# profess-dev/profess-ad

Hardware: AMD Instinct MI355X
Metric: energy+grad evals/sec (higher is better)
Workload: dtype f64; 1 GPU; 256^3 grid, f64, IonElectron+Hartree+WGC99(+TF+vW)+PBE closure chi->(E,dE/dchi); density=converged fcc-Al 32^3 fixture tiled 8^3 + 1e-3 low-|k| perturbation, parallelism=single GPU

## Files before the change

include/ofdft_hip.h:

```cpp
#ifndef OFDFT_HIP_H
#define OFDFT_HIP_H

#include <stdint.h>

#ifdef __cplusplus
extern "C" {
#endif

typedef struct ofdft_ctx ofdft_ctx;

#define OFDFT_OK            0
#define OFDFT_EINVAL       -1
#define OFDFT_EHIP         -2
#define OFDFT_ESTATE       -3
#define OFDFT_ENOMEM       -4

#define OFDFT_F64 0
#define OFDFT_F32 1

#define OFDFT_ION_ELECTRON  (1u << 0)
#define OFDFT_HARTREE       (1u << 1)
#define OFDFT_TF            (1u << 2)
#define OFDFT_VW            (1u << 3)
#define OFDFT_WT_NL         (1u << 4)
#define OFDFT_WGC99_NL      (1u << 5)
#define OFDFT_LDA_X         (1u << 6)
#define OFDFT_PZ_C          (1u << 7)
#define OFDFT_PW_C          (1u << 8)
#define OFDFT_CHACHIYO_C    (1u << 9)
#define OFDFT_PBE_X         (1u << 10)
#define OFDFT_PBE_C         (1u << 11)
#define OFDFT_GGA_K         (1u << 12)
#define OFDFT_VWGTF         (1u << 13)
#define OFDFT_NTERMS        14

#define OFDFT_P_WT_ALPHA    0
#define OFDFT_P_WT_BETA     1
#define OFDFT_P_WGC_ALPHA   2
#define OFDFT_P_WGC_BETA    3
#define OFDFT_P_WGC_GAMMA   4
#define OFDFT_P_WGC_KAPPA   5
#define OFDFT_P_GGAK_KIND   6
#define OFDFT_P_GGAK_MU     7
#define OFDFT_P_GGAK_BETA   8
#define OFDFT_P_GGAK_LAMBDA 9
#define OFDFT_P_GGAK_SIGMA  10
#define OFDFT_P_VWGTF_KIND  11
#define OFDFT_P_WTS_KIND    12
#define OFDFT_NPARAMS       13

#define OFDFT_Q_FFT_COUNT        0
#define OFDFT_Q_WORKSPACE_BYTES  1
#define OFDFT_Q_FAST_PATH        2
#define OFDFT_Q_KERNEL_MS        3
#define OFDFT_Q_LAUNCH_COUNT     4
#define OFDFT_Q_YPASS_COUNT      5
#define OFDFT_Q_GRAPH_REPLAYS     6
#define OFDFT_Q_RESIDENT_EVALS    7
#define OFDFT_Q_XCHG_CHUNKS      9
#define OFDFT_Q_YFWD_FUSED      10
#define OFDFT_Q_RESIDENT_FALLBACKS 8
#define OFDFT_Q_XPASS_KINDS     11
#define OFDFT_XPASS_GROUP    (1u << 0)
#define OFDFT_XPASS_WAVE     (1u << 1)
#define OFDFT_XPASS_CROSS1   (1u << 2)
#define OFDFT_XPASS_CROSS2   (1u << 3)
#define OFDFT_XPASS_CHIRPZ   (1u << 4)

int  ofdft_create(ofdft_ctx** out, int n0, int n1, int n2, int dtype, int device_id);
void ofdft_destroy(ofdft_ctx* ctx);
const char* ofdft_last_error(const ofdft_ctx* ctx);

int  ofdft_set_cell(ofdft_ctx* ctx, const double box_vecs[9]);
int  ofdft_set_terms(ofdft_ctx* ctx, uint32_t term_mask, const double* params, int nparams);

int  ofdft_energy_potential(ofdft_ctx* ctx, const void* den_dev, const void* vext_dev,
                            double* E_terms_host, void* dEdn_dev, void* stream);

int  ofdft_energy_grad_chi(ofdft_ctx* ctx, const void* chi_dev, const void* vext_dev, double n_electrons,
                           double* E_terms_host, double* mu_host, void* grad_dev, void* stream);

int  ofdft_rfftn(ofdft_ctx* ctx, const void* real_dev, void* spec_dev, void* stream);
int  ofdft_irfftn(ofdft_ctx* ctx, const void* spec_dev, void* real_dev, void* stream);
int  ofdft_debug_math(ofdft_ctx* ctx, int kind, const void* in_dev, void* out_dev, long long n, void* stream);

int  ofdft_query(ofdft_ctx* ctx, int what, double* out);

int  ofdft_ipc_export(ofdft_ctx* ctx, void* handle64, unsigned long long* offsets5);
int  ofdft_ipc_attach(ofdft_ctx* ctx, int peer_rank, const void* handle64, const unsigned long long* offsets5);
int  ofdft_ipc_detach(ofdft_ctx* ctx);
int  ofdft_dist_closure(ofdft_ctx* ctx, const void* chi_local_dev, const void* vext_local_dev, double n_electrons_global,
                        double* E_terms_host, double* mu_host, void* grad_local_dev, void* v_work_local_dev, void* stream);

typedef int (*ofdft_all_to_all_fn)(void* user, void* send_dev, void* recv_dev, unsigned long long bytes_per_peer, void* stream);
typedef int (*ofdft_all_reduce_fn)(void* user, double* host_buf, int count);
int  ofdft_set_collectives(ofdft_ctx* ctx, ofdft_all_to_all_fn all_to_all, ofdft_all_reduce_fn all_reduce, void* user);

int  ofdft_create_dist(ofdft_ctx** out, int n0_global, int n1_global, int n2, int dtype, int device_id, int nranks, int rank);
int  ofdft_dist_sumsq(ofdft_ctx* ctx, const void* x_local_dev, int square, double* local_sum_host, void* stream);
int  ofdft_dist_begin(ofdft_ctx* ctx, const void* src_local_dev, int from_chi, double cscale, double n_electrons_global,
                      const void* vext_local_dev, void* v_out_local_dev, void* stream);
int  ofdft_dist_stage(ofdft_ctx* ctx, int stage, int chain, void* stream, unsigned long long* bytes_per_peer, void** sendbuf_dev,
                      void** recvbuf_dev);
int  ofdft_dist_step(ofdft_ctx* ctx, int step, int chain, int chunk, void* stream, unsigned long long* bytes_per_peer,
                     void** sendbuf_dev, void** recvbuf_dev);
int  ofdft_dist_finish(ofdft_ctx* ctx, double* local_sums_host , void* stream);
int  ofdft_dist_scalars(ofdft_ctx* ctx, void** scalars_dev );
int  ofdft_dist_energies(ofdft_ctx* ctx, const double* global_sums , double* E_terms_host, double* vn_integral);
int  ofdft_dist_chi_grad(ofdft_ctx* ctx, const void* chi_local_dev, const void* v_local_dev, void* grad_local_dev,
                         double cscale, double mu, void* stream);

int  ofdft_ionic_potential(ofdft_ctx* ctx, const double* frac_coords_host, int nions, const double* table_k_host,
                           const double* table_v_host, int ntable, double z_ion, int pme_order, void* vext_dev,
                           int accumulate, void* stream);

int  ofdft_ion_electron_forces(ofdft_ctx* ctx, const void* den_dev, const double* frac_coords_host, int nions,
                               const double* table_k_host, const double* table_v_host, int ntable, double z_ion,
                               int pme_order, double* forces_host, void* stream);

int  ofdft_stress(ofdft_ctx* ctx, const void* den_dev, double* sigma_terms_host, void* stream);
int  ofdft_ion_electron_stress(ofdft_ctx* ctx, const void* den_dev, const double* frac_coords_host, int nions,
                               const double* table_k_host, const double* table_v_host, int ntable, double z_ion,
                               int pme_order, double* sigma_host , void* stream);

int  ofdft_ion_ion(ofdft_ctx* ctx, const double* frac_coords_host, const double* charges_host, int nions, double Rc,
                   double* E_host, double* forces_host, double* stress_host, void* stream);

typedef struct ofdft_lbfgs ofdft_lbfgs;
int  ofdft_lbfgs_create(ofdft_lbfgs** out, long long n_local, int history , int device_id);
void ofdft_lbfgs_destroy(ofdft_lbfgs* h);
const char* ofdft_lbfgs_last_error(const ofdft_lbfgs* h);
int  ofdft_lbfgs_reset(ofdft_lbfgs* h);
int  ofdft_lbfgs_direction(ofdft_lbfgs* h, const double* dots , int npairs, int first_iteration,
                           double* coef_s , double* coef_y , double* coef_g, double* g_dot_d,
                           int* npairs_out, int* pushed_out);
int  ofdft_lbfgs_abs_step(ofdft_lbfgs* h, double* abs_step_sum);
int  ofdft_lbfgs_dots(ofdft_lbfgs* h, const void* g_dev, double* dots_host , int* npairs, void* stream);
int  ofdft_lbfgs_commit(ofdft_lbfgs* h, int push);
int  ofdft_lbfgs_update(ofdft_lbfgs* h, const double* coef_s, const double* coef_y, double coef_g, double t, void* x_dev,
                        const void* g_dev, double* abs_step_sum_host, void* stream);

#define OFDFT_OPT_PIPELINE 0
#define OFDFT_OPT_XCHUNKS     2
#define OFDFT_OPT_XCHUNK_MASK 3
#define OFDFT_OPT_SPLIT_COMBINE 4
#define OFDFT_OPT_BLUESTEIN 5
#define OFDFT_OPT_GGA_SPLIT 6
#define OFDFT_OPT_GRAPH 7
#define OFDFT_OPT_SIDE_STREAM 1
#define OFDFT_OPT_MIXED_RADIX 9
#define OFDFT_OPT_RESIDENT 10
#define OFDFT_OPT_XCHG_CHUNKS 12
#define OFDFT_OPT_YBATCH 14
#define OFDFT_OPT_IPC_WAIT_MS 13
#define OFDFT_OPT_TEST_FAULT 11
#define OFDFT_OPT_BS_FUSED 15
#define OFDFT_OPT_WGC_FOLD 28
#define OFDFT_OPT_XWAVE 8
int  ofdft_set_option(ofdft_ctx* ctx, int option, double value);

int  ofdft_set_profiling(ofdft_ctx* ctx, int on);
int  ofdft_profile_count(ofdft_ctx* ctx);
int  ofdft_profile_get(ofdft_ctx* ctx, int idx, char* name_buf, int buflen, double* total_ms, long long* launches);

#ifdef __cplusplus
}
#endif
#endif
```

professad_amd/csrc/engine.hip:

```cpp
#include "engine_ctx.h"
#include <atomic>
#include <chrono>
#ifndef OFDFT_REAL_F32
#include "ion_kernels.h"
#include "stress_kernels.h"
#endif

namespace {
thread_local char g_create_error[512] = "";
}

namespace eng {

int fail(ofdft_ctx* c, int code, const char* fmt, ...) {
    va_list ap;
    va_start(ap, fmt);
    vsnprintf(c ? c->err : g_create_error, 512, fmt, ap);
    va_end(ap);
    return code;
}

int get_twiddle(ofdft_ctx* c, int n, cplx** out) {
    auto it = c->tw.find(n);
    if (it != c->tw.end()) {
// ... 1344 lines not shown
        *bytes_per_peer = (unsigned long long)(sizeof(cplx) * (size_t)c->xg.nxl * c->xg.arr_sz * r.xlist[chain].size());
        *sendbuf = send;
        *recvbuf = recv;
        c->recv_parity[chain] ^= 1;
    }
    HIP_TRY(c, hipGetLastError());
    return OFDFT_OK;
}

int ofdft_dist_step(ofdft_ctx* c, int step, int chain, int chunk, void* stream, unsigned long long* bytes_per_peer, void** sendbuf,
                    void** recvbuf) {
    hipStream_t st = (hipStream_t)stream;
    if (!c || !bytes_per_peer || !sendbuf || !recvbuf || chain < 0 || chain > 1) return OFDFT_EINVAL;
    OFDFT_ON_DEVICE(c, c->device);
    ZRun& r = zrun(c);
    const int K = c->xc.n;
    const bool next_chunk = step == r.step[chain] && chunk == r.step_chunk[chain] + 1 && chunk < K;
    const bool next_step = step == r.step[chain] + 1 && chunk == 0 && (r.step[chain] == 0 || r.step_chunk[chain] == K - 1);
    if (step < 1 || step > 6 || !(next_chunk || next_step) || (chain == 1 && r.step[0] < 1))
        return fail(c, OFDFT_ESTATE, "step %d chunk %d of chain %d out of order (last: step %d chunk %d of %d)", step, chunk, chain,
                    r.step[chain], r.step_chunk[chain], K);
    int rc;
    switch (step) {
        case 1: rc = zstage1(c, st, chain, chunk); break;
        case 2: rc = zstage2(c, st, chain, chunk); break;
        case 3: rc = zstage3(c, st, chain, 1, chunk); break;
        case 4: rc = zstage3(c, st, chain, 2, chunk); break;
        case 5: rc = zstage4(c, st, chain, chunk); break;
        default: rc = chain == 0 ? zstage5(c, nullptr, st, false, 1, chunk) : 0; break;
    }
    if (rc) return rc;
    r.step[chain] = step;
    r.step_chunk[chain] = chunk;
    *bytes_per_peer = 0;
    *sendbuf = *recvbuf = nullptr;
    const bool sends = step == 1 || step == 2 || step == 4 || step == 5;
    if (sends && c->nranks > 1 && !r.xlist[chain].empty()) {
        cplx *send, *recv;
        if ((rc = dist_buffers(c, chain, &send, &recv))) return rc;
        if ((rc = dist_recv_next(c, chain, &recv))) return rc;
        const XcView v = xc_view(c, chunk);
        const long long narr = (long long)r.xlist[chain].size();
        *bytes_per_peer = (unsigned long long)(sizeof(cplx) * (size_t)c->xg.nxl * v.arr_sz * narr);
        *sendbuf = send + narr * v.base1;
        *recvbuf = recv + narr * v.base1;
        if (chunk == K - 1) c->recv_parity[chain] ^= 1;
    }
    if (step == 5 && chunk == K - 1) r.stage[chain] = 4;
    HIP_TRY(c, hipGetLastError());
    return OFDFT_OK;
}

int ofdft_dist_finish(ofdft_ctx* c, double* local_sums, void* stream) {
    hipStream_t st = (hipStream_t)stream;
    if (!c) return OFDFT_EINVAL;
    OFDFT_ON_DEVICE(c, c->device);
    ZRun& r = zrun(c);
    if (r.stage[0] != 4 || r.stage[1] != 4) return fail(c, OFDFT_ESTATE, "ofdft_dist_finish called before stage 4 of both chains");
    const bool stepped = r.step[0] > 0;
    if (stepped && !(r.step[0] == 6 && r.step_chunk[0] == c->xc.n - 1 && r.step[1] == 6 && r.step_chunk[1] == c->xc.n - 1))
        return fail(c, OFDFT_ESTATE, "ofdft_dist_finish called before step 6 of both chains");
    int rc;
    if ((rc = zstage5(c, local_sums, st, false, stepped ? 2 : 0))) return rc;
    if (!local_sums) {
        HIP_TRY(c, hipEventRecord(c->ev1, st));
        c->ms_pending = true;
        HIP_TRY(c, hipGetLastError());
        if (c->profiling) {
            HIP_TRY(c, hipStreamSynchronize(st));
            prof_collect(c);
        }
        return OFDFT_OK;
    }
    return end_call(c, st);
}

int ofdft_dist_energies(ofdft_ctx* c, const double* global_sums, double* E_terms, double* vn_int) {
    if (!c || !global_sums || !E_terms || !vn_int) return OFDFT_EINVAL;
    for (int i = 0; i < OFDFT_NTERMS; ++i) E_terms[i] = 0.0;
    energies_from_sums(c, global_sums, global_sums + kCombineScalars, E_terms, vn_int);
    return OFDFT_OK;
}

int ofdft_dist_chi_grad(ofdft_ctx* c, const void* chi_local, const void* v_local, void* grad_local, double cscale,
                        double mu, void* stream) {
    hipStream_t st = (hipStream_t)stream;
    if (!c || !chi_local || !v_local || !grad_local) return OFDFT_EINVAL;
    OFDFT_ON_DEVICE(c, c->device);
    OFDFT_LAUNCH(c, st, "chi_grad", chi_grad_kernel, dim3(grid_for(c->npts / 2 + 1)), dim3(256), 0, (const real*)chi_local,
                 (const real*)v_local, (real*)grad_local, c->npts, cscale * 2.0 * c->dV,
                 cscale > 0.0 ? (const acc_t*)nullptr : (const acc_t*)c->d_scal, 2.0 * c->dV, mu);
    HIP_TRY(c, hipGetLastError());
    return OFDFT_OK;
}

#ifndef OFDFT_REAL_F32
#include "engine_ions_stress.inc.h"
#else
#define OFDFT_F64_ONLY(c) fail(c, OFDFT_EINVAL, "%s is served by the fp64 library (libofdft_hip.so) only", __func__)
extern "C" {
int ofdft_ionic_potential(ofdft_ctx* c, const double*, int, const double*, const double*, int, double, int, void*, int, void*) {
    return OFDFT_F64_ONLY(c);
}
int ofdft_ion_electron_forces(ofdft_ctx* c, const void*, const double*, int, const double*, const double*, int, double, int,
                              double*, void*) {
    return OFDFT_F64_ONLY(c);
}
int ofdft_stress(ofdft_ctx* c, const void*, double*, void*) { return OFDFT_F64_ONLY(c); }
int ofdft_ion_electron_stress(ofdft_ctx* c, const void*, const double*, int, const double*, const double*, int, double, int,
                              double*, void*) {
    return OFDFT_F64_ONLY(c);
}
int ofdft_ion_ion(ofdft_ctx* c, const double*, const double*, int, double, double*, double*, double*, void*) {
    return OFDFT_F64_ONLY(c);
}
}
#endif

int ofdft_set_collectives(ofdft_ctx* c, ofdft_all_to_all_fn all_to_all, ofdft_all_reduce_fn all_reduce, void* user) {
    if (!c) return OFDFT_EINVAL;
    c->a2a = all_to_all;
    c->allreduce = all_reduce;
    c->coll_user = user;
    return OFDFT_OK;
}

int ofdft_set_option(ofdft_ctx* c, int option, double value) {
    if (!c) return OFDFT_EINVAL;
    c->version++;
    switch (option) {
        case OFDFT_OPT_GRAPH:
            c->use_graph = value != 0.0;
            return OFDFT_OK;
        case OFDFT_OPT_PIPELINE:
            c->force_unfused = value == 1.0;
            c->pipeline = (int)value;
            return OFDFT_OK;
        case OFDFT_OPT_SIDE_STREAM:
            c->use_side_stream = value != 0.0;
            return OFDFT_OK;
        case OFDFT_OPT_XCHUNKS:
            if (value < 0.0 || value > 64.0) return fail(c, OFDFT_EINVAL, "x chunks must be 0 (automatic) or 1..64");
            c->xchunks = (int)value;
            return OFDFT_OK;
        case OFDFT_OPT_BLUESTEIN:
            c->use_bluestein = value != 0.0;
            return OFDFT_OK;
        case OFDFT_OPT_BS_FUSED:
            c->bs_fused = value != 0.0;
            return OFDFT_OK;
        case OFDFT_OPT_GGA_SPLIT:
            c->gga_split = value != 0.0;
            return OFDFT_OK;
        case OFDFT_OPT_SPLIT_COMBINE:
            c->split_combine = value != 0.0;
            c->defer_vpart = value != 1.0;
            return OFDFT_OK;
        case OFDFT_OPT_XCHUNK_MASK:
            c->xchunk_mask = (int)value & 31;
            return OFDFT_OK;
        case OFDFT_OPT_MIXED_RADIX:
            if (c->nranks > 1 && value == 0.0 && !all_pow2(c))
                return fail(c, OFDFT_EINVAL, "a slab-decomposed context on extents with factors 3 / 5 has no other path than the mixed-radix plans");
            c->fast = line_extent_ok(c->n0g) && line_extent_ok(c->n1g) && row_extent_ok(c->n2) && is_pow2(c->nranks) &&
                      (value != 0.0 || all_pow2(c));
            return OFDFT_OK;
        case OFDFT_OPT_XWAVE:
            c->use_xwave = (int)value;
            return OFDFT_OK;
        case OFDFT_OPT_RESIDENT:
            if (value != 0.0 && value != 1.0 && value != 2.0) return fail(c, OFDFT_EINVAL, "OFDFT_OPT_RESIDENT takes 0, 1 or 2");
            c->resident = (int)value;
            return OFDFT_OK;
        case OFDFT_OPT_XCHG_CHUNKS:
            if (value < 0.0 || value > 16.0) return fail(c, OFDFT_EINVAL, "OFDFT_OPT_XCHG_CHUNKS takes 0 (automatic) or 1..16");
            xchg_chunks_set(c, (int)value);
            c->wgc_valid = false;
            return OFDFT_OK;
        case OFDFT_OPT_YBATCH:
            c->ybatch = (int)value;
            return OFDFT_OK;
        case OFDFT_OPT_WGC_FOLD:
            c->wgc_fold = value != 0.0;
            return OFDFT_OK;
        case OFDFT_OPT_IPC_WAIT_MS:
            if (!(value >= 1.0 && value <= 3.6e6)) return fail(c, OFDFT_EINVAL, "OFDFT_OPT_IPC_WAIT_MS takes 1 .. 3 600 000 ms");
            c->ipc_wait_ms = value;
            return OFDFT_OK;
        case OFDFT_OPT_TEST_FAULT:
            c->test_fault = (int)value;
            if (c->test_fault == 2) c->res_fits = 0;
            return OFDFT_OK;
    }
    return fail(c, OFDFT_EINVAL, "unknown option %d", option);
}

int ofdft_set_profiling(ofdft_ctx* c, int on) {
    if (!c) return OFDFT_EINVAL;
    c->profiling = on != 0;
    c->prof.clear();
    c->pending.clear();
    c->ev_used = 0;
    return OFDFT_OK;
}

int ofdft_profile_count(ofdft_ctx* c) { return c ? (int)c->prof.size() : OFDFT_EINVAL; }

int ofdft_profile_get(ofdft_ctx* c, int idx, char* name_buf, int buflen, double* total_ms, long long* launches) {
    if (!c || idx < 0 || idx >= (int)c->prof.size() || !name_buf || buflen < 2) return OFDFT_EINVAL;
    auto it = c->prof.begin();
    std::advance(it, idx);
    std::snprintf(name_buf, (size_t)buflen, "%s", it->first.c_str());
    if (total_ms) *total_ms = it->second.ms;
    if (launches) *launches = it->second.launches;
    return OFDFT_OK;
}

int ofdft_query(ofdft_ctx* c, int what, double* out) {
    if (!c || !out) return OFDFT_EINVAL;
    switch (what) {
        case OFDFT_Q_FFT_COUNT: *out = c->fft_count; return OFDFT_OK;
        case OFDFT_Q_WORKSPACE_BYTES: *out = (double)c->ws_bytes; return OFDFT_OK;
        case OFDFT_Q_FAST_PATH: *out = c->fast ? 1.0 : 0.0; return OFDFT_OK;
        case OFDFT_Q_KERNEL_MS:
            if (c->ms_pending) {
                OFDFT_ON_DEVICE(c, c->device);
                HIP_TRY(c, hipEventSynchronize(c->ev1));
                HIP_TRY(c, hipEventElapsedTime(&c->last_ms, c->ev0, c->ev1));
                c->ms_pending = false;
            }
            *out = c->last_ms;
            return OFDFT_OK;
        case OFDFT_Q_LAUNCH_COUNT: *out = c->launch_count; return OFDFT_OK;
        case OFDFT_Q_YPASS_COUNT: *out = c->ypass_count; return OFDFT_OK;
        case OFDFT_Q_GRAPH_REPLAYS: *out = (double)c->graph_replays; return OFDFT_OK;
        case OFDFT_Q_RESIDENT_EVALS: *out = (double)c->resident_evals; return OFDFT_OK;
        case OFDFT_Q_RESIDENT_FALLBACKS: *out = (double)c->resident_fallbacks; return OFDFT_OK;
        case OFDFT_Q_XCHG_CHUNKS: *out = (double)c->xc.n; return OFDFT_OK;
        case OFDFT_Q_YFWD_FUSED: *out = (double)c->yfwd_fused; return OFDFT_OK;
        case OFDFT_Q_XPASS_KINDS: *out = (double)c->xpass_kinds; return OFDFT_OK;
        case 16: case 17: case 18: case 19: case 20: case 21: case 22: case 23: case 24: case 25: case 26: case 27:
            *out = c->h_partial[what] * 0.01;
            return OFDFT_OK;
    }
    return fail(c, OFDFT_EINVAL, "unknown query %d", what);
}

}

#include "lbfgs_abi.h"
```

professad_amd/csrc/engine_ctx.h:

```cpp
#pragma once
#include <hip/hip_runtime.h>

#include <algorithm>
#include <cmath>
#include <cstdarg>
#include <cstdio>
#include <cstring>
#include <map>
#include <string>
#include <vector>

#include "../../include/ofdft_hip.h"
#include "bluestein.h"
#include "zpass.h"
#include "xwave.h"

using namespace ofdft;

struct DevBuf {
    void* p = nullptr;
    size_t bytes = 0;
    bool borrowed = false;
};

struct XchgChunks {
    int n = 1;
    int kb[17] = {0};
};

struct ofdft_ctx {
    int n0 = 0, n1 = 0, n2 = 0, device = 0;
    int n0g = 0, n1g = 0, nranks = 1, rank = 0;
    SpecGeom g{};
    SpecGeom gx{};
    KGeom kg{};
    XchgGeom xg{};
    XchgChunks xc{};
    int xchg_chunks_req = 0;
    long long npts = 0;
    long long npts_g = 0;
    bool fast = false, cell_set = false, force_unfused = false;
    int pipeline = 0;
    double box[9] = {0}, vol = 0.0, dV = 0.0;
    unsigned mask = 0;
    double params[OFDFT_NPARAMS];
    std::map<int, cplx*> tw;
    std::map<std::string, DevBuf> ws;
    size_t ws_bytes = 0;
    double* d_partial = nullptr;
    double* d_reduced = nullptr;
    double* d_scal = nullptr;
    double* h_partial = nullptr;
    long long partial_rows = 0;
    double* d_wgc_coef = nullptr;
    long long wgc_key_nel = -1;
    int fft_passes_fused = 0;
    int yfwd_fused = 0;
    bool wgc_valid = false;
    double wgc_ck = 0.0;
    bool wgc_fold = true;
    int fft_count = 0, launch_count = 0;
    unsigned xpass_kinds = 0;
    double ypass_count = 0.0;
    float last_ms = 0.f;
    bool ms_pending = false;
    hipEvent_t ev0 = nullptr, ev1 = nullptr, ev_fork = nullptr, ev_join = nullptr, ev_join2 = nullptr, ev_a = nullptr, ev_b = nullptr, ev_c = nullptr;
    hipStream_t side_stream = nullptr, side_stream2 = nullptr;
    bool use_side_stream = true;
    bool bs_fused = true;
    bool use_bluestein = true;
    bool gga_split = true;
    bool split_combine = true;
    bool defer_vpart = true;
    int ybatch = 1;
    int xchunk_mask = 2;
    int use_xwave = 1;
    int xchunks = 1;
    bool profiling = false;
    std::vector<hipEvent_t> ev_pool;
    size_t ev_used = 0;
    struct Pending { const char* name; size_t a, b; };
    std::vector<Pending> pending;
    struct Acc { double ms = 0.0; long long launches = 0; };
    std::map<std::string, Acc> prof;
    struct ofdft_zrun_holder* zr = nullptr;
    struct GraphEntry {
        const void *chi = nullptr, *vext = nullptr, *grad = nullptr;
        double nel = 0.0;
        unsigned long long version = 0;
        int seen = 0;
        hipGraphExec_t exec = nullptr;
        int collect = 0;
        int fft_count = 0, launch_count = 0, yfwd_fused = 0;
        unsigned xpass_kinds = 0;
        double ypass_count = 0.0;
    };
    std::vector<GraphEntry> graphs;
    unsigned long long version = 1;
    bool use_graph = true;
    int resident = 2;
    unsigned* res_sync = nullptr;
    unsigned res_epoch = 0;
    long long resident_evals = 0;
    int test_fault = 0;
    int res_fits = -1;
    long long resident_fallbacks = 0;
    unsigned* res_done = nullptr;
    unsigned res_done_target = 0;
    long long graph_replays = 0;
    hipStream_t cap_stream = nullptr;
    struct ofdft_ipc_state* ipc = nullptr;
    int recv_parity[2] = {0, 0};
    double ipc_wait_ms = 30000.0;
    ofdft_all_to_all_fn a2a = nullptr;
    ofdft_all_reduce_fn allreduce = nullptr;
    void* coll_user = nullptr;
    char err[512] = "";
};


namespace eng {

constexpr unsigned kGgaAny = OFDFT_PBE_X | OFDFT_PBE_C | OFDFT_GGA_K;
constexpr int kNSums = kCombineScalars + kPbeScalars;
constexpr int kSumsqSlot = 15;

inline GgaSel gga_sel(const ofdft_ctx* c) {
    return GgaSel{(c->mask & OFDFT_PBE_X) ? 1 : 0, (c->mask & OFDFT_PBE_C) ? 1 : 0, (c->mask & OFDFT_GGA_K) ? 1 : 0,
                  (int)c->params[OFDFT_P_GGAK_KIND], (real)c->params[OFDFT_P_GGAK_MU], (real)c->params[OFDFT_P_GGAK_BETA],
                  (real)c->params[OFDFT_P_GGAK_LAMBDA], (real)c->params[OFDFT_P_GGAK_SIGMA]};
}

inline bool gga_needs_laplacian(const ofdft_ctx* c) {
    return (c->mask & OFDFT_GGA_K) && (int)c->params[OFDFT_P_GGAK_KIND] == 1 &&
           (c->params[OFDFT_P_GGAK_BETA] != 0.0 || c->params[OFDFT_P_GGAK_LAMBDA] != 0.0 || c->params[OFDFT_P_GGAK_SIGMA] != 0.0);
}
inline bool wts_active(const ofdft_ctx* c) {
    return (int)c->params[OFDFT_P_WTS_KIND] == 1 && (c->mask & OFDFT_TF) && (c->mask & OFDFT_WT_NL);
}
inline bool zfused_serves(const ofdft_ctx* c) {
    return c->fast && c->pipeline == 0 && c->n2 / 2 <= 512 && (!gga_needs_laplacian(c) || c->gga_split);
}

int fail(ofdft_ctx* c, int code, const char* fmt, ...);

#define HIP_TRY(ctx, call)                                                                         \
    do {                                                                                           \
        hipError_t e_ = (call);                                                                    \
        if (e_ != hipSuccess)                                                                      \
            return fail(ctx, OFDFT_EHIP, "%s failed: %s (%s:%d)", #call, hipGetErrorString(e_), __FILE__, __LINE__); \
    } while (0)


#define OFDFT_ON_DEVICE(ctx, dev)                                                                   \
    DeviceScope device_scope_(dev);                                                                 \
    if (device_scope_.err != hipSuccess)                                                            \
        return fail(ctx, OFDFT_EHIP, "cannot select device %d: %s", (dev), hipGetErrorString(device_scope_.err))

inline bool graph_eligible(const ofdft_ctx* c) { return c->use_graph && c->nranks == 1 && c->npts <= (1LL << 19); }
void prof_begin(ofdft_ctx* c, hipStream_t st, const char* name);
void prof_end(ofdft_ctx* c, hipStream_t st);
void prof_collect(ofdft_ctx* c);

#define OFDFT_LAUNCH(c, st, name, kern, grid, block, lds, ...)            \
    do {                                                                  \
        prof_begin(c, st, name);                                          \
        hipLaunchKernelGGL(kern, grid, block, lds, st, __VA_ARGS__);      \
        prof_end(c, st);                                                  \
        (c)->launch_count++;                                              \
    } while (0)

inline bool is_pow2(int n) { return n > 0 && (n & (n - 1)) == 0; }

#if !defined(OFDFT_REAL_F32) || !defined(OFDFT_NO_MIXED_F32)
#define OFDFT_MIXED_LINES(X) X(48) X(96) X(120) X(144) X(160) X(192) X(240) X(250) X(270) X(288) X(320) X(384) X(480)
#define OFDFT_MIXED_ROWS(X) X(24) X(48) X(60) X(72) X(80) X(96) X(120) X(125) X(135) X(144) X(160) X(192) X(240)
#else
#define OFDFT_MIXED_LINES(X)
#define OFDFT_MIXED_ROWS(X)
#endif
inline bool mixed_line(int n) {
#define X(L) if (n == L) return true;
    OFDFT_MIXED_LINES(X)
#undef X
    return false;
}
inline bool line_extent_ok(int n) { return (is_pow2(n) && n >= 8 && n <= 1024) || mixed_line(n); }
inline bool row_extent_ok(int n2) { return (is_pow2(n2) && n2 >= 16 && n2 <= 2048) || mixed_line(n2); }
inline bool all_pow2(const ofdft_ctx* c) { return is_pow2(c->n0g) && is_pow2(c->n1g) && is_pow2(c->n2); }

inline int grid_for(long long n, int tpb = 256, int cap = 2048) {
    long long b = (n + tpb - 1) / tpb;
    if (b > cap) b = cap;
    if (b < 1) b = 1;
    return (int)b;
}

#define OFDFT_REDUCE(c, st, partial, rows, ns, ...)                                                                          \
    do {                                                                                                                     \
        const acc_t* part_ = (partial);                                                                                      \
        const int rows_ = (rows), ns_ = (ns);                                                                                \
        if (rows_ > kRedTwoLevelRows) {                                                                                      \
            acc_t* mid_ = const_cast<acc_t*>(part_) + (size_t)rows_ * ns_;                                                   \
            int g_ = rows_ / 512;                                                                                            \
            g_ = g_ < 1 ? 1 : (g_ > kRedMidRows ? kRedMidRows : g_);                                                         \
            const int per_ = (rows_ + g_ - 1) / g_;                                                                          \
            g_ = (rows_ + per_ - 1) / per_;                                                                                  \
            OFDFT_LAUNCH(c, st, "reduce", reduce_rows_kernel, dim3(g_), dim3(kRedThreads), 0, part_, rows_, ns_, per_, mid_); \
            OFDFT_LAUNCH(c, st, "reduce", reduce_partials_kernel, dim3(ns_), dim3(kRedThreads), 0, (const acc_t*)mid_, g_, ns_, \
                         __VA_ARGS__);                                                                                       \
        } else {                                                                                                             \
            OFDFT_LAUNCH(c, st, "reduce", reduce_partials_kernel, dim3(ns_), dim3(kRedThreads), 0, part_, rows_, ns_, __VA_ARGS__); \
        }                                                                                                                    \
    } while (0)


constexpr int kWholeXchg = -2;
struct XcView {
    int kb0, kb1, nb, nrem;
    long long arr_sz;
    long long base1;
};
inline XcView xc_view(const ofdft_ctx* c, int k) {
    XcView v{};
    const bool whole = k == kWholeXchg || c->xc.n <= 1;
    v.kb0 = whole ? 0 : c->xc.kb[k];
    v.kb1 = whole ? c->xg.nb : c->xc.kb[k + 1];
    v.nb = v.kb1 - v.kb0;
    v.nrem = (whole || k == c->xc.n - 1) ? c->xg.nrem : 0;
    v.arr_sz = ((long long)v.nb * 8 + v.nrem) * c->xg.nyl;
    v.base1 = (long long)c->n0g * c->xg.nyl * 8 * v.kb0;
    return v;
}
inline int xchg_chunks_for(const ofdft_ctx* c, int req) {
    if (c->nranks < 2 || c->xg.nb < 2 || c->xg.nxl % 32 || c->xg.nyl % 32) return 1;
    int k = req;
    if (k <= 0) {
        k = c->npts >= (8LL << 20) ? 4 : (c->npts >= (1LL << 20) ? 2 : 1);
        k = std::min(k, c->xg.nb / 4);
    }
    k = std::max(1, std::min(k, std::min(16, c->xg.nb)));
    return k;
}
inline void xchg_chunks_set(ofdft_ctx* c, int req) {
    c->xchg_chunks_req = req;
    c->xc = XchgChunks{};
    c->xc.n = xchg_chunks_for(c, req);
    for (int k = 0; k <= c->xc.n; ++k) c->xc.kb[k] = (int)((long long)c->xg.nb * k / c->xc.n);
}

int get_twiddle(ofdft_ctx* c, int n, cplx** out);
int get_ws(ofdft_ctx* c, const std::string& name, size_t bytes, void** out);
int real_ws(ofdft_ctx* c, const char* name, real** out);
int spec_ws(ofdft_ctx* c, const char* name, cplx** out);
size_t dist_buffer_bytes(ofdft_ctx* c, int chain);
int dist_buffers(ofdft_ctx* c, int chain, cplx** send, cplx** recv);
int dist_recv_next(ofdft_ctx* c, int chain, cplx** recv);
int dist_exchange(ofdft_ctx* c, cplx* send, cplx* recv, hipStream_t st);
int global_sums(ofdft_ctx* c, double* v, int n);

void pass_maps(const ofdft_ctx* c, int axis, LineMap& main, LineMap& rem);
template <bool INV>
int fast_axis_pass_multi(ofdft_ctx* c, int axis, cplx* const* specs, int narr, hipStream_t st, int x0 = 0, int cx = 0,
                         int kb0 = 0, int kb1 = 0);
template <bool INV> int fast_axis_pass(ofdft_ctx* c, int axis, cplx* spec, hipStream_t st);
template <bool INV> int ypass_xchg(ofdft_ctx* c, const std::vector<cplx*>& list, cplx* buf, hipStream_t st, int xk = -1);
int yderiv(ofdft_ctx* c, const cplx* in, cplx* out, double scale, hipStream_t st, cplx* fwd = nullptr);
int rfftn_internal(ofdft_ctx* c, const real* in, cplx* spec, hipStream_t st);
int rfftn_internal_multi(ofdft_ctx* c, const real* const* in, cplx* const* spec, int n, hipStream_t st);
bool bluestein_xmix_ok(const ofdft_ctx* c);
template <int NIN, int NOUT, class Mix>
int bluestein_xmix(ofdft_ctx* c, const cplx* const* in, cplx* const* out, const Mix& mix, hipStream_t st);
struct BsPrep { int kind[kBsBatch] = {0, 0, 0, 0}; double e[kBsBatch] = {0, 0, 0, 0}; double nref = 0.0; };
int bluestein_fwd_zy_multi(ofdft_ctx* c, const real* const* in, cplx* const* spec, int n, hipStream_t st, const BsPrep* prep = nullptr);
int bluestein_inv_yz_multi(ofdft_ctx* c, cplx* const* spec, real* const* out, int n, double scale, hipStream_t st);
int irfftn_internal_multi(ofdft_ctx* c, cplx* const* spec, real* const* out, int n, double scale, hipStream_t st);
int irfftn_internal(ofdft_ctx* c, cplx* spec, real* out, double scale, hipStream_t st);
int fwd_zy(ofdft_ctx* c, const real* in, cplx* spec, hipStream_t st);
int inv_yz(ofdft_ctx* c, cplx* spec, real* out, double scale, hipStream_t st);

struct XfLayout {
    long long se_in = 0, se_out = 0, tse = 0;
    int kb0 = 0, kb1 = 0;
    int xnb = -1, xnrem = 0;
    int kz0 = 0;
};
template <int NIN, int NOUT, class Mix>
int xfused(ofdft_ctx* c, const XfIo& io, const Mix& mix, hipStream_t st, const char* nm, const XfLayout& lay = XfLayout{});
int xfused_wgc(ofdft_ctx* c, const XfIo& io, const MixWgc& mix, hipStream_t st, const char* nm, const XfLayout& lay = XfLayout{});

int launch_zf_density(ofdft_ctx* c, const DenSrc& ds, cplx* out_n, cplx* out_s, hipStream_t st, int chunk = 0, int nchunks = 1,
                      real* dzn = nullptr);
int ensure_wgc_tables(ofdft_ctx* c, long long nel_rounded, hipStream_t st, double* nref_out);
inline MixWgc wgc_tab(ofdft_ctx* c, long long off = 0) {
    const cplx* t01 = (const cplx*)c->ws["t:wgc"].p;
    return MixWgc{t01 + off, reinterpret_cast<const real*>(t01 + c->g.total) + off, (real)c->wgc_ck};
}
bool resident_serves(const ofdft_ctx* c);
constexpr int kResidentDeclined = 1;
int resident_closure(ofdft_ctx* c, const real* chi, const real* vext, double nel, real* v, real* grad, hipStream_t st, bool from_den = false);
int launch_zf_powers(ofdft_ctx* c, const DenSrc& ds, const PowersArgs& pa, hipStream_t st, int chunk = 0, int nchunks = 1);
int launch_zpbe(ofdft_ctx* c, const DenSrc& ds, cplx* gx, cplx* gy, cplx* gz, real* dfdn, double inv_n, int* blocks_out,
                hipStream_t st, int chunk = 0, int nchunks = 1);
int launch_zpbe2(ofdft_ctx* c, const DenSrc& ds, cplx* A, cplx* B, const real* dzn, real* dfdn, double inv_n, int* blocks_out,
                 hipStream_t st, cplx* L = nullptr);
int launch_zi_combine(ofdft_ctx* c, const ZCombineArgs& a, int* blocks_out, hipStream_t st, int chunk = 0, int nchunks = 1);
int launch_zi_wgc(ofdft_ctx* c, const ZCombineArgs& a, real* v_part, double* partial, int* blocks_out, hipStream_t st);

}
```

professad_amd/csrc/engine_zfused.inc.h:

```cpp
void energies_from_sums(const ofdft_ctx* c, const double* sums, const double* pbe_sums, double* E_terms, double* vn_int) {
    const unsigned mask = c->mask;
    const double dV = c->dV;
    if (mask & OFDFT_ION_ELECTRON) E_terms[0] = sums[0] * dV;
    if (mask & OFDFT_HARTREE) E_terms[1] = sums[1] * dV;
    if (mask & OFDFT_TF) E_terms[2] = sums[2] * dV;
    if (mask & OFDFT_VW) E_terms[3] = sums[3] * dV;
    if (mask & OFDFT_WT_NL) E_terms[4] = sums[4] * dV;
    if (mask & OFDFT_WGC99_NL) E_terms[5] = sums[5] * dV;
    if (mask & OFDFT_LDA_X) E_terms[6] = sums[6] * dV;
    int nc = 0;
    for (int b = 7; b <= 9; ++b) nc += (mask >> b) & 1;
    for (int b = 7; b <= 9; ++b)
        if ((mask >> b) & 1) E_terms[b] = sums[7] * dV / nc;
    if (mask & OFDFT_PBE_X) E_terms[10] = pbe_sums[0] * dV;
    if (mask & OFDFT_PBE_C) E_terms[11] = pbe_sums[1] * dV;
    if (mask & OFDFT_GGA_K) E_terms[12] = pbe_sums[2] * dV;
    if (mask & OFDFT_VWGTF) E_terms[13] = sums[9] * dV;
    *vn_int = sums[8] * dV;
}

struct ZRun {
    DenSrc ds{};
    double nel = 0.0;
    const real* vext = nullptr;
    real* v_out = nullptr;
    ZCombineArgs za{};
    double pbe_sums[kPbeScalars] = {0.0, 0.0, 0.0};
    bool has_h = false, has_g = false, has_vw = false, has_wt = false, has_wgc = false;
    cplx *s_n = nullptr, *s_s = nullptr, *s_vh = nullptr, *s_g[3] = {nullptr, nullptr, nullptr};
    cplx *s_b = nullptr, *s_a = nullptr, *sw[6] = {nullptr, nullptr, nullptr, nullptr, nullptr, nullptr};
    real* dfdn = nullptr;
    double wt_pref = 0.0, wt_kf = 1.0;
    std::vector<cplx*> xlist[2];
    bool gsplit = false;
    bool lapl = false;
    cplx* s_l = nullptr;
    real* dzn = nullptr;
    bool wgc_yinv_done = false;
    bool wgc_split = false;
    bool closure = false;
    bool setup_done = false;
    bool late_join = false;
    bool vpart_deferred = false;
    std::vector<cplx*> deferred;
    int stage[2] = {0, 0};
    int step[2] = {0, 0}, step_chunk[2] = {0, 0};
    std::vector<cplx*> in_list[2];
    int combine_blocks = 0, pbe_blocks = 0;
    hipStream_t sb = nullptr;
    hipStream_t sc = nullptr;
    bool forked = false;
};

}
struct ofdft_zrun_holder { ZRun r; };
namespace {

ZRun& zrun(ofdft_ctx* c);

int chunks_for(const ofdft_ctx* c, int narr, int which = 15) {
    if (c->nranks > 1 || c->xchunks == 1 || !(c->xchunk_mask & which) || !all_pow2(c)) return 1;
    if (which == 8 && wts_active(c)) return 1;
    int want = c->xchunks > 1 ? (c->xchunks * narr + 5) / 6
                              : (int)std::min<double>(64.0, (double)narr * sizeof(cplx) * (double)c->g.total / 100e6);
    int n = 1;
    while (n * 2 <= want && c->n0 % (n * 2) == 0 && ((long long)(c->n0 / (n * 2)) * c->n1) % 256 == 0) n *= 2;
    return n;
}

#ifndef OFDFT_YDERIV_FWD
#define OFDFT_YDERIV_FWD 1
#endif
int zsetup(ofdft_ctx* c) {
    ZRun& r = zrun(c);
    const unsigned mask = c->mask;
    r.has_h = mask & OFDFT_HARTREE;
    r.has_g = mask & kGgaAny;
    r.has_vw = mask & OFDFT_VW;
    r.has_wt = mask & OFDFT_WT_NL;
    r.has_wgc = mask & OFDFT_WGC99_NL;
    r.za = ZCombineArgs{};
    r.za.ds = r.ds;
    r.za.vext = r.vext;
    r.za.v_out = r.v_out;
    r.za.mask = mask;
    r.za.inv_n = 1.0 / (double)c->npts_g;
    r.za.gtf_kind = (int)c->params[OFDFT_P_VWGTF_KIND];
    r.za.gtf_inv_n0 = (mask & OFDFT_VWGTF) ? c->vol / (double)std::llround(r.nel) : 0.0;
    r.pbe_sums[0] = r.pbe_sums[1] = r.pbe_sums[2] = 0.0;
    r.wgc_yinv_done = false;
    r.s_g[0] = r.s_g[1] = r.s_g[2] = nullptr;
    r.s_n = r.s_s = r.s_vh = r.s_b = r.s_a = nullptr;
    if ((mask & OFDFT_ION_ELECTRON) && !r.vext) return fail(c, OFDFT_EINVAL, "IonElectron term needs vext");
    r.setup_done = true;
    return 0;
}

int zstage1(ofdft_ctx* c, hipStream_t st, int chain, int xk = -1) {
    ZRun& r = zrun(c);
    int rc;
    hipStream_t sb = r.forked ? r.sb : st, sc = r.forked ? r.sc : st;
    const bool dx = c->nranks > 1;
    std::vector<cplx*>& xl = r.xlist[chain];
    if (xk <= 0) {
    xl.clear();
    if (chain == 0) {
        if (!r.setup_done && (rc = zsetup(c))) return rc;
        r.setup_done = false;
        if (r.has_h || r.has_g)
            if ((rc = spec_ws(c, "zn", &r.s_n))) return rc;
        if (r.has_vw)
            if ((rc = spec_ws(c, "zs", &r.s_s))) return rc;
        if (r.s_n || r.s_s) {
            cplx* both[2];
            int nb = 0;
            if (r.s_n) both[nb++] = r.s_n;
            if (r.s_s) both[nb++] = r.s_s;
            r.gsplit = r.has_g && c->gga_split;
            r.lapl = r.gsplit && gga_needs_laplacian(c);
            r.s_l = nullptr;
            if (r.gsplit) {
                if ((rc = real_ws(c, "dzn", &r.dzn))) return rc;
                if ((rc = spec_ws(c, "zgx", &r.s_g[0]))) return rc;
                if ((rc = spec_ws(c, "zgy", &r.s_g[1]))) return rc;
                if (r.lapl && (rc = spec_ws(c, "zgl", &r.s_l))) return rc;
            }
            const int nch = r.gsplit ? 1 : chunks_for(c, nb, 1);
            if (nch > 1) {
                for (int ch = 0; ch < nch; ++ch) {
                    if ((rc = launch_zf_density(c, r.ds, r.s_n, r.s_s, st, ch, nch))) return rc;
                    if ((rc = fast_axis_pass_multi<false>(c, 1, both, nb, st, ch * (c->n0 / nch), c->n0 / nch))) return rc;
                }
            } else if ((rc = launch_zf_density(c, r.ds, r.s_n, r.s_s, st, 0, 1, r.gsplit ? r.dzn : nullptr))) {
                return rc;
            }
            const bool yfwd = OFDFT_YDERIV_FWD && r.gsplit && !dx && nch == 1;
            if (r.gsplit && (rc = yderiv(c, r.s_n, r.s_g[1], (double)c->n0g, st, yfwd ? r.s_n : nullptr))) return rc;
            if (r.forked && r.s_s) {
                HIP_TRY(c, hipEventRecord(c->ev_a, st));
                HIP_TRY(c, hipStreamWaitEvent(sc, c->ev_a, 0));
            }
            if (!dx && nch == 1 && r.s_n && !yfwd && (rc = fast_axis_pass<false>(c, 1, r.s_n, st))) return rc;
            if (!dx && nch == 1 && r.s_s && (rc = fast_axis_pass<false>(c, 1, r.s_s, sc))) return rc;
            if (r.s_n) xl.push_back(r.s_n);
            if (r.s_s) xl.push_back(r.s_s);
        }
    } else {
        if (r.has_wt) {
            const double al = c->params[OFDFT_P_WT_ALPHA], be = c->params[OFDFT_P_WT_BETA];
            const double nbar = r.nel / c->vol;
            r.wt_kf = std::cbrt(3.0 * kPi * kPi * nbar);
            r.wt_pref = 5.0 / (9.0 * al * be * std::pow(nbar, al + be - kFiveThirds));
            if ((rc = spec_ws(c, "zwb", &r.s_b))) return rc;
            if (al != be && (rc = spec_ws(c, "zwa", &r.s_a))) return rc;
            PowersArgs pa{};
            pa.out[0] = r.s_b;
            pa.out[3] = r.s_a;
            pa.e0 = be;
            pa.e1 = al;
            if ((rc = launch_zf_powers(c, r.ds, pa, sb))) return rc;
            for (cplx* sp : {r.s_b, r.s_a}) {
                if (!sp) continue;
                if (!dx && (rc = fast_axis_pass<false>(c, 1, sp, sb))) return rc;
                xl.push_back(sp);
            }
            r.za.wt_alpha = al;
            r.za.wt_beta = be;
            r.za.wt_nbar_pa = std::pow(nbar, al);
            r.za.wt_is_56 = (al == kFiveSixths && be == kFiveSixths) ? 1 : 0;
        }
        if (r.has_wgc) {
            const double al = c->params[OFDFT_P_WGC_ALPHA], be = c->params[OFDFT_P_WGC_BETA];
            const long long nel_r = std::llround(r.nel);
            double nref;
            if ((rc = ensure_wgc_tables(c, nel_r, sb, &nref))) return rc;
            const char* wn[6] = {"zw0", "zw1", "zw2", "zw3", "zw4", "zw5"};
            PowersArgs pa{};
            for (int i = 0; i < 6; ++i) {
                if ((rc = spec_ws(c, wn[i], &r.sw[i]))) return rc;
                pa.out[i] = r.sw[i];
            }
            pa.e0 = be;
            pa.e1 = al;
            pa.nref = nref;
            pa.sum53 = (std::fabs(al + be - kFiveThirds) < 4e-16) ? 1 : 0;
            const int nch = chunks_for(c, 6, 2);
            if (nch > 1) {
                for (int ch = 0; ch < nch; ++ch) {
                    if ((rc = launch_zf_powers(c, r.ds, pa, sb, ch, nch))) return rc;
                    if ((rc = fast_axis_pass_multi<false>(c, 1, r.sw, 6, sb, ch * (c->n0 / nch), c->n0 / nch))) return rc;
                }
            } else if ((rc = launch_zf_powers(c, r.ds, pa, sb))) {
                return rc;
            }
            if (r.forked) {
                HIP_TRY(c, hipEventRecord(c->ev_b, sb));
                HIP_TRY(c, hipStreamWaitEvent(sc, c->ev_b, 0));
            }
            if (!dx && nch == 1 && c->ybatch) {
                if ((rc = fast_axis_pass_multi<false>(c, 1, r.sw, 3, sb))) return rc;
                if ((rc = fast_axis_pass_multi<false>(c, 1, r.sw + 3, 3, sc))) return rc;
            }
            for (int i = 0; i < 6; ++i) {
                if (!dx && nch == 1 && !c->ybatch && (rc = fast_axis_pass<false>(c, 1, r.sw[i], i < 3 ? sb : sc))) return rc;
                xl.push_back(r.sw[i]);
            }
            r.za.wgc_alpha = al;
            r.za.wgc_beta = be;
            r.za.nref = nref;
            r.za.wgc_sum_53 = pa.sum53;
        }
    }
    }
    if (dx && !xl.empty()) {
        cplx *send, *recv;
        if ((rc = dist_buffers(c, chain, &send, &recv))) return rc;
        if ((rc = ypass_xchg<false>(c, xl, send, st, xk))) return rc;
    }
    r.stage[chain] = 1;
    return 0;
}

int zstage2(ofdft_ctx* c, hipStream_t st, int chain, int xk = -1) {
    ZRun& r = zrun(c);
    int rc;
    hipStream_t sb = r.forked ? r.sb : st, sc = r.forked ? r.sc : st;
    const bool dx = c->nranks > 1;
    if (dx && xk == -1 && c->xc.n > 1) {
        for (int k = 0; k < c->xc.n; ++k)
            if ((rc = zstage2(c, st, chain, k))) return rc;
        return 0;
    }
    std::vector<cplx*>& xl = r.xlist[chain];
    if (xk <= 0) r.in_list[chain] = xl;
    const std::vector<cplx*>& in_list = r.in_list[chain];
    xl.clear();
    cplx *send = nullptr, *recv = nullptr;
    XfLayout lay{};
    const XcView xv = xc_view(c, xk < 0 ? 0 : xk);
    int nout = 0;
    if (dx) {
        if ((rc = dist_buffers(c, chain, &send, &recv))) return rc;
        nout = chain == 0 ? (r.has_h ? 1 : 0) + (r.has_g ? (r.gsplit ? (r.lapl ? 2 : 1) : 3) : 0) + (r.s_s ? 1 : 0)
                          : (r.s_b ? 1 : 0) + (r.s_a ? 1 : 0) + (r.has_wgc ? 6 : 0);
        lay = XfLayout{(long long)in_list.size() * xv.arr_sz, nout * xv.arr_sz, xv.arr_sz, 0, 0, xv.nb, xv.nrem, xv.kb0 * 8};
        recv += (long long)in_list.size() * xv.base1;
        send += (long long)nout * xv.base1;
    }
    auto in_of = [&](cplx* arr) -> cplx* {
        if (!dx) return arr;
        for (size_t i = 0; i < in_list.size(); ++i)
            if (in_list[i] == arr) return recv + (long long)i * xv.arr_sz;
        return nullptr;
    };
    auto out_of = [&](cplx* arr) -> cplx* {
        xl.push_back(arr);
        return dx ? send + (long long)(xl.size() - 1) * xv.arr_sz : arr;
    };
    if (chain == 0) {
        if (r.s_n) {
            XfIo io{};
            io.in[0] = in_of(r.s_n);
            int no = 0;
            if (r.has_h) {
                if ((rc = spec_ws(c, "zvh", &r.s_vh))) return rc;
                io.out[no++] = out_of(r.s_vh);
            }
            if (r.has_g && r.gsplit) {
                io.out[no++] = out_of(r.s_g[0]);
                if (r.lapl) io.out[no++] = out_of(r.s_l);
            } else if (r.has_g) {
                const char* gn[3] = {"zgx", "zgy", "zgz"};
                for (int k = 0; k < 3; ++k) {
                    if ((rc = spec_ws(c, gn[k], &r.s_g[k]))) return rc;
                    io.out[no++] = out_of(r.s_g[k]);
                }
            }
            if (r.lapl && r.has_h) rc = xfused<1, 3>(c, io, MixDensityA<true, true>{c->kg}, st, "xfused_n", lay);
            else if (r.lapl) rc = xfused<1, 2>(c, io, MixDensityA<false, true>{c->kg}, st, "xfused_n", lay);
            else if (r.gsplit && r.has_h) rc = xfused<1, 2>(c, io, MixDensityA<true>{c->kg}, st, "xfused_n", lay);
            else if (r.gsplit) rc = xfused<1, 1>(c, io, MixDensityA<false>{c->kg}, st, "xfused_n", lay);
            else if (r.has_h && r.has_g) rc = xfused<1, 4>(c, io, MixDensity<true, true>{c->kg}, st, "xfused_n", lay);
            else if (r.has_h) rc = xfused<1, 1>(c, io, MixDensity<true, false>{c->kg}, st, "xfused_n", lay);
            else rc = xfused<1, 3>(c, io, MixDensity<false, true>{c->kg}, st, "xfused_n", lay);
            if (rc) return rc;
        }
        if (r.s_s) {
            XfIo io{};
            io.in[0] = in_of(r.s_s);
            io.out[0] = out_of(r.s_s);
            if ((rc = xfused<1, 1>(c, io, MixScale<SPEC_LAPLACE>{c->kg, 0.0, 0.0}, sc, "xfused_lap", lay))) return rc;
        }
    } else {
        if (r.has_wt) {
            const MixScale<SPEC_LINDHARD> lind{c->kg, (real)r.wt_pref, (real)(1.0 / (2.0 * r.wt_kf))};
            for (cplx* sp : {r.s_b, r.s_a}) {
                if (!sp) continue;
                XfIo io{};
                io.in[0] = in_of(sp);
                io.out[0] = out_of(sp);
                if ((rc = xfused<1, 1>(c, io, lind, sb, "xfused_lind", lay))) return rc;
            }
        }
        if (r.has_wgc) {
            const MixWgc mix = wgc_tab(c, dx ? xv.base1 : 0);
            const int nb = c->g.nzm / 8;
            int nkz = (!dx && (c->xchunk_mask & 16) && c->xchunks != 1) ? chunks_for(c, 6, 16) : 1;
            while (nkz > 1 && nb % nkz) nkz >>= 1;
            r.wgc_yinv_done = nkz > 1;
            for (int half = 0; half < 2; ++half) {
                XfIo io{};
                for (int i = 0; i < 3; ++i) {
                    io.in[i] = in_of(r.sw[3 * half + i]);
                    io.out[i] = out_of(r.sw[3 * half + i]);
                }
                hipStream_t hs = half == 0 ? sb : sc;
                if (nkz == 1) {
                    if ((rc = xfused_wgc(c, io, mix, hs, "xfused_wgc", lay))) return rc;
                    continue;
                }
                for (int ch = 0; ch < nkz; ++ch) {
                    XfLayout lk = lay;
                    lk.kb0 = ch * (nb / nkz);
                    lk.kb1 = (ch + 1) * (nb / nkz);
                    if ((rc = xfused_wgc(c, io, mix, hs, "xfused_wgc", lk))) return rc;
                    if ((rc = fast_axis_pass_multi<true>(c, 1, r.sw + 3 * half, 3, hs, 0, 0, lk.kb0, lk.kb1))) return rc;
                }
            }
        }
    }
    r.stage[chain] = 2;
    return 0;
}

int zstage3(ofdft_ctx* c, hipStream_t st, int chain, int part = 0, int xk = -1) {
    ZRun& r = zrun(c);
    int rc;
    hipStream_t sb = r.forked ? r.sb : st, sc = r.forked ? r.sc : st;
    const bool dx = c->nranks > 1;
    std::vector<cplx*>& xl = r.xlist[chain];
    cplx *send = nullptr, *recv = nullptr;
    if (dx && !xl.empty() && part != 2) {
        if ((rc = dist_buffers(c, chain, &send, &recv))) return rc;
        if ((rc = ypass_xchg<true>(c, xl, recv, st, xk))) return rc;
    }
    if (part == 1) return 0;
    if (part == 2 && xk > 0) {
        if (dx && chain == 0 && !xl.empty()) {
            if ((rc = dist_buffers(c, 0, &send, &recv))) return rc;
            if ((rc = ypass_xchg<false>(c, xl, send, st, xk))) return rc;
        }
        return 0;
    }
    const int yk = part == 2 ? 0 : -1;
    const bool chunked = chunks_for(c, 6, 8) > 1, pbe_chunked = !r.gsplit && chunks_for(c, 6, 4) > 1;
    const bool wbatch = !dx && c->ybatch && chain == 1 && r.has_wgc && !r.wgc_yinv_done && !chunked && xl.size() >= 6;
    if (wbatch) {
        if ((rc = fast_axis_pass_multi<true>(c, 1, r.sw, 3, sb))) return rc;
        if ((rc = fast_axis_pass_multi<true>(c, 1, r.sw + 3, 3, sc))) return rc;
    }
    for (cplx* sp : xl) {
        const bool on_b = sp == r.s_b || sp == r.s_a || sp == r.sw[0] || sp == r.sw[1] || sp == r.sw[2];
        const bool on_c = sp == r.s_s || sp == r.sw[3] || sp == r.sw[4] || sp == r.sw[5];
        const bool is_g = sp == r.s_g[0] || sp == r.s_g[1] || sp == r.s_g[2] || (r.s_l && sp == r.s_l);
        const bool is_w = sp == r.sw[0] || sp == r.sw[1] || sp == r.sw[2] || sp == r.sw[3] || sp == r.sw[4] || sp == r.sw[5];
        if (is_w && (r.wgc_yinv_done || wbatch)) {
        } else if (is_g ? pbe_chunked : chunked) {
            if (!is_g) r.deferred.push_back(sp);
        } else if (!dx && (rc = fast_axis_pass<true>(c, 1, sp, on_b ? sb : (on_c ? sc : st)))) {
            return rc;
        }
        if (!is_g) c->fft_count++;
    }
    xl.clear();
    if (chain == 1) {
        if (r.has_wt) {
            r.za.conv_b = r.s_b;
            r.za.conv_a = r.s_a;
        }
        if (r.has_wgc)
            for (int i = 0; i < 3; ++i) {
                r.za.u[i] = r.sw[i];
                r.za.gw[i] = r.sw[3 + i];
            }
        r.wgc_split = false;
        if (r.has_wgc && !chunked && c->split_combine && !graph_eligible(c)) {
            real* vp;
            acc_t* part2;
            int blocks = 0;
            if ((rc = real_ws(c, "vpart", &vp))) return rc;
            if ((rc = get_ws(c, "zwgc:part", sizeof(double) * 2 * (size_t)(c->partial_rows + kRedMidRows), (void**)&part2))) return rc;
            if (r.forked) {
                HIP_TRY(c, hipEventRecord(c->ev_c, sc));
                HIP_TRY(c, hipStreamWaitEvent(sb, c->ev_c, 0));
            }
            if ((rc = launch_zi_wgc(c, r.za, vp, part2, &blocks, sb))) return rc;
            OFDFT_REDUCE(c, sb, (const acc_t*)part2, blocks, 2, c->d_scal + 2, c->h_partial + kNSums);
            r.za.v_part = vp;
            r.wgc_split = true;
            r.vpart_deferred = r.closure && r.forked && c->defer_vpart;
            r.za.v_part_deferred = r.vpart_deferred ? 1 : 0;
        }
        r.stage[1] = 3;
        return 0;
    }
    if (r.has_h) r.za.vh = r.s_vh;
    if (r.s_s) r.za.lap = r.s_s;
    if (r.has_g && r.gsplit) {
        if ((rc = real_ws(c, "dfdn", &r.dfdn))) return rc;
        if ((rc = launch_zpbe2(c, r.ds, r.s_g[0], r.s_g[1], r.dzn, r.dfdn, r.za.inv_n, &r.pbe_blocks, st, r.lapl ? r.s_l : nullptr)))
            return rc;
        OFDFT_REDUCE(c, st, c->d_partial, r.pbe_blocks, kPbeScalars, c->d_reduced + kCombineScalars, c->h_partial + kCombineScalars);
        if ((rc = yderiv(c, r.s_g[1], r.s_g[1], (double)c->n0g, st))) return rc;
        if (!dx && (rc = fast_axis_pass<false>(c, 1, r.s_g[0], st))) return rc;
        xl.push_back(r.s_g[0]);
        if (r.lapl) {
            if (!dx && (rc = fast_axis_pass<false>(c, 1, r.s_l, st))) return rc;
            xl.push_back(r.s_l);
        }
        if (dx) {
            if ((rc = dist_buffers(c, 0, &send, &recv))) return rc;
            if ((rc = ypass_xchg<false>(c, xl, send, st, yk))) return rc;
        }
    } else if (r.has_g) {
        if ((rc = real_ws(c, "dfdn", &r.dfdn))) return rc;
        const int nch = chunks_for(c, 6, 4);
        for (int ch = 0; ch < nch; ++ch) {
            const int x0 = ch * (c->n0 / nch), cx = c->n0 / nch;
            if (pbe_chunked && (rc = fast_axis_pass_multi<true>(c, 1, r.s_g, 3, st, x0, cx))) return rc;
            if ((rc = launch_zpbe(c, r.ds, r.s_g[0], r.s_g[1], r.s_g[2], r.dfdn, r.za.inv_n, &r.pbe_blocks, st, ch, nch)))
                return rc;
            if (pbe_chunked && (rc = fast_axis_pass_multi<false>(c, 1, r.s_g, 3, st, x0, cx))) return rc;
        }
        OFDFT_REDUCE(c, st, c->d_partial, r.pbe_blocks, kPbeScalars, c->d_reduced + kCombineScalars, c->h_partial + kCombineScalars);
        for (int k = 0; k < 3; ++k) {
            if (!dx && !pbe_chunked && (rc = fast_axis_pass<false>(c, 1, r.s_g[k], st))) return rc;
            xl.push_back(r.s_g[k]);
        }
        if (dx) {
            if ((rc = dist_buffers(c, 0, &send, &recv))) return rc;
            if ((rc = ypass_xchg<false>(c, xl, send, st, yk))) return rc;
        }
    }
    r.stage[0] = 3;
    return 0;
}

int zstage4(ofdft_ctx* c, hipStream_t st, int chain, int xk = -1) {
    ZRun& r = zrun(c);
    if (c->nranks > 1 && xk == -1 && c->xc.n > 1) {
        for (int k = 0; k < c->xc.n; ++k)
            if (int rc = zstage4(c, st, chain, k)) return rc;
        return 0;
    }
    r.xlist[chain].clear();
    const XcView xv = xc_view(c, xk < 0 ? 0 : xk);
    if (chain == 0 && r.has_g && r.gsplit) {
        XfIo dio{};
        XfLayout lay{};
        dio.in[0] = dio.out[0] = r.s_g[0];
        const int nin = r.lapl ? 2 : 1;
        if (c->nranks > 1) {
            cplx *send, *recv;
            if (int rc = dist_buffers(c, 0, &send, &recv)) return rc;
            dio.in[0] = recv + (long long)nin * xv.base1;
            dio.out[0] = send + xv.base1;
            lay = XfLayout{xv.arr_sz, xv.arr_sz, xv.arr_sz, 0, 0, xv.nb, xv.nrem, xv.kb0 * 8};
        }
        if (r.lapl) {
            dio.in[1] = r.s_l;
            if (c->nranks > 1) {
                dio.in[1] = dio.in[0] + xv.arr_sz;
                lay.se_in = 2 * xv.arr_sz;
            }
            if (int rc = xfused<2, 1>(c, dio, MixDerivAL{c->kg}, st, "xfused_div", lay)) return rc;
        } else if (int rc = xfused<1, 1>(c, dio, MixDerivA{c->kg}, st, "xfused_div", lay)) {
            return rc;
        }
        r.xlist[0].push_back(r.s_g[0]);
    } else if (chain == 0 && r.has_g) {
        XfIo dio{};
        XfLayout lay{};
        for (int k = 0; k < 3; ++k) dio.in[k] = r.s_g[k];
        dio.out[0] = r.s_n;
        if (c->nranks > 1) {
            cplx *send, *recv;
            if (int rc = dist_buffers(c, 0, &send, &recv)) return rc;
            for (int k = 0; k < 3; ++k) dio.in[k] = recv + 3 * xv.base1 + k * xv.arr_sz;
            dio.out[0] = send + xv.base1;
            lay = XfLayout{3 * xv.arr_sz, xv.arr_sz, xv.arr_sz, 0, 0, xv.nb, xv.nrem, xv.kb0 * 8};
        }
        if (int rc = xfused<3, 1>(c, dio, MixDiv{c->kg}, st, "xfused_div", lay)) return rc;
        r.xlist[0].push_back(r.s_n);
    }
    r.stage[chain] = 4;
    return 0;
}

constexpr int kCollectWgcSplit = 1;
constexpr int kCollectVnShare = 2;
constexpr int kCollectNoGga = 4;
int collect_flags(const ZRun& r, bool late_join) {
    return (r.wgc_split ? kCollectWgcSplit : 0) | (late_join ? kCollectVnShare : 0) | (r.has_g ? 0 : kCollectNoGga);
}
void zfused_collect(const ofdft_ctx* c, int flags, double* sums) {
    for (int i = 0; i < kNSums; ++i) sums[i] = c->h_partial[i];
    if (flags & kCollectNoGga)
        for (int i = kCombineScalars; i < kNSums; ++i) sums[i] = 0.0;
    if (flags & kCollectWgcSplit) sums[5] += c->h_partial[kNSums];
    if (flags & kCollectVnShare) sums[8] += c->h_partial[kNSums + 1];
}

int zstage5(ofdft_ctx* c, double* sums, hipStream_t st, bool defer = false, int part = 0, int xk = -1) {
    ZRun& r = zrun(c);
    int rc;
    const bool chunked = chunks_for(c, 6, 8) > 1;
    if (part == 1) {
        if (r.has_g && c->nranks > 1) {
            cplx *send, *recv;
            if ((rc = dist_buffers(c, 0, &send, &recv))) return rc;
            if ((rc = ypass_xchg<true>(c, {r.gsplit ? r.s_g[0] : r.s_n}, recv, st, xk))) return rc;
        }
        return 0;
    }
    if (r.has_g) {
        cplx* dsp = r.gsplit ? r.s_g[0] : r.s_n;
        if (c->nranks > 1) {
            cplx *send, *recv;
            if ((rc = dist_buffers(c, 0, &send, &recv))) return rc;
            if (part != 2 && (rc = ypass_xchg<true>(c, {dsp}, recv, st))) return rc;
        } else if (chunked) {
            r.deferred.push_back(dsp);
        } else if ((rc = fast_axis_pass<true>(c, 1, dsp, st))) {
            return rc;
        }
        c->fft_count++;
        r.za.div = dsp;
        r.za.div2 = r.gsplit ? r.s_g[1] : nullptr;
        r.za.dfdn = r.dfdn;
    }
    r.xlist[0].clear();
    r.xlist[1].clear();
    const bool late_join = r.forked && r.vpart_deferred && r.wgc_split;
    if (r.forked) {
        if (!late_join) {
            HIP_TRY(c, hipEventRecord(c->ev_join, r.sb));
            HIP_TRY(c, hipStreamWaitEvent(st, c->ev_join, 0));
        }
        HIP_TRY(c, hipEventRecord(c->ev_join2, r.sc));
        HIP_TRY(c, hipStreamWaitEvent(st, c->ev_join2, 0));
    }
    const bool wts = wts_active(c);
    r.za.wts_w = nullptr;
    if (wts) {
        ZCombineArgs z1 = r.za;
        z1.v_out = nullptr;
        if ((rc = launch_zi_combine(c, z1, &r.combine_blocks, st))) return rc;
        OFDFT_REDUCE(c, st, c->d_partial, r.combine_blocks, kCombineScalars, c->d_reduced);
        OFDFT_LAUNCH(c, st, "reduce", wts_weights_kernel, dim3(1), dim3(64), 0, (const acc_t*)c->d_reduced, c->d_scal + 4);
        r.za.wts_w = c->d_scal + 4;
    }
    if (chunked) {
        const int narr = (int)r.deferred.size();
        const int nch = chunks_for(c, narr + 2, 8);
        for (int ch = 0; ch < nch; ++ch) {
            if (narr && (rc = fast_axis_pass_multi<true>(c, 1, r.deferred.data(), narr, st, ch * (c->n0 / nch), c->n0 / nch)))
                return rc;
            if ((rc = launch_zi_combine(c, r.za, &r.combine_blocks, st, ch, nch))) return rc;
        }
        r.deferred.clear();
    } else if ((rc = launch_zi_combine(c, r.za, &r.combine_blocks, st))) {
        return rc;
    }
    OFDFT_REDUCE(c, st, c->d_partial, r.combine_blocks, kCombineScalars, c->d_reduced, (sums && !wts) ? c->h_partial : (acc_t*)nullptr);
    if (wts) OFDFT_LAUNCH(c, st, "reduce", wts_finalize_kernel, dim3(1), dim3(64), 0, c->d_reduced, (const acc_t*)(c->d_scal + 4));
    if (late_join) {
        HIP_TRY(c, hipEventRecord(c->ev_join, r.sb));
        HIP_TRY(c, hipStreamWaitEvent(st, c->ev_join, 0));
        if (!sums)
            OFDFT_LAUNCH(c, st, "reduce", (axpy_kernel<acc_t>), dim3(1), dim3(64), 0, (const acc_t*)(c->d_scal + 3), c->d_reduced + 8,
                         (long long)1, 1);
    }
    r.late_join = late_join && sums != nullptr;
    if (!r.has_g) HIP_TRY(c, hipMemsetAsync(c->d_reduced + kCombineScalars, 0, kPbeScalars * sizeof(double), st));
    r.stage[0] = r.stage[1] = 5;
    if (!sums) {
        if (r.wgc_split)
            OFDFT_LAUNCH(c, st, "reduce", (axpy_kernel<acc_t>), dim3(1), dim3(64), 0, (const acc_t*)(c->d_scal + 2), c->d_reduced + 5,
                         (long long)1, 1);
        return 0;
    }
    if (wts) HIP_TRY(c, hipMemcpyAsync(c->h_partial, c->d_reduced, sizeof(double) * kCombineScalars, hipMemcpyDeviceToHost, st));
    if (defer) return 0;
    HIP_TRY(c, hipStreamSynchronize(st));
    zfused_collect(c, collect_flags(r, r.late_join), sums);
    return 0;
}

int zfused_enqueue(ofdft_ctx* c, const DenSrc& ds, double nel, const real* vext, real* v_out, double* sums, hipStream_t st,
                   bool defer) {
    if ((c->mask & OFDFT_ION_ELECTRON) && !vext) return fail(c, OFDFT_EINVAL, "IonElectron term needs vext");
    if (!ds.src) return fail(c, OFDFT_EINVAL, "null density pointer");
    ZRun& r = zrun(c);
    r.ds = ds;
    r.nel = nel;
    r.vext = vext;
    r.v_out = v_out;
    r.deferred.clear();
    r.closure = defer;
    r.vpart_deferred = false;
    r.za.v_part_deferred = 0;
    int rc;
    r.forked = c->use_side_stream && c->side_stream && c->side_stream2 && (c->mask & (OFDFT_WT_NL | OFDFT_WGC99_NL)) &&
               (c->mask & (OFDFT_HARTREE | OFDFT_VW | kGgaAny));
    if (r.forked) {
        r.sb = c->side_stream;
        r.sc = c->side_stream2;
        HIP_TRY(c, hipEventRecord(c->ev_fork, st));
        HIP_TRY(c, hipStreamWaitEvent(r.sb, c->ev_fork, 0));
        HIP_TRY(c, hipStreamWaitEvent(r.sc, c->ev_fork, 0));
    }
    r.setup_done = false;
    rc = zsetup(c);
    const bool nl_first = r.forked && c->nranks == 1;
    for (int i = 0; i < 2 && !rc; ++i) rc = zstage1(c, st, nl_first ? 1 - i : i);
    for (int chain = 0; chain < 2 && !rc; ++chain) rc = zstage2(c, st, chain);
    for (int chain = 0; chain < 2 && !rc; ++chain) rc = zstage3(c, st, chain);
    if (!rc) rc = zstage4(c, st, 0);
    if (!rc) rc = zstage5(c, sums, st, defer);
    r.setup_done = false;
    return rc;
}

int run_terms_zfused(ofdft_ctx* c, const DenSrc& ds, double nel, const real* vext, double* E_terms, real* v_out,
                     double* vn_int, hipStream_t st) {
    for (int i = 0; i < OFDFT_NTERMS; ++i) E_terms[i] = 0.0;
    double sums[kNSums];
    if (int rc = zfused_enqueue(c, ds, nel, vext, v_out, sums, st, false)) return rc;
    energies_from_sums(c, sums, sums + kCombineScalars, E_terms, vn_int);
    return 0;
}

ZRun& zrun(ofdft_ctx* c) {
    if (!c->zr) c->zr = new ofdft_zrun_holder();
    return c->zr->r;
}

int begin_call(ofdft_ctx* c, hipStream_t st, bool timed = true) {
    if (!c) return OFDFT_EINVAL;
    if (!c->cell_set) return fail(c, OFDFT_ESTATE, "ofdft_set_cell has not been called");
    c->fft_count = 0;
    c->launch_count = 0;
    c->xpass_kinds = 0;
    c->ypass_count = 0.0;
    c->yfwd_fused = 0;
    if (timed) HIP_TRY(c, hipEventRecord(c->ev0, st));
    return 0;
}
int end_call(ofdft_ctx* c, hipStream_t st, bool timed = true) {
    if (timed) HIP_TRY(c, hipEventRecord(c->ev1, st));
    HIP_TRY(c, hipStreamSynchronize(st));
    if (timed) HIP_TRY(c, hipEventElapsedTime(&c->last_ms, c->ev0, c->ev1));
    else c->last_ms = 0.f;
    c->ms_pending = false;
    HIP_TRY(c, hipGetLastError());
    if (c->profiling) prof_collect(c);
    return 0;
}

}
```

professad_amd/csrc/fft_kernels.h:

```cpp
#pragma once
#include "fft_radix.h"

namespace ofdft {

struct SpecGeom {
    int n0, n1, n2, nzc, nzm;
    int blk0 = 0;
    long long nrows;
    long long main_count;
    long long total;
};

__host__ __device__ inline long long spec_index(const SpecGeom& g, int x, int y, int kz) {
    const long long row = (long long)x * g.n1 + y;
    if (kz < g.nzm) return (((long long)(kz >> 3)) * g.nrows + row) * 8 + (kz & 7);
    return g.main_count + (long long)(kz - g.nzm) * g.nrows + row;
}

__device__ inline void spec_decode(const SpecGeom& g, long long i, int& x, int& y, int& kz) {
    if (i < g.main_count) {
        const int kin = (int)(i & 7);
        const long long r = i >> 3;
        const long long row = r % g.nrows;
        kz = (int)(r / g.nrows) * 8 + kin;
        x = (int)(row / g.n1);
        y = (int)(row % g.n1);
    } else {
        const long long r = i - g.main_count;
        const long long row = r % g.nrows;
        kz = g.nzm + (int)(r / g.nrows);
        x = (int)(row / g.n1);
        y = (int)(row % g.n1);
    }
}

struct LineMap {
    long long sb;
    long long se;
    int d;
    int sl;
    int nlines;
    int lf;
    int gc = 0, gn = 0, g0 = 0;
    int blk0 = 0;
    int kz0 = 0;
};

#ifndef OFDFT_CPASS_TPB
#define OFDFT_CPASS_TPB 256
#endif
template <int LEN> struct PassCfg {
    static constexpr int P = Plan<LEN>::P;
    static constexpr int E = Plan<LEN>::E;
    static constexpr int TPB = (8 * P > OFDFT_CPASS_TPB) ? 8 * P : OFDFT_CPASS_TPB;
    static constexpr int LPW = TPB / P;
    static constexpr int LSTR = kCXMul * LineBuf<LEN>::STRIDE;
    static constexpr size_t LDS = (Plan<LEN>::NST > 1) ? sizeof(real) * LPW * LSTR : 0;
};

__device__ __forceinline__ long long line_base(const LineMap& m, long long L) {
    long long grp = L / m.d;
    if (m.gc) grp = (grp / m.gc) * m.gn + m.g0 + grp % m.gc;
    return grp * m.sb + (L % m.d) * (long long)m.sl;
}

struct ArrList { cplx* p[16]; };

#ifndef OFDFT_CPASS_LD_AUX
#define OFDFT_CPASS_LD_AUX 2
#endif
#ifndef OFDFT_CPASS_ST_AUX
#define OFDFT_CPASS_ST_AUX 2
#endif
#ifndef OFDFT_XF_LD_AUX
#define OFDFT_XF_LD_AUX 0
#endif
#ifndef OFDFT_XF_BATCH_TABLES
#define OFDFT_XF_BATCH_TABLES 1
#endif
#ifndef OFDFT_XF_ST_AUX
#define OFDFT_XF_ST_AUX 2
#endif
#ifndef OFDFT_ZS_LD_AUX
#define OFDFT_ZS_LD_AUX 0
#endif
#ifndef OFDFT_ZS_ST_AUX
#define OFDFT_ZS_ST_AUX 0
#endif
#ifndef OFDFT_ZR_LD_AUX
#define OFDFT_ZR_LD_AUX 0
#endif
#ifndef OFDFT_ZR_ST_AUX
#define OFDFT_ZR_ST_AUX 0
#endif

#ifndef OFDFT_CPASS_TILES
#define OFDFT_CPASS_TILES 1
#endif
template <int LEN, bool INV>
__global__ __launch_bounds__(PassCfg<LEN>::TPB) void cpass_kernel(ArrList arrs, LineMap m_main, LineMap m_rem,
                                                                   int main_blocks, long long rem_offset,
                                                                   const cplx* __restrict__ tw) {
    cplx* data0 = arrs.p[blockIdx.y];
    constexpr int P = PassCfg<LEN>::P, E = PassCfg<LEN>::E, LPW = PassCfg<LEN>::LPW, T = OFDFT_CPASS_TILES;
    extern __shared__ __attribute__((aligned(16))) real lds[];
    const int tid = threadIdx.x;
    using PL = Plan<LEN>;
    cplx v[T][E];
    cplx* ubs[T];
    unsigned voffs[T];
    bool valids[T];
    long long se_us[T];
    int js[T], ls[T];
#pragma unroll
    for (int t = 0; t < T; ++t) {
        const int blk = (int)blockIdx.x * T + t;
        const bool in_rem = blk >= main_blocks;
        const LineMap m = in_rem ? m_rem : m_main;
        cplx* data = in_rem ? data0 + rem_offset : data0;
        const int bid = in_rem ? blk - main_blocks : blk + m.blk0;
        const int l_lo = tid % m.lf;
        const int j = (tid / m.lf) % P;
        const int l = (tid / (m.lf * P)) * m.lf + l_lo;
        const long long L0 = (long long)bid * LPW;
        const long long L = L0 + l;
        const bool valid = L < m.nlines;
        const long long b0 = uniform64(line_base(m, L0));
        ubs[t] = data + b0;
        voffs[t] = valid ? (unsigned)((line_base(m, L) - b0 + (long long)j * m.se) * kCB) : 0u;
        se_us[t] = uniform64(m.se);
        valids[t] = valid;
        js[t] = j;
        ls[t] = l;
#pragma unroll
        for (int q = 0; q < E; ++q)
            v[t][q] = (PL::slot_in(q) && valid && PL::lane_in(j, q)) ? buf_load_c_aux<OFDFT_CPASS_LD_AUX>(ubs[t] + PL::cin(q) * se_us[t], voffs[t])
                                                                       : mkc(0.0, 0.0);
    }
#pragma unroll
    for (int t = 0; t < T; ++t) {
        if (t > 0) __syncthreads();
        line_fft<LEN, INV, kCX>(v[t], js[t], lds + ls[t] * PassCfg<LEN>::LSTR, tw);
        if (valids[t]) {
#pragma unroll
            for (int q = 0; q < E; ++q)
                if (PL::slot_out(q) && PL::lane_out(js[t], q)) buf_store_c_aux<OFDFT_CPASS_ST_AUX>(ubs[t] + PL::cout(q) * se_us[t], voffs[t], v[t][q]);
        }
    }
}

template <class PL, bool WAVE>
__device__ __forceinline__ void repattern_out_to_in(cplx (&v)[PL::E], int j, real* line) {
    if constexpr (!PL::EXACT) {
        constexpr int E = PL::E;
        real re[E];
        exchange_sync<WAVE>();
#pragma unroll
        for (int q = 0; q < E; ++q)
            if (PL::slot_out(q) && PL::lane_out(j, q)) line[lpos<PL>(j + PL::cout(q))] = v[q].x;
        exchange_sync<WAVE>();
#pragma unroll
        for (int q = 0; q < E; ++q) re[q] = (PL::slot_in(q) && PL::lane_in(j, q)) ? line[lpos<PL>(j + PL::cin(q))] : (real)0.0;
        exchange_sync<WAVE>();
#pragma unroll
        for (int q = 0; q < E; ++q)
            if (PL::slot_out(q) && PL::lane_out(j, q)) line[lpos<PL>(j + PL::cout(q))] = v[q].y;
        exchange_sync<WAVE>();
#pragma unroll
        for (int q = 0; q < E; ++q)
            v[q] = (PL::slot_in(q) && PL::lane_in(j, q)) ? mkc(re[q], line[lpos<PL>(j + PL::cin(q))]) : mkc(0.0, 0.0);
        exchange_sync<WAVE>();
    }
}

template <int LEN>
__global__ __launch_bounds__(PassCfg<LEN>::TPB) void yderiv_kernel(const cplx* in, cplx* out,
                                                                   LineMap m_main, LineMap m_rem, int main_blocks,
                                                                   long long rem_offset, const cplx* __restrict__ tw,
                                                                   real scale, cplx* fwd) {
    constexpr int P = PassCfg<LEN>::P, E = PassCfg<LEN>::E, LPW = PassCfg<LEN>::LPW;
    extern __shared__ __attribute__((aligned(16))) real lds[];
    const int tid = threadIdx.x;
    const bool in_rem = (int)blockIdx.x >= main_blocks;
    const LineMap m = in_rem ? m_rem : m_main;
    const long long roff = in_rem ? rem_offset : 0;
    const int bid = in_rem ? (int)blockIdx.x - main_blocks : (int)blockIdx.x + m.blk0;
    const int l_lo = tid % m.lf;
    const int j = (tid / m.lf) % P;
    const int l = (tid / (m.lf * P)) * m.lf + l_lo;
    const long long L0 = (long long)bid * LPW;
    const long long L = L0 + l;
    const bool valid = L < m.nlines;
    const long long b0 = uniform64(line_base(m, L0));
    const unsigned voff = valid ? (unsigned)((line_base(m, L) - b0 + (long long)j * m.se) * kCB) : 0u;
    const long long se_u = uniform64(m.se);
    using PL = Plan<LEN>;
    cplx v[E];
#pragma unroll
    for (int q = 0; q < E; ++q)
        v[q] = (PL::slot_in(q) && valid && PL::lane_in(j, q)) ? buf_load_c(in + roff + b0 + PL::cin(q) * se_u, voff) : mkc(0.0, 0.0);
    real* mine = lds + l * PassCfg<LEN>::LSTR;
    line_fft<LEN, false, kCX>(v, j, mine, tw);
    if (fwd && valid) {
#pragma unroll
        for (int q = 0; q < E; ++q)
            if (PL::slot_out(q) && PL::lane_out(j, q)) buf_store_c_aux<OFDFT_CPASS_ST_AUX>(fwd + roff + b0 + PL::cout(q) * se_u, voff, v[q]);
    }
#pragma unroll
    for (int q = 0; q < E; ++q) {
        const int e = j + PL::cout(q);
        const real f = scale * (real)(e <= LEN / 2 ? e : e - LEN);
        v[q] = mkc(-f * v[q].y, f * v[q].x);
    }
    __syncthreads();
    repattern_out_to_in<PL, false>(v, j, mine);
    line_fft<LEN, true, kCX>(v, j, mine, tw);
    if (valid) {
#pragma unroll
        for (int q = 0; q < E; ++q)
            if (PL::slot_out(q) && PL::lane_out(j, q)) buf_store_c_aux<OFDFT_CPASS_ST_AUX>(out + roff + b0 + PL::cout(q) * se_u, voff, v[q]);
    }
}

struct XchgGeom {
    int nxl, nyl, log_nyl, nb, nrem;
    long long arr_sz;
    long long rec;
    long long chunk;
    int kb0 = 0;
};
template <int LEN, bool INV>
__global__ __launch_bounds__(PassCfg<LEN>::TPB) void ypass_xchg_kernel(ArrList arrs, cplx* __restrict__ buf, XchgGeom xg,
                                                                       LineMap m_main, LineMap m_rem, int main_blocks,
                                                                       long long rem_offset,
                                                                       const cplx* __restrict__ tw) {
    constexpr int P = PassCfg<LEN>::P, E = PassCfg<LEN>::E, LPW = PassCfg<LEN>::LPW;
    extern __shared__ __attribute__((aligned(16))) real lds[];
    const int tid = threadIdx.x;
    const int a = blockIdx.y;
    const bool in_rem = (int)blockIdx.x >= main_blocks;
    const LineMap m = in_rem ? m_rem : m_main;
    cplx* data = arrs.p[a] + (in_rem ? rem_offset : 0);
    const int bid = in_rem ? (int)blockIdx.x - main_blocks : (int)blockIdx.x + m.blk0;
    const int l_lo = tid % m.lf;
    const int j = (tid / m.lf) % P;
    const int l = (tid / (m.lf * P)) * m.lf + l_lo;
    const long long L0 = (long long)bid * LPW;
    const long long L = L0 + l;
    const bool valid = L < m.nlines;
    const long long b0 = uniform64(line_base(m, L0));
    cplx* ub = data + b0;
    const unsigned voff = valid ? (unsigned)((line_base(m, L) - b0 + (long long)j * m.se) * kCB) : 0u;
    using PL = Plan<LEN>;
    long long lb;
    int es;
    if (!in_rem) {
        const long long r = L >> 3;
        const int kin = (int)(L & 7), xl = (int)(r % xg.nxl);
        const long long b = r / xg.nxl - xg.kb0;
        lb = xl * xg.rec + a * xg.arr_sz + b * xg.nyl * 8 + kin;
        es = 8;
    } else {
        const int xl = (int)(L % xg.nxl);
        const long long plane = L / xg.nxl;
        lb = xl * xg.rec + a * xg.arr_sz + (long long)xg.nb * xg.nyl * 8 + plane * xg.nyl;
        es = 1;
    }
    auto bpos = [&](int e) -> long long {
        int peer, yl;
        if constexpr (PL::EXACT) {
            peer = e >> xg.log_nyl;
            yl = e & (xg.nyl - 1);
        } else {
            peer = e / xg.nyl;
            yl = e - peer * xg.nyl;
        }
        return lb + (long long)peer * xg.chunk + (long long)yl * es;
    };
    const long long se_u = uniform64(m.se);
    cplx v[E];
#pragma unroll
    for (int q = 0; q < E; ++q) {
        const bool on = valid && PL::slot_in(q) && PL::lane_in(j, q);
        if (INV) v[q] = on ? nt_load_c(buf + bpos(j + PL::cin(q))) : mkc(0.0, 0.0);
        else v[q] = on ? buf_load_c_aux<OFDFT_CPASS_LD_AUX>(ub + PL::cin(q) * se_u, voff) : mkc(0.0, 0.0);
    }
    line_fft<LEN, INV, kCX>(v, j, lds + l * PassCfg<LEN>::LSTR, tw);
    if (valid) {
#pragma unroll
        for (int q = 0; q < E; ++q) {
            if (!(PL::slot_out(q) && PL::lane_out(j, q))) continue;
            if (INV) buf_store_c_aux<OFDFT_CPASS_ST_AUX>(ub + PL::cout(q) * se_u, voff, v[q]);
            else nt_store_c(buf + bpos(j + PL::cout(q)), v[q]);
        }
    }
}

template <int M> struct ZCfg {
    static constexpr int P = Plan<M>::P;
    static constexpr int E = Plan<M>::E;
    static constexpr int TPB = (8 * P > 256) ? 8 * P : 256;
    static constexpr int RPW = TPB / P;
    static constexpr int RS = LineBuf<M>::STRIDE;
    static constexpr size_t LDS = sizeof(real) * RPW * RS;
};

struct PreIdentity {
    __device__ __forceinline__ real operator()(real a, long long) const { return a; }
};

template <int M, class Pre>
__global__ __launch_bounds__(ZCfg<M>::TPB) void zfwd_kernel(const real* __restrict__ in, cplx* __restrict__ spec,
                                                            SpecGeom g, const cplx* __restrict__ twM,
                                                            const cplx* __restrict__ twN, Pre pre) {
    constexpr int P = ZCfg<M>::P, E = ZCfg<M>::E, RPW = ZCfg<M>::RPW, RS = ZCfg<M>::RS, TPB = ZCfg<M>::TPB;
    constexpr int N2 = 2 * M;
    extern __shared__ __attribute__((aligned(16))) real lds[];
    const int tid = threadIdx.x;
    const int j = tid % P, r = tid / P;
    const long long row0 = (long long)blockIdx.x * RPW;
    const long long row = row0 + r;
    const bool valid = row < g.nrows;
    cplx v[E];
    if (valid) {
        const cplx* ub = reinterpret_cast<const cplx*>(in + row0 * N2);
        const unsigned voff = (unsigned)((r * M + j) * kCB);
#pragma unroll
        for (int q = 0; q < E; ++q) {
            const cplx t = buf_load_c(ub + q * P, voff);
            const long long e = row * N2 + 2 * (j + P * q);
            v[q] = mkc(pre(t.x, e), pre(t.y, e + 1));
        }
    } else {
#pragma unroll
        for (int q = 0; q < E; ++q) v[q] = mkc(0.0, 0.0);
    }
    real* mine = lds + r * RS;
    line_fft<M, false>(v, j, mine, twM);

    real cr_k[E], cr_m[E], c0r = 0.0, c0i = 0.0;
    __syncthreads();
#pragma unroll
    for (int q = 0; q < E; ++q) mine[lpad(j + P * q)] = v[q].x;
    __syncthreads();
#pragma unroll
    for (int it = 0; it < E; ++it) {
        const int idx = tid + it * TPB;
        const int kin = idx & 7, rr = (idx >> 3) % RPW, b = idx / (8 * RPW);
        const int k = 8 * b + kin, mk = (M - k) & (M - 1);
        cr_k[it] = lds[rr * RS + lpad(k)];
        cr_m[it] = lds[rr * RS + lpad(mk)];
    }
    if (tid < RPW) c0r = lds[tid * RS];
    __syncthreads();
#pragma unroll
    for (int q = 0; q < E; ++q) mine[lpad(j + P * q)] = v[q].y;
    __syncthreads();
#pragma unroll
    for (int it = 0; it < E; ++it) {
        const int idx = tid + it * TPB;
        const int kin = idx & 7, rr = (idx >> 3) % RPW, b = idx / (8 * RPW);
        const int k = 8 * b + kin, mk = (M - k) & (M - 1);
        const real ci_k = lds[rr * RS + lpad(k)];
        const real ci_m = lds[rr * RS + lpad(mk)];
        const cplx ev = mkc(0.5 * (cr_k[it] + cr_m[it]), 0.5 * (ci_k - ci_m));
// ... 408 lines not shown
```

professad_amd/csrc/lines.hip:

```cpp
#include "engine_ctx.h"

namespace eng {

template <int LEN, bool INV>
int launch_cpass_t(ofdft_ctx* c, const ArrList& arrs, int narr, const LineMap& main, const LineMap& rem, hipStream_t st,
                   const char* nm) {
    cplx* tw;
    if (int rc = get_twiddle(c, LEN, &tw)) return rc;
    using Cfg = PassCfg<LEN>;
    LineMap mm = main;
    mm.blk0 = main.blk0 / Cfg::LPW;
    constexpr int T = OFDFT_CPASS_TILES;
    const int mb = ((main.nlines - main.blk0 + Cfg::LPW - 1) / Cfg::LPW + T - 1) / T * T, rb = (rem.nlines + Cfg::LPW - 1) / Cfg::LPW;
    OFDFT_LAUNCH(c, st, nm, (cpass_kernel<LEN, INV>), dim3((mb + rb + T - 1) / T, narr), dim3(Cfg::TPB), Cfg::LDS, arrs, mm, rem, mb,
                 c->g.main_count, tw);
    return 0;
}

void pass_maps(const ofdft_ctx* c, int axis, LineMap& main, LineMap& rem) {
    const SpecGeom& g = axis == 0 ? c->gx : c->g;
    const int nb = g.nzm / 8, nrem = g.nzc - g.nzm;
    if (axis == 0) {
        main.d = g.n1 * 8; main.sb = (long long)g.n0 * g.n1 * 8; main.sl = 1; main.se = (long long)g.n1 * 8;
        main.nlines = nb * g.n1 * 8; main.lf = 0;
// ... 403 lines not shown
        int x, yl, kz;
        spec_decode(gx, i, x, yl, kz);
        const long long r = (long long)x * xg.arr_sz +
                            (kz < gx.nzm ? (((long long)(kz >> 3) * xg.nyl + yl) * 8 + (kz & 7))
                                         : ((long long)xg.nb * xg.nyl * 8 + (long long)(kz - gx.nzm) * xg.nyl + yl));
        if (pack) const_cast<cplx*>(buf)[r] = spec[i];
        else spec[i] = buf[r];
    }
}
static int dist_rfftn(ofdft_ctx* c, const real* in, cplx* spec, hipStream_t st);
static int dist_irfftn(ofdft_ctx* c, cplx* spec, real* out, double scale, hipStream_t st);

static bool bluestein_ok_fwd(const ofdft_ctx* c);
int rfftn_internal_multi(ofdft_ctx* c, const real* const* in, cplx* const* spec, int n, hipStream_t st) {
    if (n > 1 && n <= kBsBatch && c->nranks == 1 && !c->fast && bluestein_ok_fwd(c)) {
        BsIo io{};
        for (int a = 0; a < n; ++a) {
            io.spec[a] = spec[a];
            io.rin[a] = in[a];
        }
        c->fft_count += n;
        if (int rc = bluestein_pass_multi(c, 1, 2, 0, io, n, 1.0, st)) return rc;
        if (int rc = bluestein_pass_multi(c, 0, 1, 0, io, n, 1.0, st)) return rc;
        return bluestein_pass_multi(c, 0, 0, 0, io, n, 1.0, st);
    }
    for (int a = 0; a < n; ++a)
        if (int rc = rfftn_internal(c, in[a], spec[a], st)) return rc;
    return 0;
}
int irfftn_internal_multi(ofdft_ctx* c, cplx* const* spec, real* const* out, int n, double scale, hipStream_t st) {
    if (n > 1 && n <= kBsBatch && c->nranks == 1 && !c->fast && bluestein_ok_fwd(c)) {
        BsIo io{};
        for (int a = 0; a < n; ++a) {
            io.spec[a] = spec[a];
            io.rout[a] = out[a];
        }
        c->fft_count += n;
        if (int rc = bluestein_pass_multi(c, 0, 0, 1, io, n, 1.0, st)) return rc;
        if (int rc = bluestein_pass_multi(c, 0, 1, 1, io, n, 1.0, st)) return rc;
        return bluestein_pass_multi(c, 2, 2, 1, io, n, scale, st);
    }
    for (int a = 0; a < n; ++a)
        if (int rc = irfftn_internal(c, spec[a], out[a], scale, st)) return rc;
    return 0;
}

int rfftn_internal(ofdft_ctx* c, const real* in, cplx* spec, hipStream_t st) {
    c->fft_count++;
    if (c->nranks > 1) return dist_rfftn(c, in, spec, st);
    if (c->fast) {
        int rc = zfwd_any(c, in, spec, st);
        if (rc) return rc;
        if ((rc = fast_axis_pass<false>(c, 1, spec, st))) return rc;
        return fast_axis_pass<false>(c, 0, spec, st);
    }
    if (bluestein_ok(c)) {
        if (int rc = bluestein_pass(c, 1, 2, 0, spec, in, nullptr, 1.0, st)) return rc;
        if (int rc = bluestein_pass(c, 0, 1, 0, spec, nullptr, nullptr, 1.0, st)) return rc;
        return bluestein_pass(c, 0, 0, 0, spec, nullptr, nullptr, 1.0, st);
    }
    cplx *tw2, *tmp;
    if (int rc = get_twiddle(c, c->n2, &tw2)) return rc;
    if (int rc = spec_ws(c, "gen_tmp", &tmp)) return rc;
    OFDFT_LAUNCH(c, st, "gen_r2c_z", gen_r2c_z_kernel, dim3((unsigned)((c->g.total + 255) / 256)), dim3(256), 0, in, spec, c->g, tw2);
    cplx *cur = spec, *other = tmp;
    if (int rc = gen_axis(c, 1, 0, cur, other, st)) return rc;
    if (int rc = gen_axis(c, 0, 0, cur, other, st)) return rc;
    if (cur != spec) HIP_TRY(c, hipMemcpyAsync(spec, cur, sizeof(cplx) * c->g.total, hipMemcpyDeviceToDevice, st));
    return 0;
}

int irfftn_internal(ofdft_ctx* c, cplx* spec, real* out, double scale, hipStream_t st) {
    c->fft_count++;
    if (c->nranks > 1) return dist_irfftn(c, spec, out, scale, st);
    if (c->fast) {
        int rc;
        if ((rc = fast_axis_pass<true>(c, 0, spec, st))) return rc;
        if ((rc = fast_axis_pass<true>(c, 1, spec, st))) return rc;
        return zinv_any(c, spec, out, scale, st);
    }
    if (bluestein_ok(c)) {
        if (int rc = bluestein_pass(c, 0, 0, 1, spec, nullptr, nullptr, 1.0, st)) return rc;
        if (int rc = bluestein_pass(c, 0, 1, 1, spec, nullptr, nullptr, 1.0, st)) return rc;
        return bluestein_pass(c, 2, 2, 1, spec, nullptr, out, scale, st);
    }
    cplx *tw2, *tmp;
    if (int rc = get_twiddle(c, c->n2, &tw2)) return rc;
    if (int rc = spec_ws(c, "gen_tmp", &tmp)) return rc;
    cplx *cur = spec, *other = tmp;
    if (int rc = gen_axis(c, 0, 1, cur, other, st)) return rc;
    if (int rc = gen_axis(c, 1, 1, cur, other, st)) return rc;
    PostScale post{(real)scale};
    OFDFT_LAUNCH(c, st, "gen_c2r_z", (gen_c2r_z_kernel<PostScale>), dim3((unsigned)((c->npts + 255) / 256)), dim3(256), 0, cur, out,
                       c->g, tw2, post);
    return 0;
}


int fwd_zy(ofdft_ctx* c, const real* in, cplx* spec, hipStream_t st) {
    c->fft_count++;
    int rc = zfwd_any(c, in, spec, st);
    if (rc) return rc;
    return fast_axis_pass<false>(c, 1, spec, st);
}

int inv_yz(ofdft_ctx* c, cplx* spec, real* out, double scale, hipStream_t st) {
    c->fft_count++;
    if (int rc = fast_axis_pass<true>(c, 1, spec, st)) return rc;
    return zinv_any(c, spec, out, scale, st);
}

static int dist_rfftn(ofdft_ctx* c, const real* in, cplx* spec, hipStream_t st) {
    cplx *send, *recv, *tmp;
    if (int rc = dist_buffers(c, 0, &send, &recv)) return rc;
    if (int rc = spec_ws(c, "x:tmp", &tmp)) return rc;
    int rc = zfwd_any(c, in, tmp, st);
    if (rc) return rc;
    if ((rc = ypass_xchg<false>(c, {tmp}, send, st, kWholeXchg))) return rc;
    if ((rc = dist_exchange(c, send, recv, st))) return rc;
    XchgGeom xg = c->xg;
    xg.rec = xg.arr_sz;
    OFDFT_LAUNCH(c, st, "xchg_unpack", xchg_unpack_kernel, dim3(grid_for(c->gx.total)), dim3(256), 0, (const cplx*)recv, spec, c->gx, xg, 0);
    return fast_axis_pass<false>(c, 0, spec, st);
}

static int dist_irfftn(ofdft_ctx* c, cplx* spec, real* out, double scale, hipStream_t st) {
    cplx *send, *recv, *tmp;
    if (int rc = dist_buffers(c, 0, &send, &recv)) return rc;
    if (int rc = spec_ws(c, "x:tmp", &tmp)) return rc;
    int rc;
    if ((rc = fast_axis_pass<true>(c, 0, spec, st))) return rc;
    XchgGeom xg = c->xg;
    xg.rec = xg.arr_sz;
    OFDFT_LAUNCH(c, st, "xchg_pack", xchg_unpack_kernel, dim3(grid_for(c->gx.total)), dim3(256), 0, (const cplx*)send, spec, c->gx, xg, 1);
    if ((rc = dist_exchange(c, send, recv, st))) return rc;
    if ((rc = ypass_xchg<true>(c, {tmp}, recv, st, kWholeXchg))) return rc;
    return zinv_any(c, tmp, out, scale, st);
}


template <int LEN>
int launch_yderiv_t(ofdft_ctx* c, const cplx* in, cplx* out, double scale, hipStream_t st, cplx* fwd) {
    cplx* tw;
    if (int rc = get_twiddle(c, LEN, &tw)) return rc;
    using Cfg = PassCfg<LEN>;
    LineMap main, rem;
    pass_maps(c, 1, main, rem);
    const int mb = (main.nlines + Cfg::LPW - 1) / Cfg::LPW, rb = (rem.nlines + Cfg::LPW - 1) / Cfg::LPW;
    OFDFT_LAUNCH(c, st, "yderiv", (yderiv_kernel<LEN>), dim3(mb + rb), dim3(Cfg::TPB), Cfg::LDS, in, out, main, rem, mb,
                 c->g.main_count, (const cplx*)tw, (real)scale, fwd);
    if (fwd) c->fft_passes_fused++, c->yfwd_fused++;
    return 0;
}
int yderiv(ofdft_ctx* c, const cplx* in, cplx* out, double scale, hipStream_t st, cplx* fwd) {
    switch (c->n1) {
        case 8: return launch_yderiv_t<8>(c, in, out, scale, st, fwd);
        case 16: return launch_yderiv_t<16>(c, in, out, scale, st, fwd);
        case 32: return launch_yderiv_t<32>(c, in, out, scale, st, fwd);
        case 64: return launch_yderiv_t<64>(c, in, out, scale, st, fwd);
        case 128: return launch_yderiv_t<128>(c, in, out, scale, st, fwd);
        case 256: return launch_yderiv_t<256>(c, in, out, scale, st, fwd);
        case 512: return launch_yderiv_t<512>(c, in, out, scale, st, fwd);
        case 1024: return launch_yderiv_t<1024>(c, in, out, scale, st, fwd);
#define X(L) case L: return launch_yderiv_t<L>(c, in, out, scale, st, fwd);
        OFDFT_MIXED_LINES(X)
#undef X
    }
    return fail(c, OFDFT_EINVAL, "unsupported fast FFT length %d", c->n1);
}


template int fast_axis_pass_multi<false>(ofdft_ctx*, int, cplx* const*, int, hipStream_t, int, int, int, int);
template int fast_axis_pass_multi<true>(ofdft_ctx*, int, cplx* const*, int, hipStream_t, int, int, int, int);
template int fast_axis_pass<false>(ofdft_ctx*, int, cplx*, hipStream_t);
template int fast_axis_pass<true>(ofdft_ctx*, int, cplx*, hipStream_t);
template int ypass_xchg<false>(ofdft_ctx*, const std::vector<cplx*>&, cplx*, hipStream_t, int);
template int ypass_xchg<true>(ofdft_ctx*, const std::vector<cplx*>&, cplx*, hipStream_t, int);

}
```

professad_amd/csrc/pointwise_kernels.h:

```cpp
#pragma once
#include <type_traits>

#include "fastmath.h"
#include "fft_kernels.h"

namespace ofdft {

constexpr double kPi = (double)3.14159265358979323846264338327950288L;
constexpr double kFiveThirds = (double)5 / 3, kFiveSixths = (double)5 / 6;
constexpr real kPiR = (real)kPi;
constexpr real kThird = (real)(1.0L / 3.0L);
constexpr real kCbrt9Pi4 = (real)9.570780000627306053141655531512398907L;
constexpr real kCbrt3OverPi = (real)0.984745021842696541178973376907781690L;
constexpr real kCrs = (real)0.620350490899400016668006812047778167L;
constexpr real kSqrtCrs = (real)0.787623317899743250528011536241166179L;
constexpr real kInvSqrtCrs = (real)1.269642451250142171583074982042715431L;
constexpr real kCbrtPiOver3 = (real)1.015491297563259267239386001491459489L;
constexpr real kPbeGamma = (real)0.031090690869654895034940863712730629L;
constexpr real kPbeInvGamma = (real)32.16396844291482112072009037084516073L;
constexpr real kLn2 = (real)0.693147180559945309417232121458176568L;
constexpr real kCtf = (real)(0.3L * 9.570780000627306053141655531512398907L);
constexpr real kCs2 = (real)(0.25L / 9.570780000627306053141655531512398907L);
constexpr real kCx = (real)(-0.75L * 0.984745021842696541178973376907781690L);
constexpr int kRedBlocks = 1024;
// ... 269 lines not shown
    if (z < tm.nzm)
        for (k = 0; k < tm.nch - 1 && b >= tm.kb[k + 1]; ++k) {}
    const int kb0 = tm.kb[k], nbk = tm.kb[k + 1] - kb0;
    const long long arr = ((long long)nbk * 8 + (k == tm.nch - 1 ? tm.nrem : 0)) * tm.nyl;
    const long long base = (long long)tm.n0g * tm.nyl * 8 * kb0;
    const long long in = z < tm.nzm ? (((long long)(b - kb0) * tm.nyl + y) * 8 + (z & 7))
                                    : ((long long)nbk * 8 * tm.nyl + (long long)(z - tm.nzm) * tm.nyl + y);
    return base + x * arr + in;
}

template <bool THIRD>
__device__ __forceinline__ void wgc_series(double eta, const WgcSeries& s, double& w0, double& w1, double& w2, double& w3) {
    const bool inner = eta <= 1.0;
    const bool on = (s.u >= 0.0) ? inner : !inner;
    const double C1 = on ? s.c1 : 0.0, C2 = on ? s.c2 : 0.0;
    const double le = log(eta);
    double H0, H1, H2, H3 = 0.0;
    if (s.v > 0.0) {
        const double rv = sqrt(s.v), x = s.u + rv, y = s.u - rv;
        const double px = pow(eta, x - 2.0), py = pow(eta, y - 2.0);
        H0 = (C1 * px + C2 * py) * eta * eta;
        H1 = (C1 * x * px + C2 * y * py) * eta;
        H2 = C1 * x * (x - 1.0) * px + C2 * y * (y - 1.0) * py;
        if (THIRD) H3 = (C1 * x * (x - 1.0) * (x - 2.0) * px + C2 * y * (y - 1.0) * (y - 2.0) * py) / eta;
    } else if (s.v == 0.0) {
        const double pu2 = pow(eta, s.u - 2.0), pu1 = pu2 * eta, pu = pu1 * eta;
        H0 = pu * (C2 * le + C1);
        H1 = C2 * pu1 * (1.0 + s.u * le) + C1 * s.u * pu1;
        H2 = C2 * ((s.u - 1.0) * pu2 * (1.0 + s.u * le) + pu2) + C1 * s.u * (s.u - 1.0) * pu2;
        if (THIRD) {
            const double a3 = s.u * (s.u - 1.0) * (s.u - 2.0), b3 = 3.0 * s.u * s.u - 6.0 * s.u + 2.0;
            H3 = pu2 / eta * (C2 * (a3 * le + b3) + C1 * a3);
        }
    } else {
        const double rv = sqrt(-s.v);
        const double tc = cos(rv * le), ts = sin(rv * le);
        const double p = s.u * tc - rv * ts, q = s.u * ts + rv * tc;
        const double pu2 = pow(eta, s.u - 2.0), pu1 = pu2 * eta, pu = pu1 * eta;
        H0 = pu * (C1 * tc + C2 * ts);
        H1 = pu1 * (C1 * p + C2 * q);
        H2 = pu2 * ((s.u - 1.0) * (C1 * p + C2 * q) + rv * (C2 * p - C1 * q));
        if (THIRD) {
            const double zr = s.u, zi = rv;
            double ar = zr * (zr - 1.0) - zi * zi, ai = zi * (2.0 * zr - 1.0);
            const double br = ar * (zr - 2.0) - ai * zi, bi = ar * zi + ai * (zr - 2.0);
            const double dr = C1 * br + C2 * bi, di = C1 * bi - C2 * br;
            H3 = pu2 / eta * (dr * tc - di * ts);
        }
    }
    const double x = inner ? eta * eta : 1.0 / (eta * eta);
    double P0 = 0.0, P1 = 0.0, P2 = 0.0, P3 = 0.0;
    for (int t = s.nt - 1; t >= 0; --t) {
        const double ti = 2.0 * t;
        const double c = inner ? s.cb[t] : s.ca[t];
        const double d1 = inner ? ti * c : -ti * c;
        const double d2 = inner ? ti * (ti - 1.0) * c : ti * (ti + 1.0) * c;
        P0 = P0 * x + c;
        P1 = P1 * x + d1;
        P2 = P2 * x + d2;
        if (THIRD) P3 = P3 * x + (inner ? ti * (ti - 1.0) * (ti - 2.0) * c : -ti * (ti + 1.0) * (ti + 2.0) * c);
    }
    P1 /= eta;
    P2 /= eta * eta;
    w0 = H0 + P0;
    w1 = H1 + P1;
    w2 = H2 + P2;
    w3 = THIRD ? H3 + P3 / (eta * eta * eta) : 0.0;
}

static __global__ void wgc_table_kernel(cplx* __restrict__ t01, real* __restrict__ t2, KGeom kg, WgcSeries s, TabMap tm) {
    for (long long ii = (long long)blockIdx.x * blockDim.x + threadIdx.x; ii < kg.g.total; ii += (long long)gridDim.x * blockDim.x) {
        real kx, ky, kz, k2;
        kvec(kg, ii, kx, ky, kz, k2);
        long long i = ii;
        if (tm.on) {
            int x, y, z;
            spec_decode(kg.g, ii, x, y, z);
            i = tabmap_index(tm, x, y, z);
        }
        const double eta = (k2 != 0.0) ? sqrt((double)k2) * s.inv2kf : 0.0;
        double w0 = 0.0, w1 = 0.0, w2 = 0.0, w3;
        if (eta != 0.0) wgc_series<false>(eta, s, w0, w1, w2, w3);
        w0 *= s.pref;
        w1 *= s.pref;
        w2 *= s.pref;
        t01[i] = mkc((real)w0, (real)(-eta * w1 / (6.0 * s.nref)));
        t2[i] = (real)((eta * eta * w2 + (7.0 - s.gamma) * eta * w1) / (36.0 * s.nref * s.nref));
    }
}

__device__ __forceinline__ void kvec_xyz(const KGeom& kg, int x, int y, int z, real& kx, real& ky, real& kz,
                                         real& k2) {
    const real fa = ifreq(x, kg.g.n0), fb = ifreq(y + kg.y0, kg.n1g), fc = (real)z;
    kx = fa * kg.b[0] + fb * kg.b[3] + fc * kg.b[6];
    ky = fa * kg.b[1] + fb * kg.b[4] + fc * kg.b[7];
    kz = fa * kg.b[2] + fb * kg.b[5] + fc * kg.b[8];
    k2 = kx * kx + ky * ky + kz * kz;
}

template <bool HAS_H, bool HAS_G> struct MixDensity {
    KGeom kg;
    static __device__ __forceinline__ constexpr bool imag(int o) { return HAS_H ? o >= 1 : true; }
    template <int O, int I> static __device__ __forceinline__ constexpr bool present() { return true; }
    template <int O, int I> static __device__ __forceinline__ constexpr bool imag_oi() { return imag(O); }
    template <int O, int I>
    __device__ __forceinline__ real coef(int x, int y, int z, long long, unsigned) const {
        real kx, ky, kz, k2;
        kvec_xyz(kg, x, y, z, kx, ky, kz, k2);
        if (HAS_H && O == 0) return (k2 != 0.0) ? 4.0 * kPiR / k2 : 0.0;
        constexpr int c = O - (HAS_H ? 1 : 0);
        return c == 0 ? kx : (c == 1 ? ky : kz);
    }
};

template <bool HAS_H, bool HAS_L = false> struct MixDensityA {
    KGeom kg;
    static __device__ __forceinline__ constexpr bool imag(int o) { return o == (HAS_H ? 1 : 0); }
    template <int O, int I> static __device__ __forceinline__ constexpr bool present() { return true; }
    template <int O, int I> static __device__ __forceinline__ constexpr bool imag_oi() { return imag(O); }
    template <int O, int I>
    __device__ __forceinline__ real coef(int x, int y, int z, long long, unsigned) const {
        if constexpr (O == (HAS_H ? 1 : 0)) {
            return ifreq(x, kg.g.n0);
        } else {
            real kx, ky, kz, k2;
            kvec_xyz(kg, x, y, z, kx, ky, kz, k2);
            if (HAS_H && O == 0) return (k2 != 0.0) ? 4.0 * kPiR / k2 : 0.0;
            return -k2;
        }
    }
};
struct MixDerivA {
    KGeom kg;
    static __device__ __forceinline__ constexpr bool imag(int) { return true; }
    template <int O, int I> static __device__ __forceinline__ constexpr bool present() { return true; }
    template <int O, int I> static __device__ __forceinline__ constexpr bool imag_oi() { return true; }
    template <int O, int I>
    __device__ __forceinline__ real coef(int x, int, int, long long, unsigned) const { return ifreq(x, kg.g.n0); }
};
struct MixDerivAL {
    KGeom kg;
    static __device__ __forceinline__ constexpr bool imag(int) { return true; }
    template <int O, int I> static __device__ __forceinline__ constexpr bool present() { return true; }
    template <int O, int I> static __device__ __forceinline__ constexpr bool imag_oi() { return I == 0; }
    template <int O, int I>
    __device__ __forceinline__ real coef(int x, int y, int z, long long, unsigned) const {
        if constexpr (I == 0) {
            return ifreq(x, kg.g.n0);
        } else {
            real kx, ky, kz, k2;
            kvec_xyz(kg, x, y, z, kx, ky, kz, k2);
            return 0.5 * k2;
        }
    }
};

template <int OP> struct MixScale {
    KGeom kg;
    real p0, p1;
    static __device__ __forceinline__ constexpr bool imag(int) { return false; }
    template <int O, int I> static __device__ __forceinline__ constexpr bool present() { return true; }
    template <int O, int I> static __device__ __forceinline__ constexpr bool imag_oi() { return imag(O); }
    template <int O, int I>
    __device__ __forceinline__ real coef(int x, int y, int z, long long, unsigned) const {
        real kx, ky, kz, k2;
        kvec_xyz(kg, x, y, z, kx, ky, kz, k2);
        if (OP == SPEC_HARTREE) return (k2 != 0.0) ? 4.0 * kPiR / k2 : 0.0;
        if (OP == SPEC_LAPLACE) return -k2;
        return p0 * lindhard_shape((k2 != 0.0) ? sqrt(k2) * p1 : 0.0);
    }
};

struct MixDiv {
    KGeom kg;
    static __device__ __forceinline__ constexpr bool imag(int) { return true; }
    template <int O, int I> static __device__ __forceinline__ constexpr bool present() { return true; }
    template <int O, int I> static __device__ __forceinline__ constexpr bool imag_oi() { return imag(O); }
    template <int O, int I>
    __device__ __forceinline__ real coef(int x, int y, int z, long long, unsigned) const {
        real kx, ky, kz, k2;
        kvec_xyz(kg, x, y, z, kx, ky, kz, k2);
        return I == 0 ? kx : (I == 1 ? ky : kz);
    }
};

struct MixWgc {
    static constexpr bool kTables = true;
    const cplx* t01;
    const real* t2;
    real ck;
    static __device__ __forceinline__ constexpr bool imag(int) { return false; }
    template <int O, int I> static __device__ __forceinline__ constexpr bool present() { return O + I <= 2; }
    template <int O, int I> static __device__ __forceinline__ constexpr bool imag_oi() { return false; }
    template <int O, int I>
    __device__ __forceinline__ real coef(int, int, int, long long uoff, unsigned loff) const {
        if constexpr (O + I <= 1) {
            const cplx pr = buf_load_c(t01 + uoff, loff * (unsigned)sizeof(cplx));
            return (O + I == 0) ? pr.x : pr.y;
        } else {
            const real k2 = buf_load_d(t2 + uoff, loff * (unsigned)sizeof(real));
            if constexpr (O == 1) {
                const cplx pr = buf_load_c(t01 + uoff, loff * (unsigned)sizeof(cplx));
                return k2 + ck * pr.y;
            } else {
                return k2;
            }
        }
    }
    static constexpr int kTableReals = 3;
    __device__ __forceinline__ void fetch(real (&cf)[3], long long uoff, unsigned loff, bool valid) const {
#ifdef OFDFT_WGC_TABLE_PROBE
        cf[0] = (real)1.0; cf[1] = (real)0.5; cf[2] = valid ? (real)0.25 : (real)0.0;
        (void)uoff; (void)loff;
#else
        const cplx p0 = valid ? buf_load_c(t01 + uoff, loff * (unsigned)sizeof(cplx)) : mkc(0.0, 0.0);
        const real k2 = valid ? buf_load_d(t2 + uoff, loff * (unsigned)sizeof(real)) : (real)0.0;
        cf[0] = p0.x; cf[1] = p0.y; cf[2] = k2;
#endif
    }
    __device__ __forceinline__ void apply(cplx (&o)[3], const cplx (&in)[3], const real (&cf)[3]) const {
        const real k3 = cf[2] + ck * cf[1];
        o[0] = mkc(cf[0] * in[0].x + cf[1] * in[1].x + cf[2] * in[2].x, cf[0] * in[0].y + cf[1] * in[1].y + cf[2] * in[2].y);
        o[1] = mkc(cf[1] * in[0].x + k3 * in[1].x, cf[1] * in[0].y + k3 * in[1].y);
        o[2] = mkc(cf[2] * in[0].x, cf[2] * in[0].y);
    }
};

struct MixWgcFold : MixWgc {
    int fold_n0;
};

__device__ __forceinline__ void pw92(real rs, real& eps, real& deps_drs) {
    const real A = 0.0310907, a1 = 0.2137, b1 = 7.5957, b2 = 3.5876, b3 = 1.6382, b4 = 0.49294;
    const real sr = sqrt(rs);
    const real zeta = 2.0 * A * (b1 * sr + b2 * rs + b3 * rs * sr + b4 * rs * rs);
    const real izeta = 1.0 / zeta;
    const real lg = log(1.0 + izeta);
    eps = -2.0 * A * (1.0 + a1 * rs) * lg;
    const real dzeta = 2.0 * A * (0.5 * b1 / sr + b2 + 1.5 * b3 * sr + 2.0 * b4 * rs);
    deps_drs = -2.0 * A * a1 * lg + 2.0 * A * (1.0 + a1 * rs) * dzeta * izeta / (zeta + 1.0);
}
__device__ __forceinline__ void pw92_roots(real sr, real isr, real& eps, real& deps_drs) {
    const real A = 0.0310907, a1 = 0.2137, b1 = 7.5957, b2 = 3.5876, b3 = 1.6382, b4 = 0.49294;
    const real rs = sr * sr;
    const real zeta = 2.0 * A * (sr * (b1 + sr * (b2 + sr * (b3 + sr * b4))));
    const real zp1 = zeta + 1.0;
    const real iz2 = fm::rcp(zeta * zp1);
    const real lg = fm::log(zp1 * zp1 * iz2);
    const real pre = 2.0 * A * (1.0 + a1 * rs);
    eps = -pre * lg;
    const real dzeta = 2.0 * A * (0.5 * b1 * isr + b2 + 1.5 * b3 * sr + 2.0 * b4 * rs);
    deps_drs = -2.0 * A * a1 * lg + pre * dzeta * iz2;
}

struct XcLocal { real ex, vx, ec, vc; };

__device__ __forceinline__ XcLocal lda_point(real n, unsigned mask, const fm::Roots<real>& q) {
    XcLocal r = {0.0, 0.0, 0.0, 0.0};
    const real n13 = q.n13;
    if (mask & (1u << 6)) {
        r.ex = kCx * n13 * n;
        r.vx = (4.0 / 3.0) * kCx * n13;
    }
    if (mask & ((1u << 7) | (1u << 8) | (1u << 9))) {
        const real rs = kCrs * q.inv13;
        if (mask & (1u << 7)) {
            const real gm = -0.1423, b1 = 1.0529, b2 = 0.3334, A = 0.0311, B = -0.048, C = 0.002, D = -0.0116;
            real eps, v;
            if (rs < 1.0) {
                const real lr = fm::log(rs);
                eps = A * lr + B + C * rs * lr + D * rs;
                v = lr * (A + (2.0 / 3.0) * C * rs) + (B - A / 3.0) + rs * ((2.0 * D - C) / 3.0);
            } else {
                const real sr = kSqrtCrs * q.y, iden = fm::rcp(1.0 + b1 * sr + b2 * rs);
                eps = gm * iden;
                v = gm * (1.0 + (7.0 / 6.0) * b1 * sr + (4.0 / 3.0) * b2 * rs) * iden * iden;
            }
            r.ec += eps * n;
            r.vc += v;
        }
        if (mask & (1u << 8)) {
            real eps, d;
            pw92_roots(kSqrtCrs * q.y, kInvSqrtCrs * (n * q.inv13 * q.inv13 * q.y), eps, d);
            r.ec += eps * n;
            r.vc += eps - rs * kThird * d;
        }
        if (mask & (1u << 9)) {
            const real a = (kLn2 - 1.0) / (2.0 * kPiR * kPiR), b = 20.4562557;
            const real irs = fm::rcp(rs);
            const real arg = 1.0 + b * irs + b * irs * irs;
            const real eps = a * fm::log(arg);
            const real d = a * fm::rcp(arg) * (-b * irs * irs - 2.0 * b * irs * irs * irs);
            r.ec += eps * n;
            r.vc += eps - rs * kThird * d;
        }
    }
    return r;
}

__device__ __forceinline__ XcLocal lda_point(real n, unsigned mask) { return lda_point(n, mask, fm::roots(n)); }

struct PbePoint { real fx, fc, fk, dfdn, dfdg; };
struct GgaSel { int x, c, k, kkind; real kmu, kbeta, klambda, ksigma; };
constexpr int kPbeScalars = 3;

__device__ __forceinline__ PbePoint pbe_point(real n, real gn2, const GgaSel& sel) {
// ... 364 lines not shown
```

professad_amd/csrc/xcross.h:

```cpp
#pragma once
#include "xwave.h"

namespace ofdft {

#ifndef OFDFT_XC_A512
#define OFDFT_XC_A512 8
#endif
template <int LEN> struct XcWaves { static constexpr int A = 4; };
#ifndef OFDFT_XC_A256
#ifdef OFDFT_REAL_F32
#define OFDFT_XC_A256 4
#else
#define OFDFT_XC_A256 4
#endif
#endif
template <> struct XcWaves<256> { static constexpr int A = OFDFT_XC_A256; };
template <> struct XcWaves<512> { static constexpr int A = OFDFT_XC_A512; };
template <> struct XcWaves<1024> { static constexpr int A = 8; };

#ifndef OFDFT_XC_NL_F32
#define OFDFT_XC_NL_F32 2
#endif
template <int LEN> struct XcCfg {
    static constexpr int A = XcWaves<LEN>::A;
// ... 51 lines not shown
    } else {
        o[0] = buf_load_c_aux<AUX>(ubase, voff_bytes);
        o[1] = buf_load_c_aux<AUX>(ubase + 1, voff_bytes);
    }
}
template <int NL, int AUX> __device__ __forceinline__ void buf_store_cn(cplx* ubase, unsigned voff_bytes, const cplx (&v)[NL]) {
    if constexpr (NL == 1) {
        buf_store_c_aux<AUX>(ubase, voff_bytes, v[0]);
    } else if constexpr (sizeof(cplx) == 8) {
        u32x4 t;
        *reinterpret_cast<cplx*>(&t) = v[0];
        *(reinterpret_cast<cplx*>(&t) + 1) = v[1];
        __builtin_amdgcn_raw_buffer_store_b128(t, make_rsrc(ubase), (int)voff_bytes, 0, AUX);
    } else {
        buf_store_c_aux<AUX>(ubase, voff_bytes, v[0]);
        buf_store_c_aux<AUX>(ubase + 1, voff_bytes, v[1]);
    }
}

template <int LEN, int NIN, int NOUT, class Mix>
__global__ __launch_bounds__(XcCfg<LEN>::TPB, (xc_waves<LEN, NIN, NOUT>())) void xc_kernel(XfIo io, LineMap m_main, LineMap m_rem, int main_blocks,
                                                                              SpecGeom g, const cplx* __restrict__ tw_g, Mix mix,
                                                                              XfStride xs) {
    using Cfg = XcCfg<LEN>;
    constexpr int A = Cfg::A, S = Cfg::S, E = Cfg::E, LPWV = Cfg::LPWV, LPB = Cfg::LPB, PP = Cfg::PP, RR = Cfg::RR,
                  TPB = Cfg::TPB, WREG = Cfg::WREG, WPT = Cfg::WPT, NL = Cfg::NL, G = NIN > NOUT ? NIN : NOUT;
    constexpr int LDA = (LPB * sizeof(cplx) >= 128) ? OFDFT_XC_LD_AUX : 0;
    constexpr int STA = (LPB * sizeof(cplx) >= 128) ? OFDFT_XC_ST_AUX : OFDFT_XC_ST_AUX_HALF;
    extern __shared__ __attribute__((aligned(16))) real lds[];
    constexpr bool ONEBUF = xc_one_buffer<LEN, NIN, NOUT>();
    cplx* xb = reinterpret_cast<cplx*>(lds);
    cplx* twN = xb + (ONEBUF ? 1 : 2) * Cfg::XB;
    cplx* twS = twN + Cfg::TWN;
    const int t = threadIdx.x;
    const int lane = t & 63;
    const int a = __builtin_amdgcn_readfirstlane(t >> 6);
    const int l = lane % LPWV;
    const int j = lane / LPWV;
    const int J = t / LPWV;
    constexpr int TWC = (Cfg::TWN + TPB - 1) / TPB;
    cplx twr[TWC];
#pragma unroll
    for (int c = 0; c < TWC; ++c) {
        const int i = t + c * TPB;
        twr[c] = tw_g[i < Cfg::TWN ? i : 0];
    }
    const cplx tws = tw_g[(t < S ? t : 0) * A];
    const bool is_rem = (int)blockIdx.x >= main_blocks;
    const LineMap m = is_rem ? m_rem : m_main;
    int bid = is_rem ? (int)blockIdx.x - main_blocks : (int)blockIdx.x;
    if (LPB * sizeof(cplx) < 128 && !is_rem && bid < (main_blocks & ~15)) {
        bid = (bid & ~15) + ((bid & 7) << 1) + ((bid >> 3) & 1);
    }
    if (!is_rem) bid += m.blk0;
    const long long L0 = (long long)bid * LPB;
    const long long L = L0 + NL * l;
    const bool valid = L < m.nlines;
    const long long base = valid ? (L / m.d) * m.sb + (L % m.d) * (long long)m.sl : 0;
    int y[NL], kz[NL];
#pragma unroll
    for (int nl = 0; nl < NL; ++nl) {
        const long long Ln = L + nl;
        if (is_rem) {
            y[nl] = (int)(Ln % g.n1);
            kz[nl] = g.nzm + (int)(Ln / g.n1);
        } else {
            const int c = (int)(Ln % m.d);
            y[nl] = c >> 3;
            kz[nl] = m.kz0 + (int)(Ln / m.d) * 8 + (c & 7);
        }
    }
    const long long region = is_rem ? g.main_count : 0;
    const long long lb0 = line_base(m, L0);
    const long long b0 = uniform64(region + lb0);
    const long long se_o = xs.se_out ? xs.se_out : m.se, se_t = xs.tse ? xs.tse : m.se;
    const int xa = A * j + a;
    const unsigned voff = valid ? (unsigned)((base - lb0 + (long long)xa * m.se) * kCB) : 0u;
    const unsigned voff_o = valid ? (unsigned)((base - lb0 + (long long)xa * se_o) * kCB) : 0u;
    const unsigned tloff = valid ? (unsigned)(base - lb0 + (long long)J * se_t) : 0u;
    const unsigned tl0 = valid ? (unsigned)(base - lb0) : 0u;
    const long long qstep = uniform64((long long)PP * m.se), qstep_o = uniform64((long long)PP * se_o),
                    tqstep = uniform64((long long)PP * se_t);

    cplx v[G][NL][E];
    static_for<NIN>([&](auto ic) {
        constexpr int I = decltype(ic)::value;
        const cplx* ub = io.in[I] + b0;
#pragma unroll
        for (int q = 0; q < E; ++q) {
            cplx pr[NL];
            if (valid) {
                buf_load_cn<NL, LDA>(pr, ub + q * qstep, voff);
            } else {
#pragma unroll
                for (int nl = 0; nl < NL; ++nl) pr[nl] = mkc(0.0, 0.0);
            }
#pragma unroll
            for (int nl = 0; nl < NL; ++nl) v[I][nl][q] = pr[nl];
        }
    });
    constexpr int NC = OFDFT_XW_PREFETCH ? mix_coef_count<Mix>::N : 0;
    real cfs[NL][E][NC > 0 ? NC : 1];
    if constexpr (NC > 0) {
#pragma unroll
        for (int nl = 0; nl < NL; ++nl)
#pragma unroll
            for (int q = 0; q < E; ++q) {
                if constexpr (mix_has_fold<Mix>::value) {
                    const int xq = J + PP * q, xf = 2 * xq > mix.fold_n0 ? mix.fold_n0 - xq : xq;
                    mix.fetch(cfs[nl][q], b0, tl0 + nl + (unsigned)xf * (unsigned)se_t, valid);
                } else {
                    mix.fetch(cfs[nl][q], b0 + q * tqstep, tloff + nl, valid);
                }
            }
    }
#pragma unroll
    for (int c = 0; c < TWC; ++c) {
        const int i = t + c * TPB;
        if (i < Cfg::TWN) twN[i] = twr[c];
    }
    if (t < S) twS[t] = tws;
    __syncthreads();
    const int lx = (l * XwSwz<S>::LMUL) & 31;
    static_for<NIN>([&](auto ic) {
        constexpr int I = decltype(ic)::value;
        cplx* buf = ONEBUF ? xb : xb + (I & 1) * Cfg::XB;
        if constexpr (ONEBUF && I > 0) __syncthreads();
#pragma unroll
        for (int nl = 0; nl < NL; ++nl) {
            real* mine = reinterpret_cast<real*>(buf + a * WREG) + (nl * LPWV + l) * Cfg::RS;
            xw_line_fft<S, false>(v[I][nl], j, mine, twS, lx);
        }
        exchange_sync<true>();
#pragma unroll
        for (int nl = 0; nl < NL; ++nl)
#pragma unroll
            for (int q = 0; q < E; ++q) buf[a * WREG + nl * WPT + lane + 64 * q] = v[I][nl][q];
        __syncthreads();
#pragma unroll
        for (int nl = 0; nl < NL; ++nl)
#pragma unroll
            for (int r = 0; r < RR; ++r) {
                const int bp = J + PP * r;
                cplx c[A];
#pragma unroll
                for (int aa = 0; aa < A; ++aa) c[aa] = buf[aa * WREG + nl * WPT + t + TPB * r];
#pragma unroll
                for (int aa = 1; aa < A; ++aa) c[aa] = cmul(c[aa], twN[aa * bp]);
                Dft<A, false>::run(c);
#pragma unroll
                for (int ap = 0; ap < A; ++ap) v[I][nl][r + RR * ap] = c[ap];
            }
    });
#pragma unroll
    for (int nl = 0; nl < NL; ++nl)
#pragma unroll
        for (int q = 0; q < E; ++q) {
            cplx in[NIN], out[NOUT];
#pragma unroll
            for (int I = 0; I < NIN; ++I) in[I] = v[I][nl][q];
            if constexpr (NC > 0) mix.apply(out, in, cfs[nl][q]);
            else xw_outputs<NIN, NOUT, 0, Mix>(out, in, mix, J + PP * q, y[nl], kz[nl], b0 + q * tqstep, tloff + nl);
#pragma unroll
            for (int O = 0; O < NOUT; ++O) v[O][nl][q] = out[O];
        }
    static_for<NOUT>([&](auto oc) {
        constexpr int O = decltype(oc)::value;
        cplx* buf = ONEBUF ? xb : xb + ((NIN + O) & 1) * Cfg::XB;
        if constexpr (ONEBUF) __syncthreads();
#pragma unroll
        for (int nl = 0; nl < NL; ++nl)
#pragma unroll
            for (int r = 0; r < RR; ++r) {
                const int bp = J + PP * r;
                cplx c[A];
#pragma unroll
                for (int ap = 0; ap < A; ++ap) c[ap] = v[O][nl][r + RR * ap];
                Dft<A, true>::run(c);
#pragma unroll
                for (int aa = 1; aa < A; ++aa) c[aa] = cmul(c[aa], cconj(twN[aa * bp]));
#pragma unroll
                for (int aa = 0; aa < A; ++aa) buf[aa * WREG + nl * WPT + t + TPB * r] = c[aa];
            }
        __syncthreads();
#pragma unroll
        for (int nl = 0; nl < NL; ++nl)
#pragma unroll
            for (int q = 0; q < E; ++q) v[O][nl][q] = buf[a * WREG + nl * WPT + lane + 64 * q];
        exchange_sync<true>();
#pragma unroll
        for (int nl = 0; nl < NL; ++nl) {
            real* mine = reinterpret_cast<real*>(buf + a * WREG) + (nl * LPWV + l) * Cfg::RS;
            xw_line_fft<S, true>(v[O][nl], j, mine, twS, lx);
        }
        exchange_sync<true>();
        if (valid) {
            cplx* ub = io.out[O] + b0;
#pragma unroll
            for (int q = 0; q < E; ++q) {
                cplx pr[NL];
#pragma unroll
                for (int nl = 0; nl < NL; ++nl) pr[nl] = v[O][nl][q];
                if (xs.se_out) buf_store_cn<NL, 0>(ub + q * qstep_o, voff_o, pr);
                else buf_store_cn<NL, STA>(ub + q * qstep_o, voff_o, pr);
            }
        }
    });
}

}
```

professad_amd/csrc/xpass_a.hip:

```cpp
#include "xpass_impl.h"

namespace eng {
template int xfused<3, 3, MixWgc>(ofdft_ctx*, const XfIo&, const MixWgc&, hipStream_t, const char*, const XfLayout&);
template int xfused<1, 1, MixScale<SPEC_LAPLACE>>(ofdft_ctx*, const XfIo&, const MixScale<SPEC_LAPLACE>&, hipStream_t, const char*, const XfLayout&);
template int xfused<1, 1, MixScale<SPEC_LINDHARD>>(ofdft_ctx*, const XfIo&, const MixScale<SPEC_LINDHARD>&, hipStream_t, const char*, const XfLayout&);
template int xfused<1, 1, MixDerivA>(ofdft_ctx*, const XfIo&, const MixDerivA&, hipStream_t, const char*, const XfLayout&);
template int xfused<2, 1, MixDerivAL>(ofdft_ctx*, const XfIo&, const MixDerivAL&, hipStream_t, const char*, const XfLayout&);
template int xfused<3, 1, MixDiv>(ofdft_ctx*, const XfIo&, const MixDiv&, hipStream_t, const char*, const XfLayout&);
}
```

professad_amd/csrc/xpass_impl.h:

```cpp
#pragma once
#include "engine_ctx.h"
#include "xcross.h"

namespace eng {

template <int LEN, int NIN, int NOUT, class Mix>
int launch_xfused_t(ofdft_ctx* c, const XfIo& io, const Mix& mix, const XfLayout& lay, hipStream_t st, const char* nm) {
    constexpr int G = NIN > NOUT ? NIN : NOUT;
    using Cfg = XfCfg<LEN, G, NOUT>;
    cplx* tw;
    if (int rc = get_twiddle(c, LEN, &tw)) return rc;
    LineMap main, rem;
    SpecGeom gk = c->gx;
    if (lay.se_in) {
        const int nyl = c->xg.nyl;
        const int xnb = lay.xnb >= 0 ? lay.xnb : c->xg.nb, xnrem = lay.xnb >= 0 ? lay.xnrem : c->xg.nrem;
        main.d = nyl * 8; main.sb = nyl * 8; main.sl = 1; main.se = lay.se_in; main.nlines = xnb * nyl * 8;
        main.kz0 = lay.kz0;
        rem.d = nyl; rem.sb = nyl; rem.sl = 1; rem.se = lay.se_in; rem.nlines = xnrem * nyl;
        if (main.nlines == 0) main.d = 1;
        if (rem.nlines == 0) rem.d = 1;
        gk.main_count = (long long)xnb * nyl * 8;
    } else {
        pass_maps(c, 0, main, rem);
    }
    main.lf = rem.lf = Cfg::LPW;
    int line0 = 0;
    if (lay.kb1 > lay.kb0 && !lay.se_in) {
        const int per_block = c->gx.n1 * 8;
        line0 = lay.kb0 * per_block;
        main.nlines = lay.kb1 * per_block;
        if (lay.kb1 != c->gx.nzm / 8) rem.nlines = 0;
    }
    main.blk0 = line0 / Cfg::LPW;
    const int mb = (main.nlines - line0 + Cfg::LPW - 1) / Cfg::LPW, rb = (rem.nlines + Cfg::LPW - 1) / Cfg::LPW;
    c->xpass_kinds |= OFDFT_XPASS_GROUP;
    OFDFT_LAUNCH(c, st, nm, (xfused_kernel<LEN, NIN, NOUT, Mix>), dim3(mb + rb), dim3(Cfg::TPB), Cfg::LDS, io, main, rem, mb,
                 gk, tw, mix, XfStride{lay.se_out, lay.tse});
    return 0;
}

template <int LEN, int NIN, int NOUT, class Mix>
int launch_xw_t(ofdft_ctx* c, const XfIo& io, const Mix& mix, const XfLayout& lay, hipStream_t st, const char* nm) {
    using Cfg = XwCfg<LEN>;
    cplx* tw;
    if (int rc = get_twiddle(c, LEN, &tw)) return rc;
    LineMap main, rem;
    SpecGeom gk = c->gx;
    if (lay.se_in) {
        const int nyl = c->xg.nyl;
        const int xnb = lay.xnb >= 0 ? lay.xnb : c->xg.nb, xnrem = lay.xnb >= 0 ? lay.xnrem : c->xg.nrem;
        main.d = nyl * 8; main.sb = nyl * 8; main.sl = 1; main.se = lay.se_in; main.nlines = xnb * nyl * 8;
        main.kz0 = lay.kz0;
        rem.d = nyl; rem.sb = nyl; rem.sl = 1; rem.se = lay.se_in; rem.nlines = xnrem * nyl;
        if (main.nlines == 0) main.d = 1;
        if (rem.nlines == 0) rem.d = 1;
        gk.main_count = (long long)xnb * nyl * 8;
    } else {
        pass_maps(c, 0, main, rem);
    }
    main.lf = rem.lf = Cfg::LPB;
    int line0 = 0;
    if (lay.kb1 > lay.kb0 && !lay.se_in) {
        const int per_block = c->gx.n1 * 8;
        if (per_block % Cfg::LPB) return fail(c, OFDFT_EINVAL, "kz-range x pass needs whole workgroups per kz block");
        line0 = lay.kb0 * per_block;
        main.nlines = lay.kb1 * per_block;
        if (lay.kb1 != c->gx.nzm / 8) rem.nlines = 0;
    }
    main.blk0 = line0 / Cfg::LPB;
    const int mb = (main.nlines - line0 + Cfg::LPB - 1) / Cfg::LPB, rb = (rem.nlines + Cfg::LPB - 1) / Cfg::LPB;
    c->xpass_kinds |= OFDFT_XPASS_WAVE;
    OFDFT_LAUNCH(c, st, nm, (xw_kernel<LEN, NIN, NOUT, Mix>), dim3(mb + rb), dim3(Cfg::TPB), Cfg::LDS, io, main, rem, mb, gk,
                 (const cplx*)tw, mix, XfStride{lay.se_out, lay.tse});
    return 0;
}

template <int LEN, int NIN, int NOUT, class Mix>
int launch_xc_t(ofdft_ctx* c, const XfIo& io, const Mix& mix, const XfLayout& lay, hipStream_t st, const char* nm) {
    using Cfg = XcCfg<LEN>;
    cplx* tw;
    if (int rc = get_twiddle(c, LEN, &tw)) return rc;
    LineMap main, rem;
    SpecGeom gk = c->gx;
    if (lay.se_in) {
        const int nyl = c->xg.nyl;
        const int xnb = lay.xnb >= 0 ? lay.xnb : c->xg.nb, xnrem = lay.xnb >= 0 ? lay.xnrem : c->xg.nrem;
        main.d = nyl * 8; main.sb = nyl * 8; main.sl = 1; main.se = lay.se_in; main.nlines = xnb * nyl * 8;
        main.kz0 = lay.kz0;
        rem.d = nyl; rem.sb = nyl; rem.sl = 1; rem.se = lay.se_in; rem.nlines = xnrem * nyl;
        if (main.nlines == 0) main.d = 1;
        if (rem.nlines == 0) rem.d = 1;
        gk.main_count = (long long)xnb * nyl * 8;
    } else {
        pass_maps(c, 0, main, rem);
    }
    main.lf = rem.lf = Cfg::LPB;
    if constexpr (Cfg::NL > 1) {
        if (main.sl != 1 || rem.sl != 1 || main.d % Cfg::NL || rem.d % Cfg::NL || main.nlines % Cfg::NL || rem.nlines % Cfg::NL)
        {
            if constexpr (LEN <= 512) return launch_xw_t<LEN, NIN, NOUT, Mix>(c, io, mix, lay, st, nm);
            else return launch_xfused_t<LEN, NIN, NOUT, Mix>(c, io, mix, lay, st, nm);
        }
    }
    int line0 = 0;
    if (lay.kb1 > lay.kb0 && !lay.se_in) {
        const int per_block = c->gx.n1 * 8;
        if (per_block % Cfg::LPB) return fail(c, OFDFT_EINVAL, "kz-range x pass needs whole workgroups per kz block");
        line0 = lay.kb0 * per_block;
        main.nlines = lay.kb1 * per_block;
        if (lay.kb1 != c->gx.nzm / 8) rem.nlines = 0;
    }
    main.blk0 = line0 / Cfg::LPB;
    const int mb = (main.nlines - line0 + Cfg::LPB - 1) / Cfg::LPB, rb = (rem.nlines + Cfg::LPB - 1) / Cfg::LPB;
    constexpr size_t lds = Cfg::lds_bytes(xc_one_buffer<LEN, NIN, NOUT>());
    if constexpr (lds > 64 * 1024) {
        static bool declared[64] = {};
        const int dv = c->device & 63;
        if (!declared[dv]) {
            HIP_TRY(c, hipFuncSetAttribute(reinterpret_cast<const void*>(&xc_kernel<LEN, NIN, NOUT, Mix>),
                                           hipFuncAttributeMaxDynamicSharedMemorySize, (int)lds));
            declared[dv] = true;
        }
    }
    c->xpass_kinds |= Cfg::NL == 2 ? OFDFT_XPASS_CROSS2 : OFDFT_XPASS_CROSS1;
    OFDFT_LAUNCH(c, st, nm, (xc_kernel<LEN, NIN, NOUT, Mix>), dim3(mb + rb), dim3(Cfg::TPB), lds, io, main, rem, mb, gk,
                 (const cplx*)tw, mix, XfStride{lay.se_out, lay.tse});
    return 0;
}

template <int NIN, int NOUT> bool xc_serves(const ofdft_ctx* c) {
    constexpr bool xc_1024_f32 = sizeof(real) == 4;
    const bool xc_len = (c->n0g == 256 && !(sizeof(real) == 4 && NIN + NOUT == 2)) || c->n0g == 512;
    const bool len_ok = c->n0g == 128 || c->n0g == 256 || c->n0g == 512 || c->n0g == 1024;
    return len_ok && (c->use_xwave == 5 || (c->use_xwave == 6 && NIN + NOUT >= 3) ||
                      (c->use_xwave == 1 && (xc_len || (c->n0g == 1024 && (NIN + NOUT >= 3 || xc_1024_f32)))));
}

template <int NIN, int NOUT, class Mix>
int xfused(ofdft_ctx* c, const XfIo& io, const Mix& mix, hipStream_t st, const char* nm, const XfLayout& lay) {
    if (xc_serves<NIN, NOUT>(c)) {
        switch (c->n0g) {
            case 128: return launch_xc_t<128, NIN, NOUT, Mix>(c, io, mix, lay, st, nm);
            case 256: return launch_xc_t<256, NIN, NOUT, Mix>(c, io, mix, lay, st, nm);
            case 512: return launch_xc_t<512, NIN, NOUT, Mix>(c, io, mix, lay, st, nm);
            case 1024: return launch_xc_t<1024, NIN, NOUT, Mix>(c, io, mix, lay, st, nm);
        }
    }
    if (c->use_xwave == 2 || ((c->use_xwave == 1 || c->use_xwave >= 5 || (c->use_xwave == 4 && c->n0g < 512)) && NIN + NOUT >= 3)) {
        switch (c->n0g) {
            case 8: return launch_xw_t<8, NIN, NOUT, Mix>(c, io, mix, lay, st, nm);
            case 16: return launch_xw_t<16, NIN, NOUT, Mix>(c, io, mix, lay, st, nm);
            case 32: return launch_xw_t<32, NIN, NOUT, Mix>(c, io, mix, lay, st, nm);
            case 64: return launch_xw_t<64, NIN, NOUT, Mix>(c, io, mix, lay, st, nm);
            case 128: return launch_xw_t<128, NIN, NOUT, Mix>(c, io, mix, lay, st, nm);
            case 256: return launch_xw_t<256, NIN, NOUT, Mix>(c, io, mix, lay, st, nm);
            case 512: return launch_xw_t<512, NIN, NOUT, Mix>(c, io, mix, lay, st, nm);
        }
    }
    switch (c->n0g) {
        case 8: return launch_xfused_t<8, NIN, NOUT, Mix>(c, io, mix, lay, st, nm);
        case 16: return launch_xfused_t<16, NIN, NOUT, Mix>(c, io, mix, lay, st, nm);
        case 32: return launch_xfused_t<32, NIN, NOUT, Mix>(c, io, mix, lay, st, nm);
        case 64: return launch_xfused_t<64, NIN, NOUT, Mix>(c, io, mix, lay, st, nm);
        case 128: return launch_xfused_t<128, NIN, NOUT, Mix>(c, io, mix, lay, st, nm);
        case 256: return launch_xfused_t<256, NIN, NOUT, Mix>(c, io, mix, lay, st, nm);
        case 512: return launch_xfused_t<512, NIN, NOUT, Mix>(c, io, mix, lay, st, nm);
        case 1024: return launch_xfused_t<1024, NIN, NOUT, Mix>(c, io, mix, lay, st, nm);
#define X(L) case L: return launch_xfused_t<L, NIN, NOUT, Mix>(c, io, mix, lay, st, nm);
        OFDFT_MIXED_LINES(X)
#undef X
    }
    return fail(c, OFDFT_EINVAL, "unsupported fast FFT length %d", c->n0g);
}

}
```

professad_amd/csrc/xwave.h:

```cpp
#pragma once
#include "fft_kernels.h"

namespace ofdft {

#ifndef OFDFT_XW_SWIZZLE
#define OFDFT_XW_SWIZZLE 1
#endif
template <int LEN> struct XwSwz { static constexpr int XS = 0, XM = 0, XMUL = 0, LMUL = 0, RS = LineBuf<LEN>::STRIDE; };
#if OFDFT_XW_SWIZZLE
#if defined(OFDFT_REAL_F32) && !OFDFT_F32_CX
template <> struct XwSwz<32> { static constexpr int XS = 3, XM = 1, XMUL = 1, LMUL = 0, RS = 34; };
template <> struct XwSwz<64> { static constexpr int XS = 3, XM = 3, XMUL = 1, LMUL = 0, RS = 68; };
template <> struct XwSwz<128> { static constexpr int XS = 3, XM = 7, XMUL = 1, LMUL = 0, RS = 136; };
template <> struct XwSwz<256> { static constexpr int XS = 3, XM = 15, XMUL = 1, LMUL = 0, RS = 272; };
template <> struct XwSwz<512> { static constexpr int XS = 3, XM = 31, XMUL = 1, LMUL = 0, RS = 512; };
#else
template <> struct XwSwz<32> { static constexpr int XS = 1, XM = 1, XMUL = 1, LMUL = 1, RS = 48; };
template <> struct XwSwz<64> { static constexpr int XS = 1, XM = 1, XMUL = 1, LMUL = 1, RS = 72; };
template <> struct XwSwz<128> { static constexpr int XS = 1, XM = 15, XMUL = 1, LMUL = 5, RS = 144; };
template <> struct XwSwz<256> { static constexpr int XS = 3, XM = 7, XMUL = 1, LMUL = 8, RS = 272; };
template <> struct XwSwz<512> { static constexpr int XS = 3, XM = 15, XMUL = 1, LMUL = 0, RS = 512; };
#endif
#endif
template <int LEN> struct XwPlan : ZPlan<LEN, 8> {};
template <int LEN> struct LdsLayout<XwPlan<LEN>> : LdsLayoutDefault {
    static constexpr int XS = XwSwz<LEN>::XS, XM = XwSwz<LEN>::XM, XMUL = XwSwz<LEN>::XMUL;
};
template <int LEN, bool INV>
__device__ __forceinline__ void xw_line_fft(cplx (&v)[8], int j, real* line, const cplx* __restrict__ tw, int lx) {
    StageP<XwPlan<LEN>, 0, 1, INV, true, false, kCX>::run(v, j, line, tw, lx);
}

template <int LEN> struct XwCfg {
    static constexpr int E = 8;
    using PL = ZPlan<LEN, E>;
    static constexpr int P = LEN / E;
    static constexpr int LPWV = 64 / P;
#ifndef OFDFT_XW_TPB512
#define OFDFT_XW_TPB512 0
#endif
#ifdef OFDFT_XW_TPB
    static constexpr int TPB = OFDFT_XW_TPB;
#else
    static constexpr int TPB = (P == 64 && OFDFT_XW_TPB512) ? 512 : 256;
#endif
    static constexpr int LPB = LPWV * (TPB / 64);
    static constexpr int RS = kCXMul * XwSwz<LEN>::RS;
    static constexpr int ROWS = LPB * RS;
    static constexpr size_t LDS = sizeof(real) * ROWS + sizeof(cplx) * LEN;
};

template <class Mix, class = void> struct mix_has_fold : std::false_type {};
template <class Mix> struct mix_has_fold<Mix, std::void_t<decltype(std::declval<const Mix&>().fold_n0)>> : std::true_type {};
template <class Mix, class = void> struct mix_coef_count { static constexpr int N = 0; };
template <class Mix> struct mix_coef_count<Mix, std::void_t<decltype(Mix::kTableReals)>> { static constexpr int N = Mix::kTableReals; };

template <int NIN, int NOUT, int O, int I, class Mix>
__device__ __forceinline__ void xw_accumulate(real& acr, real& aci, const cplx (&in)[NIN], const Mix& mix, int x, int y, int kz,
                                              long long uoff, unsigned loff) {
    if constexpr (I < NIN) {
        if constexpr (Mix::template present<O, I>()) {
            const real cf = mix.template coef<O, I>(x, y, kz, uoff, loff);
            if constexpr (Mix::template imag_oi<O, I>()) {
                acr -= cf * in[I].y;
                aci += cf * in[I].x;
            } else {
                acr += cf * in[I].x;
                aci += cf * in[I].y;
            }
        }
        xw_accumulate<NIN, NOUT, O, I + 1, Mix>(acr, aci, in, mix, x, y, kz, uoff, loff);
    }
}
template <int NIN, int NOUT, int O, class Mix>
__device__ __forceinline__ void xw_outputs(cplx (&out)[NOUT], const cplx (&in)[NIN], const Mix& mix, int x, int y, int kz,
                                           long long uoff, unsigned loff) {
    if constexpr (O < NOUT) {
        real acr = 0.0, aci = 0.0;
        xw_accumulate<NIN, NOUT, O, 0, Mix>(acr, aci, in, mix, x, y, kz, uoff, loff);
        out[O] = mkc(acr, aci);
        xw_outputs<NIN, NOUT, O + 1, Mix>(out, in, mix, x, y, kz, uoff, loff);
    }
}

#ifndef OFDFT_XW_WAVES
#define OFDFT_XW_WAVES 2
#endif
#ifndef OFDFT_XW_LD_AUX
#define OFDFT_XW_LD_AUX 0
#endif
#ifndef OFDFT_XW_ST_AUX
#define OFDFT_XW_ST_AUX 0
#endif

template <int LEN, int NIN, int NOUT, class Mix>
__global__ __launch_bounds__(XwCfg<LEN>::TPB, (NIN + NOUT > 3 ? OFDFT_XW_WAVES : 3)) void xw_kernel(XfIo io, LineMap m_main, LineMap m_rem,
                                                                                     int main_blocks, SpecGeom g,
                                                                                     const cplx* __restrict__ tw_g, Mix mix,
                                                                                     XfStride xs) {
    using Cfg = XwCfg<LEN>;
    constexpr int E = Cfg::E, P = Cfg::P, LPWV = Cfg::LPWV, LPB = Cfg::LPB, G = NIN > NOUT ? NIN : NOUT;
    extern __shared__ __attribute__((aligned(16))) real lds[];
    const int lane = threadIdx.x & 63;
    const int wave = __builtin_amdgcn_readfirstlane((int)(threadIdx.x >> 6));
    const int l = lane % LPWV;
    const int j = lane / LPWV;
    constexpr int TWC = (LEN + Cfg::TPB - 1) / Cfg::TPB;
    cplx twr[TWC];
#pragma unroll
    for (int c = 0; c < TWC; ++c) {
        const int i = threadIdx.x + c * Cfg::TPB;
        twr[c] = tw_g[i < LEN ? i : 0];
    }
    const bool is_rem = (int)blockIdx.x >= main_blocks;
    const LineMap m = is_rem ? m_rem : m_main;
    int bid = is_rem ? (int)blockIdx.x - main_blocks : (int)blockIdx.x;
    if (LPB * sizeof(cplx) < 128 && !is_rem && bid < (main_blocks & ~15)) {
        bid = (bid & ~15) + ((bid & 7) << 1) + ((bid >> 3) & 1);
    }
    if (!is_rem) bid += m.blk0;
    const long long L0 = (long long)bid * LPB;
    const long long L = L0 + wave * LPWV + l;
    const bool valid = L < m.nlines;
    const long long base = valid ? (L / m.d) * m.sb + (L % m.d) * (long long)m.sl : 0;
    int y, kz;
    if (is_rem) {
        y = (int)(L % g.n1);
        kz = g.nzm + (int)(L / g.n1);
    } else {
        const int c = (int)(L % m.d);
        y = c >> 3;
        kz = m.kz0 + (int)(L / m.d) * 8 + (c & 7);
    }
    const long long region = is_rem ? g.main_count : 0;
    const long long lb0 = line_base(m, L0);
    const long long b0 = uniform64(region + lb0);
    const long long se_o = xs.se_out ? xs.se_out : m.se, se_t = xs.tse ? xs.tse : m.se;
    const unsigned voff = valid ? (unsigned)((base - lb0 + (long long)j * m.se) * kCB) : 0u;
    const unsigned voff_o = valid ? (unsigned)((base - lb0 + (long long)j * se_o) * kCB) : 0u;
    const unsigned tloff = valid ? (unsigned)(base - lb0 + (long long)j * se_t) : 0u;
    const long long qstep = uniform64((long long)P * m.se), qstep_o = uniform64((long long)P * se_o),
                    tqstep = uniform64((long long)P * se_t);

    cplx a[G][E];
    static_for<NIN>([&](auto ic) {
        constexpr int I = decltype(ic)::value;
        const cplx* ub = io.in[I] + b0;
#pragma unroll
        for (int q = 0; q < E; ++q) a[I][q] = valid ? buf_load_c_aux<OFDFT_XW_LD_AUX>(ub + q * qstep, voff) : mkc(0.0, 0.0);
    });
#ifndef OFDFT_XW_PREFETCH
#define OFDFT_XW_PREFETCH 1
#endif
    constexpr int NC = OFDFT_XW_PREFETCH ? mix_coef_count<Mix>::N : 0;
    real cfs[E][NC > 0 ? NC : 1];
    if constexpr (NC > 0) {
#pragma unroll
        for (int q = 0; q < E; ++q) mix.fetch(cfs[q], b0 + q * tqstep, tloff, valid);
    }
    cplx* tw = reinterpret_cast<cplx*>(lds + Cfg::ROWS);
#pragma unroll
    for (int c = 0; c < TWC; ++c) {
        const int i = threadIdx.x + c * Cfg::TPB;
        if (i < LEN) tw[i] = twr[c];
    }
    __syncthreads();
    real* mine = lds + (wave * LPWV + l) * Cfg::RS;
    const int lx = (l * XwSwz<LEN>::LMUL) & 31;
    static_for<NIN>([&](auto ic) {
        constexpr int I = decltype(ic)::value;
        xw_line_fft<LEN, false>(a[I], j, mine, tw, lx);
        exchange_sync<true>();
    });
#pragma unroll
    for (int q = 0; q < E; ++q) {
        cplx in[NIN], out[NOUT];
#pragma unroll
        for (int I = 0; I < NIN; ++I) in[I] = a[I][q];
        if constexpr (NC > 0) mix.apply(out, in, cfs[q]);
        else xw_outputs<NIN, NOUT, 0, Mix>(out, in, mix, j + P * q, y, kz, b0 + q * tqstep, tloff);
#pragma unroll
        for (int O = 0; O < NOUT; ++O) a[O][q] = out[O];
    }
    static_for<NOUT>([&](auto oc) {
        constexpr int O = decltype(oc)::value;
        xw_line_fft<LEN, true>(a[O], j, mine, tw, lx);
        exchange_sync<true>();
        if (valid) {
            cplx* ub = io.out[O] + b0;
#pragma unroll
            for (int q = 0; q < E; ++q) {
                if (xs.se_out) buf_store_c(ub + q * qstep_o, voff_o, a[O][q]);
                else buf_store_c_aux<OFDFT_XW_ST_AUX>(ub + q * qstep_o, voff_o, a[O][q]);
            }
        }
    });
}

}
```

professad_amd/csrc/zpass.h:

```cpp
#pragma once
#include "pointwise_kernels.h"

namespace ofdft {

#ifndef OFDFT_ZPBE_WAVES
#define OFDFT_ZPBE_WAVES 2
#endif
#ifndef OFDFT_ZIWGC_WAVES
#define OFDFT_ZIWGC_WAVES 2
#endif
#ifndef OFDFT_Z_PREFETCH
#define OFDFT_Z_PREFETCH 1
#endif
#ifndef OFDFT_Z_PIPE_BIG_F32
#define OFDFT_Z_PIPE_BIG_F32 0
#endif
#ifndef OFDFT_ZI_ROOTS_ONCE
#define OFDFT_ZI_ROOTS_ONCE 0
#endif
#ifndef OFDFT_Z_LDS_TWIDDLES
#define OFDFT_Z_LDS_TWIDDLES 1
#endif

#ifndef OFDFT_Z_CX
// ... 482 lines not shown
    for (int q = 0; q < E; ++q) {
        __builtin_amdgcn_sched_barrier(0);
        const real ax = a[q].x * inv_n, bx = b[q].x * inv_n, cx = c[q].x * inv_n;
        const real ay = a[q].y * inv_n, by = b[q].y * inv_n, cy = c[q].y * inv_n;
        PbePoint p0 = {0, 0, 0, 0, 0}, p1 = {0, 0, 0, 0, 0};
        if (z.valid && ZW<M, E>::PL::slot_out(q) && ZW<M, E>::PL::lane_out(z.j, q)) {
            p0 = pbe_point(ds(n[q].x), ax * ax + bx * bx + cx * cx, sel);
            p1 = pbe_point(ds(n[q].y), ay * ay + by * by + cy * cy, sel);
        }
        acc[0] += p0.fx + p1.fx;
        acc[1] += p0.fc + p1.fc;
        acc[2] += p0.fk + p1.fk;
        d[q] = mkc(p0.dfdn, p1.dfdn);
        a[q] = mkc(p0.dfdg * ax, p1.dfdg * ay);
        b[q] = mkc(p0.dfdg * bx, p1.dfdg * by);
        c[q] = mkc(p0.dfdg * cx, p1.dfdg * cy);
    }
    z_store_real<M, E>(d, z, dfdn);
    using PL = typename ZW<M, E>::PL;
    repattern_out_to_in<PL, true>(a, z.j, z.mine);
    z_forward_store<M, E>(a, z, gx, g, twM, twN);
    repattern_out_to_in<PL, true>(b, z.j, z.mine);
    z_forward_store<M, E>(b, z, gy, g, twM, twN);
    repattern_out_to_in<PL, true>(c, z.j, z.mine);
    z_forward_store<M, E>(c, z, gz, g, twM, twN);
    block_reduce_store<kPbeScalars>(acc, partial + (long long)g.blk0 * kPbeScalars);
}

struct Bmat { real b[9]; };
#ifndef OFDFT_ZPBE_TWTAB
#define OFDFT_ZPBE_TWTAB 1
#endif
constexpr bool kZpbeTT = OFDFT_ZPBE_TWTAB != 0;
template <int M, int E, bool LAPL>
__global__ __launch_bounds__(256, (z_waves<M, E, OFDFT_Z_EMAX_PBE>(2))) void zpbe2_kernel(DenSrc ds, cplx* __restrict__ A, cplx* __restrict__ B,
                                                                      const real* __restrict__ dzn,
                                                                      real* __restrict__ dfdn, real inv_n, real inv_nz,
                                                                      GgaSel sel, Bmat bm, SpecGeom g,
                                                                      const cplx* __restrict__ twM_g,
                                                                      const cplx* __restrict__ twN_g,
                                                                      acc_t* __restrict__ partial, cplx* __restrict__ Lsp) {
    extern __shared__ __attribute__((aligned(16))) real lds[];
    const cplx *twM, *twN;
    const ZTwReq<M, E> twq = z_tw_request<M, E>(twM_g, twN_g);
    ds = ds.resolved();
    const ZLane<M, E> z(g, lds);
    cplx a[E], b[E], c[E], n[E];
    cplx lp[LAPL ? E : 1];
#if OFDFT_Z_PREFETCH
    {
        real nyq_a, nyq_b;
        z_issue_row<M, E>(a, nyq_a, z, A, g);
        z_issue_row<M, E>(b, nyq_b, z, B, g);
        z_tw_commit<M, E>(lds, twq, twM_g, twN_g, twM, twN);
        z_inverse_regs<M, E, kZpbeTT>(a, z, twM, twN, nyq_a);
        if constexpr (LAPL) {
            real nyq_l;
            z_issue_row<M, E>(lp, nyq_l, z, Lsp, g);
            z_inverse_regs<M, E, kZpbeTT>(b, z, twM, twN, nyq_b);
            z_inverse_regs<M, E, kZpbeTT>(lp, z, twM, twN, nyq_l);
        } else {
            z_inverse_regs<M, E, kZpbeTT>(b, z, twM, twN, nyq_b);
        }
    }
#else
    z_tw_commit<M, E>(lds, twq, twM_g, twN_g, twM, twN);
    z_load_inverse<M, E, kZpbeTT>(a, z, A, g, twM, twN);
    z_load_inverse<M, E, kZpbeTT>(b, z, B, g, twM, twN);
    if constexpr (LAPL) z_load_inverse<M, E, kZpbeTT>(lp, z, Lsp, g, twM, twN);
#endif
    z_load_real<M, E, true>(c, z, dzn);
    z_load_real<M, E, true>(n, z, ds.src);
    acc_t acc[kPbeScalars] = {0.0, 0.0, 0.0};
    cplx d[E];
    const bool diag = bm.b[1] == 0.0 && bm.b[2] == 0.0 && bm.b[3] == 0.0 && bm.b[5] == 0.0 && bm.b[6] == 0.0 && bm.b[7] == 0.0;
#pragma unroll
    for (int q = 0; q < E; ++q) {
        __builtin_amdgcn_sched_barrier(0);
        const real da0 = a[q].x * inv_n, db0 = b[q].x * inv_n, dc0 = c[q].x;
        const real da1 = a[q].y * inv_n, db1 = b[q].y * inv_n, dc1 = c[q].y;
        real gx0, gx1, gy0, gy1, gz0, gz1;
        if (diag) {
            gx0 = bm.b[0] * da0; gx1 = bm.b[0] * da1;
            gy0 = bm.b[4] * db0; gy1 = bm.b[4] * db1;
            gz0 = bm.b[8] * dc0; gz1 = bm.b[8] * dc1;
        } else {
            gx0 = bm.b[0] * da0 + bm.b[3] * db0 + bm.b[6] * dc0; gx1 = bm.b[0] * da1 + bm.b[3] * db1 + bm.b[6] * dc1;
            gy0 = bm.b[1] * da0 + bm.b[4] * db0 + bm.b[7] * dc0; gy1 = bm.b[1] * da1 + bm.b[4] * db1 + bm.b[7] * dc1;
            gz0 = bm.b[2] * da0 + bm.b[5] * db0 + bm.b[8] * dc0; gz1 = bm.b[2] * da1 + bm.b[5] * db1 + bm.b[8] * dc1;
        }
        PbePoint p0 = {0, 0, 0, 0, 0}, p1 = {0, 0, 0, 0, 0};
        if constexpr (LAPL) {
            real dl0 = 0.0, dl1 = 0.0;
            if (z.valid && ZW<M, E>::PL::slot_out(q) && ZW<M, E>::PL::lane_out(z.j, q)) {
                GgaSel nk = sel;
                nk.k = 0;
                const real g20 = gx0 * gx0 + gy0 * gy0 + gz0 * gz0, g21 = gx1 * gx1 + gy1 * gy1 + gz1 * gz1;
                p0 = pbe_point(ds(n[q].x), g20, nk);
                p1 = pbe_point(ds(n[q].y), g21, nk);
                pg_laplacian_point(ds(n[q].x), g20, lp[q].x * inv_n, sel, p0, dl0);
                pg_laplacian_point(ds(n[q].y), g21, lp[q].y * inv_n, sel, p1, dl1);
            }
            lp[q] = mkc(dl0, dl1);
        } else if (z.valid && ZW<M, E>::PL::slot_out(q) && ZW<M, E>::PL::lane_out(z.j, q)) {
            p0 = pbe_point(ds(n[q].x), gx0 * gx0 + gy0 * gy0 + gz0 * gz0, sel);
            p1 = pbe_point(ds(n[q].y), gx1 * gx1 + gy1 * gy1 + gz1 * gz1, sel);
        }
        acc[0] += p0.fx + p1.fx;
        acc[1] += p0.fc + p1.fc;
        acc[2] += p0.fk + p1.fk;
        d[q] = mkc(p0.dfdn, p1.dfdn);
        if (diag) {
            a[q] = mkc(p0.dfdg * (bm.b[0] * gx0), p1.dfdg * (bm.b[0] * gx1));
            b[q] = mkc(p0.dfdg * (bm.b[4] * gy0), p1.dfdg * (bm.b[4] * gy1));
            c[q] = mkc(p0.dfdg * (bm.b[8] * gz0), p1.dfdg * (bm.b[8] * gz1));
        } else {
            a[q] = mkc(p0.dfdg * (bm.b[0] * gx0 + bm.b[1] * gy0 + bm.b[2] * gz0),
                       p1.dfdg * (bm.b[0] * gx1 + bm.b[1] * gy1 + bm.b[2] * gz1));
            b[q] = mkc(p0.dfdg * (bm.b[3] * gx0 + bm.b[4] * gy0 + bm.b[5] * gz0),
                       p1.dfdg * (bm.b[3] * gx1 + bm.b[4] * gy1 + bm.b[5] * gz1));
            c[q] = mkc(p0.dfdg * (bm.b[6] * gx0 + bm.b[7] * gy0 + bm.b[8] * gz0),
                       p1.dfdg * (bm.b[6] * gx1 + bm.b[7] * gy1 + bm.b[8] * gz1));
        }
    }
    using PL = typename ZW<M, E>::PL;
    repattern_out_to_in<PL, true>(a, z.j, z.mine);
    z_forward_store<M, E, kZpbeTT>(a, z, A, g, twM, twN);
    repattern_out_to_in<PL, true>(b, z.j, z.mine);
    z_forward_store<M, E, kZpbeTT>(b, z, B, g, twM, twN);
    if constexpr (LAPL) {
        repattern_out_to_in<PL, true>(lp, z.j, z.mine);
        z_forward_store<M, E, kZpbeTT>(lp, z, Lsp, g, twM, twN);
    }
    repattern_out_to_in<PL, true>(c, z.j, z.mine);
    z_deriv_row<M, E, kZpbeTT>(c, z, twM, twN);
#pragma unroll
    for (int q = 0; q < E; ++q) d[q] = mkc(d[q].x - 2.0 * inv_nz * c[q].x, d[q].y - 2.0 * inv_nz * c[q].y);
    z_store_real<M, E>(d, z, dfdn);
    block_reduce_store<kPbeScalars>(acc, partial + (long long)g.blk0 * kPbeScalars);
}

struct ZCombineArgs {
    DenSrc ds;
    const real* vext;
    const real* dfdn;
    const cplx* vh;
    const cplx* lap;
    const cplx* conv_b;
    const cplx* conv_a;
    const cplx* u[3];
    const cplx* gw[3];
    const cplx* div;
    const cplx* div2;
    real* v_out;
    const real* v_part;
    int v_part_deferred;
    unsigned mask;
    real inv_n;
    real wt_alpha, wt_beta, wt_nbar_pa;
    real wgc_alpha, wgc_beta, nref;
    real gtf_inv_n0;
    int gtf_kind;
    int wt_is_56, wgc_sum_53;
    const acc_t* wts_w;
};

template <int M, int E>
__device__ __forceinline__ real wgc_row_section(const cplx (&n)[E], cplx (&vacc)[E], cplx (&w)[E], const ZLane<M, E>& z,
                                                  const ZCombineArgs& a, const SpecGeom& g, const cplx* __restrict__ twM,
                                                  const cplx* __restrict__ twN, real sc, real ctf) {
    cplx t1[E], t2[E];
    real e = 0.0;
#if OFDFT_Z_PREFETCH
    cplx nx[E];
    real nyq_nx, nyq_w;
    z_issue_row<M, E>(nx, nyq_nx, z, a.u[0], g);
#define OFDFT_ZROW(cur, nxt)                                                          \
    {                                                                                 \
        _Pragma("unroll") for (int q = 0; q < E; ++q) w[q] = nx[q];                   \
        nyq_w = nyq_nx;                                                               \
        if ((nxt) != nullptr) z_issue_row<M, E>(nx, nyq_nx, z, (nxt), g);             \
        z_inverse_regs<M, E>(w, z, twM, twN, nyq_w);                                  \
    }
#else
#define OFDFT_ZROW(cur, nxt) z_load_inverse<M, E>(w, z, (cur), g, twM, twN);
#endif
    OFDFT_ZROW(a.u[0], a.u[1])
#pragma unroll
    for (int q = 0; q < E; ++q) t1[q] = mkc(w[q].x * sc, w[q].y * sc);
    OFDFT_ZROW(a.u[1], a.u[2])
#pragma unroll
    for (int q = 0; q < E; ++q) {
        const real x0 = w[q].x * sc, x1 = w[q].y * sc;
        t1[q].x += (n[q].x - a.nref) * x0;
        t1[q].y += (n[q].y - a.nref) * x1;
        t2[q] = mkc(x0, x1);
    }
    OFDFT_ZROW(a.u[2], a.gw[0])
#pragma unroll
    for (int q = 0; q < E; ++q) {
        __builtin_amdgcn_sched_barrier(0);
        const real x0 = w[q].x * sc, x1 = w[q].y * sc;
        const real h0 = n[q].x - a.nref, h1 = n[q].y - a.nref;
        t1[q].x += 0.5 * h0 * h0 * x0;
        t1[q].y += 0.5 * h1 * h1 * x1;
        t2[q].x += h0 * x0;
        t2[q].y += h1 * x1;
        const real l0 = fm::log(n[q].x), l1 = fm::log(n[q].y);
        const real pb0 = fm::exp((a.wgc_beta - 1.0) * l0), pb1 = fm::exp((a.wgc_beta - 1.0) * l1);
        const real pa0 = fm::exp((a.wgc_alpha - 1.0) * l0), pa1 = fm::exp((a.wgc_alpha - 1.0) * l1);
        e += ctf * (pa0 * n[q].x * t1[q].x + pa1 * n[q].y * t1[q].y);
        vacc[q].x += ctf * pa0 * (a.wgc_alpha * t1[q].x + n[q].x * t2[q].x);
        vacc[q].y += ctf * pa1 * (a.wgc_alpha * t1[q].y + n[q].y * t2[q].y);
        t2[q] = mkc(pb0, pb1);
    }
    OFDFT_ZROW(a.gw[0], a.gw[1])
#pragma unroll
    for (int q = 0; q < E; ++q) t1[q] = mkc(a.wgc_beta * w[q].x * sc, a.wgc_beta * w[q].y * sc);
    OFDFT_ZROW(a.gw[1], a.gw[2])
#pragma unroll
    for (int q = 0; q < E; ++q) {
        t1[q].x += (a.wgc_beta * (n[q].x - a.nref) + n[q].x) * w[q].x * sc;
        t1[q].y += (a.wgc_beta * (n[q].y - a.nref) + n[q].y) * w[q].y * sc;
    }
    OFDFT_ZROW(a.gw[2], nullptr)
#pragma unroll
    for (int q = 0; q < E; ++q) {
        const real h0 = n[q].x - a.nref, h1 = n[q].y - a.nref;
        t1[q].x += (0.5 * a.wgc_beta * h0 * h0 + n[q].x * h0) * w[q].x * sc;
        t1[q].y += (0.5 * a.wgc_beta * h1 * h1 + n[q].y * h1) * w[q].y * sc;
        vacc[q].x += ctf * t2[q].x * t1[q].x;
        vacc[q].y += ctf * t2[q].y * t1[q].y;
    }
#undef OFDFT_ZROW
    return e;
}

constexpr int kParkIe = 0, kParkH = 1, kParkVw = 2, kParkWt = 3, kParkWgc = 4, kParkSlots = 5;
#ifndef OFDFT_ZI_WAVES_BIG_F32
#define OFDFT_ZI_WAVES_BIG_F32 4
#endif
template <int M, int E, bool WGC_INLINE> constexpr int zi_combine_waves() {
    if (sizeof(real) == 4 && M >= 512 && E <= 8 && !WGC_INLINE) return OFDFT_ZI_WAVES_BIG_F32;
    return z_waves<M, E>(2);
}
template <int M, int E, bool WGC_INLINE>
__global__ __launch_bounds__(256, (zi_combine_waves<M, E, WGC_INLINE>())) void zi_combine_kernel(ZCombineArgs a, SpecGeom g, const cplx* __restrict__ twM_g,
                                                         const cplx* __restrict__ twN_g, acc_t* __restrict__ partial) {
    extern __shared__ __attribute__((aligned(16))) real lds[];
    const cplx *twM, *twN;
    const ZTwReq<M, E> twq = z_tw_request<M, E>(twM_g, twN_g);
    a.ds = a.ds.resolved();
    const ZLane<M, E> z(g, lds);
    const real ctf = kCtf;
    real* park = lds + ZW<M, E>::LDS / sizeof(real) + threadIdx.x;
#pragma unroll
    for (int s = 0; s < kParkSlots; ++s) park[s * 256] = 0.0;
    cplx n[E], vacc[E], w[E];
    z_load_real<M, E, true>(n, z, a.ds.src);
    z_tw_commit<M, E>(lds, twq, twM_g, twN_g, twM, twN);
    using PL = typename ZW<M, E>::PL;
#pragma unroll
    for (int q = 0; q < E; ++q) {
        n[q] = (z.valid && PL::slot_out(q) && PL::lane_out(z.j, q)) ? mkc(a.ds(n[q].x), a.ds(n[q].y)) : mkc(1.0, 1.0);
        vacc[q] = mkc(0.0, 0.0);
    }
    const real sc = a.inv_n;
    const real w_tf = a.wts_w ? (real)a.wts_w[0] : (real)1.0, w_nl = a.wts_w ? (real)a.wts_w[1] : (real)1.0;
    constexpr unsigned kRootTerms = 4u | 8u | 16u | (0xFu << 6) | (1u << 13);
    constexpr bool ROOTS_ONCE = OFDFT_ZI_ROOTS_ONCE != 0;
    cplx yv[ROOTS_ONCE ? E : 1];
    if constexpr (ROOTS_ONCE) {
        if (a.mask & kRootTerms) {
#pragma unroll
            for (int q = 0; q < E; ++q)
                yv[q] = mkc(n[q].x != 0.0 ? fm::rsixth(n[q].x) : (real)0.0, n[q].y != 0.0 ? fm::rsixth(n[q].y) : (real)0.0);
        }
    }
    auto root_y = [&](int q, int c) -> real {
        if constexpr (ROOTS_ONCE) return c ? yv[q].y : yv[q].x;
        else {
            const real nn = c ? n[q].y : n[q].x;
            return nn != 0.0 ? fm::rsixth(nn) : (real)0.0;
        }
    };
    constexpr bool PIPE = OFDFT_Z_PREFETCH && !WGC_INLINE && (M < 512 || (sizeof(real) == 4 && OFDFT_Z_PIPE_BIG_F32));
    const bool gga = (a.mask & (7u << 10)) != 0;
    const cplx* chain[6] = {(a.mask & 2u) ? a.vh : nullptr,  (a.mask & 8u) ? a.lap : nullptr, (a.mask & 16u) ? a.conv_b : nullptr,
                            (a.mask & 16u) ? a.conv_a : nullptr, gga ? a.div : nullptr, gga ? a.div2 : nullptr};
    cplx nx[PIPE ? E : 1];
    real nyq_nx = 0.0;
    auto request_after = [&](auto ic) {
        constexpr int I = decltype(ic)::value;
        const cplx* p = nullptr;
#pragma unroll
        for (int k = 5; k > I; --k)
            if (chain[k]) p = chain[k];
        if constexpr (PIPE)
            if (p) z_issue_row<M, E>(nx, nyq_nx, z, p, g);
    };
    auto take_row = [&](auto ic, const cplx* spec) {
        if constexpr (PIPE) {
#pragma unroll
            for (int q = 0; q < E; ++q) w[q] = nx[q];
            const real nyq_w = nyq_nx;
            request_after(ic);
            z_inverse_regs<M, E>(w, z, twM, twN, nyq_w);
        } else {
            z_load_inverse<M, E>(w, z, spec, g, twM, twN);
        }
    };
    request_after(std::integral_constant<int, -1>{});
    if (a.mask & 2u) {
        take_row(std::integral_constant<int, 0>{}, a.vh);
        real e = 0.0;
#pragma unroll
        for (int q = 0; q < E; ++q) {
            const real x0 = w[q].x * sc, x1 = w[q].y * sc;
            e += 0.5 * (n[q].x * x0 + n[q].y * x1);
            vacc[q].x += x0;
            vacc[q].y += x1;
        }
        park[kParkH * 256] = e;
    }
    if (a.mask & 8u) {
        take_row(std::integral_constant<int, 1>{}, a.lap);
        real e = 0.0;
#pragma unroll
        for (int q = 0; q < E; ++q) {
            __builtin_amdgcn_sched_barrier(0);
            const real x0 = w[q].x * sc, x1 = w[q].y * sc;
            const real y0 = root_y(q, 0), y1 = root_y(q, 1);
            const real r0 = y0 * y0 * y0, r1 = y1 * y1 * y1;
            e += -0.5 * (n[q].x * r0 * x0 + n[q].y * r1 * x1);
            vacc[q].x += -0.5 * x0 * r0;
            vacc[q].y += -0.5 * x1 * r1;
        }
        park[kParkVw * 256] = e;
    }
    if (a.mask & 16u) {
        take_row(std::integral_constant<int, 2>{}, a.conv_b);
        cplx pa1[E];
        real e = 0.0;
#pragma unroll
        for (int q = 0; q < E; ++q) {
            __builtin_amdgcn_sched_barrier(0);
            const real x0 = w[q].x * sc, x1 = w[q].y * sc;
            pa1[q] = a.wt_is_56 ? mkc(root_y(q, 0), root_y(q, 1)) : mkc(pow_pos(n[q].x, a.wt_alpha - 1.0), pow_pos(n[q].y, a.wt_alpha - 1.0));
            e += ctf * ((pa1[q].x * n[q].x - a.wt_nbar_pa) * x0 + (pa1[q].y * n[q].y - a.wt_nbar_pa) * x1);
            const real f = w_nl * (a.conv_a ? a.wt_alpha : 2.0 * a.wt_alpha);
            vacc[q].x += ctf * f * pa1[q].x * x0;
            vacc[q].y += ctf * f * pa1[q].y * x1;
        }
        park[kParkWt * 256] = e;
        if (a.conv_a) {
            take_row(std::integral_constant<int, 3>{}, a.conv_a);
#pragma unroll
            for (int q = 0; q < E; ++q) {
                vacc[q].x += w_nl * ctf * a.wt_beta * pow_pos(n[q].x, a.wt_beta - 1.0) * w[q].x * sc;
                vacc[q].y += w_nl * ctf * a.wt_beta * pow_pos(n[q].y, a.wt_beta - 1.0) * w[q].y * sc;
            }
        }
    }
    if (a.mask & 32u) {
        if (WGC_INLINE) {
            park[kParkWgc * 256] = wgc_row_section<M, E>(n, vacc, w, z, a, g, twM, twN, sc, ctf);
        } else if (!a.v_part_deferred) {
            z_load_real<M, E, true>(w, z, a.v_part);
#pragma unroll
            for (int q = 0; q < E; ++q) {
                vacc[q].x += w[q].x;
                vacc[q].y += w[q].y;
            }
        }
    }
    if (a.mask & (7u << 10)) {
        take_row(std::integral_constant<int, 4>{}, a.div);
        cplx d[E];
        z_load_real<M, E, true>(d, z, a.dfdn);
#pragma unroll
        for (int q = 0; q < E; ++q) {
            vacc[q].x += d[q].x - 2.0 * w[q].x * sc;
            vacc[q].y += d[q].y - 2.0 * w[q].y * sc;
        }
        if (a.div2) {
            take_row(std::integral_constant<int, 5>{}, a.div2);
#pragma unroll
            for (int q = 0; q < E; ++q) {
                vacc[q].x -= 2.0 * w[q].x * sc;
                vacc[q].y -= 2.0 * w[q].y * sc;
            }
        }
    }
    if (a.mask & 1u) {
        cplx ve[E];
        z_load_real<M, E, true>(ve, z, a.vext);
        real e = 0.0;
#pragma unroll
        for (int q = 0; q < E; ++q) {
            e += n[q].x * ve[q].x + n[q].y * ve[q].y;
            vacc[q].x += ve[q].x;
            vacc[q].y += ve[q].y;
        }
        park[kParkIe * 256] = e;
    }
    acc_t acc[kCombineScalars];
#pragma unroll
    for (int s = 0; s < kCombineScalars; ++s) acc[s] = 0.0;
#pragma unroll
    for (int q = 0; q < E; ++q) {
        __builtin_amdgcn_sched_barrier(0);
        if (!(PL::slot_out(q) && PL::lane_out(z.j, q))) continue;
        const fm::Roots<real> rt0 = fm::roots_from_y(n[q].x, root_y(q, 0)), rt1 = fm::roots_from_y(n[q].y, root_y(q, 1));
        if (a.mask & 4u) {
            const real c0 = rt0.n13, c1 = rt1.n13;
            acc[2] += ctf * (c0 * c0 * n[q].x + c1 * c1 * n[q].y);
            vacc[q].x += w_tf * (5.0 / 3.0) * ctf * c0 * c0;
            vacc[q].y += w_tf * (5.0 / 3.0) * ctf * c1 * c1;
        }
        if (a.mask & (1u << 13)) {
            real e0, v0, e1, v1;
            vwgtf_point(n[q].x, rt0.n13, ctf, a.gtf_inv_n0, a.gtf_kind, e0, v0);
            vwgtf_point(n[q].y, rt1.n13, ctf, a.gtf_inv_n0, a.gtf_kind, e1, v1);
            acc[9] += e0 + e1;
            vacc[q].x += v0;
            vacc[q].y += v1;
        }
        if (a.mask & (0xFu << 6)) {
            const XcLocal x0 = lda_point(n[q].x, a.mask, rt0), x1 = lda_point(n[q].y, a.mask, rt1);
            acc[6] += x0.ex + x1.ex;
            acc[7] += x0.ec + x1.ec;
            vacc[q].x += x0.vx + x0.vc;
            vacc[q].y += x1.vx + x1.vc;
        }
        acc[8] += vacc[q].x * n[q].x + vacc[q].y * n[q].y;
    }
    acc[0] = park[kParkIe * 256];
    acc[1] = park[kParkH * 256];
    acc[3] = park[kParkVw * 256];
    acc[4] = park[kParkWt * 256];
    acc[5] = park[kParkWgc * 256];
    if (!z.valid) {
#pragma unroll
        for (int s = 0; s < kCombineScalars; ++s) acc[s] = 0.0;
    }
    if (a.v_out) z_store_real<M, E>(vacc, z, a.v_out);
    block_reduce_store<kCombineScalars>(acc, partial + (long long)g.blk0 * kCombineScalars);
}

template <int M, int E>
__global__ __launch_bounds__(256, (z_waves<M, E>(OFDFT_ZIWGC_WAVES))) void zi_wgc_kernel(ZCombineArgs a, real* __restrict__ v_part, SpecGeom g,
                                                       const cplx* __restrict__ twM_g, const cplx* __restrict__ twN_g,
                                                       acc_t* __restrict__ partial) {
    extern __shared__ __attribute__((aligned(16))) real lds[];
    const cplx *twM, *twN;
    const ZTwReq<M, E> twq = z_tw_request<M, E>(twM_g, twN_g);
    a.ds = a.ds.resolved();
    const ZLane<M, E> z(g, lds);
    const real ctf = kCtf;
    cplx n[E], vacc[E], w[E];
    z_load_real<M, E, true>(n, z, a.ds.src);
    z_tw_commit<M, E>(lds, twq, twM_g, twN_g, twM, twN);
    using PL = typename ZW<M, E>::PL;
#pragma unroll
    for (int q = 0; q < E; ++q) {
        n[q] = (z.valid && PL::slot_out(q) && PL::lane_out(z.j, q)) ? mkc(a.ds(n[q].x), a.ds(n[q].y)) : mkc(1.0, 1.0);
        vacc[q] = mkc(0.0, 0.0);
    }
    acc_t acc[2];
    acc[0] = wgc_row_section<M, E>(n, vacc, w, z, a, g, twM, twN, a.inv_n, ctf);
    acc[1] = 0.0;
#pragma unroll
    for (int q = 0; q < E; ++q)
        if (PL::slot_out(q) && PL::lane_out(z.j, q)) acc[1] += vacc[q].x * n[q].x + vacc[q].y * n[q].y;
    if (!z.valid) acc[0] = acc[1] = 0.0;
    z_store_real<M, E>(vacc, z, v_part);
    block_reduce_store<2>(acc, partial + (long long)g.blk0 * 2);
}

}
```

Baseline: 394.7 evals/s.

## Fold Hartree potential into GGA divergence spectrum and integrate Hartree energy in x pass

Adds a default-on pot_spectrum path. In the GGA-split case, the Hartree potential spectrum is no longer produced as a separate output and inverse-transformed on its own. The Hartree term is now added into the divergence x pass with the k^-2 coefficient, and the y-derivative kernel gains an add-input variant so the second gradient component is combined there. The Hartree energy is integrated in reciprocal space inside the x-pass kernel as per-block partials, which one combine block then sums. This removes one spectral buffer, one inverse transform and one potential row read in the z combine, at the cost of extra inputs in the x pass and a serial partial sum in a single block.

```diff
diff --git a/include/ofdft_hip.h b/include/ofdft_hip.h
--- a/include/ofdft_hip.h
+++ b/include/ofdft_hip.h
@@ -155,6 +155,7 @@
 #define OFDFT_OPT_IPC_WAIT_MS 13
 #define OFDFT_OPT_TEST_FAULT 11
 #define OFDFT_OPT_BS_FUSED 15
+#define OFDFT_OPT_POT_SPECTRUM 16
 #define OFDFT_OPT_WGC_FOLD 28
 #define OFDFT_OPT_XWAVE 8
 int  ofdft_set_option(ofdft_ctx* ctx, int option, double value);
diff --git a/professad_amd/csrc/engine.hip b/professad_amd/csrc/engine.hip
--- a/professad_amd/csrc/engine.hip
+++ b/professad_amd/csrc/engine.hip
@@ -1520,6 +1520,9 @@
         case OFDFT_OPT_GGA_SPLIT:
             c->gga_split = value != 0.0;
             return OFDFT_OK;
+        case OFDFT_OPT_POT_SPECTRUM:
+            c->pot_spectrum = value != 0.0;
+            return OFDFT_OK;
         case OFDFT_OPT_SPLIT_COMBINE:
             c->split_combine = value != 0.0;
             c->defer_vpart = value != 1.0;
diff --git a/professad_amd/csrc/engine_ctx.h b/professad_amd/csrc/engine_ctx.h
--- a/professad_amd/csrc/engine_ctx.h
+++ b/professad_amd/csrc/engine_ctx.h
@@ -60,6 +60,7 @@
     double wgc_ck = 0.0;
     bool wgc_fold = true;
     int fft_count = 0, launch_count = 0;
+    int xpass_blocks = 0;
     unsigned xpass_kinds = 0;
     double ypass_count = 0.0;
     float last_ms = 0.f;
@@ -70,6 +71,7 @@
     bool bs_fused = true;
     bool use_bluestein = true;
     bool gga_split = true;
+    bool pot_spectrum = true;
     bool split_combine = true;
     bool defer_vpart = true;
     int ybatch = 1;
@@ -266,6 +268,7 @@
 template <bool INV> int fast_axis_pass(ofdft_ctx* c, int axis, cplx* spec, hipStream_t st);
 template <bool INV> int ypass_xchg(ofdft_ctx* c, const std::vector<cplx*>& list, cplx* buf, hipStream_t st, int xk = -1);
 int yderiv(ofdft_ctx* c, const cplx* in, cplx* out, double scale, hipStream_t st, cplx* fwd = nullptr);
+int yderiv_add(ofdft_ctx* c, const cplx* in, const cplx* add, cplx* out, double scale, hipStream_t st);
 int rfftn_internal(ofdft_ctx* c, const real* in, cplx* spec, hipStream_t st);
 int rfftn_internal_multi(ofdft_ctx* c, const real* const* in, cplx* const* spec, int n, hipStream_t st);
 bool bluestein_xmix_ok(const ofdft_ctx* c);
@@ -288,6 +291,9 @@
 template <int NIN, int NOUT, class Mix>
 int xfused(ofdft_ctx* c, const XfIo& io, const Mix& mix, hipStream_t st, const char* nm, const XfLayout& lay = XfLayout{});
 int xfused_wgc(ofdft_ctx* c, const XfIo& io, const MixWgc& mix, hipStream_t st, const char* nm, const XfLayout& lay = XfLayout{});
+template <int NIN, class Mix>
+int xfused_energy(ofdft_ctx* c, const XfIo& io, const Mix& mix, hipStream_t st, const char* nm);
+bool xfused_energy_serves(const ofdft_ctx* c, int nin);
 
 int launch_zf_density(ofdft_ctx* c, const DenSrc& ds, cplx* out_n, cplx* out_s, hipStream_t st, int chunk = 0, int nchunks = 1,
                       real* dzn = nullptr);
diff --git a/professad_amd/csrc/engine_zfused.inc.h b/professad_amd/csrc/engine_zfused.inc.h
--- a/professad_amd/csrc/engine_zfused.inc.h
+++ b/professad_amd/csrc/engine_zfused.inc.h
@@ -34,6 +34,7 @@
     std::vector<cplx*> xlist[2];
     bool gsplit = false;
     bool lapl = false;
+    bool pspec = false;
     cplx* s_l = nullptr;
     real* dzn = nullptr;
     bool wgc_yinv_done = false;
@@ -91,6 +92,7 @@
     r.wgc_yinv_done = false;
     r.s_g[0] = r.s_g[1] = r.s_g[2] = nullptr;
     r.s_n = r.s_s = r.s_vh = r.s_b = r.s_a = nullptr;
+    r.pspec = false;
     if ((mask & OFDFT_ION_ELECTRON) && !r.vext) return fail(c, OFDFT_EINVAL, "IonElectron term needs vext");
     r.setup_done = true;
     return 0;
@@ -119,6 +121,7 @@
             r.gsplit = r.has_g && c->gga_split;
             r.lapl = r.gsplit && gga_needs_laplacian(c);
             r.s_l = nullptr;
+            r.pspec = r.gsplit && r.has_h && !dx && c->pot_spectrum && xfused_energy_serves(c, r.lapl ? 3 : 2);
             if (r.gsplit) {
                 if ((rc = real_ws(c, "dzn", &r.dzn))) return rc;
                 if ((rc = spec_ws(c, "zgx", &r.s_g[0]))) return rc;
@@ -262,7 +265,8 @@
             XfIo io{};
             io.in[0] = in_of(r.s_n);
             int no = 0;
-            if (r.has_h) {
+            const bool vh = r.has_h && !r.pspec;
+            if (vh) {
                 if ((rc = spec_ws(c, "zvh", &r.s_vh))) return rc;
                 io.out[no++] = out_of(r.s_vh);
             }
@@ -276,9 +280,9 @@
                     io.out[no++] = out_of(r.s_g[k]);
                 }
             }
-            if (r.lapl && r.has_h) rc = xfused<1, 3>(c, io, MixDensityA<true, true>{c->kg}, st, "xfused_n", lay);
+            if (r.lapl && vh) rc = xfused<1, 3>(c, io, MixDensityA<true, true>{c->kg}, st, "xfused_n", lay);
             else if (r.lapl) rc = xfused<1, 2>(c, io, MixDensityA<false, true>{c->kg}, st, "xfused_n", lay);
-            else if (r.gsplit && r.has_h) rc = xfused<1, 2>(c, io, MixDensityA<true>{c->kg}, st, "xfused_n", lay);
+            else if (r.gsplit && vh) rc = xfused<1, 2>(c, io, MixDensityA<true>{c->kg}, st, "xfused_n", lay);
             else if (r.gsplit) rc = xfused<1, 1>(c, io, MixDensityA<false>{c->kg}, st, "xfused_n", lay);
             else if (r.has_h && r.has_g) rc = xfused<1, 4>(c, io, MixDensity<true, true>{c->kg}, st, "xfused_n", lay);
             else if (r.has_h) rc = xfused<1, 1>(c, io, MixDensity<true, false>{c->kg}, st, "xfused_n", lay);
@@ -404,14 +408,14 @@
         r.stage[1] = 3;
         return 0;
     }
-    if (r.has_h) r.za.vh = r.s_vh;
+    if (r.has_h && !r.pspec) r.za.vh = r.s_vh;
     if (r.s_s) r.za.lap = r.s_s;
     if (r.has_g && r.gsplit) {
         if ((rc = real_ws(c, "dfdn", &r.dfdn))) return rc;
         if ((rc = launch_zpbe2(c, r.ds, r.s_g[0], r.s_g[1], r.dzn, r.dfdn, r.za.inv_n, &r.pbe_blocks, st, r.lapl ? r.s_l : nullptr)))
             return rc;
         OFDFT_REDUCE(c, st, c->d_partial, r.pbe_blocks, kPbeScalars, c->d_reduced + kCombineScalars, c->h_partial + kCombineScalars);
-        if ((rc = yderiv(c, r.s_g[1], r.s_g[1], (double)c->n0g, st))) return rc;
+        if (!r.pspec && (rc = yderiv(c, r.s_g[1], r.s_g[1], (double)c->n0g, st))) return rc;
         if (!dx && (rc = fast_axis_pass<false>(c, 1, r.s_g[0], st))) return rc;
         xl.push_back(r.s_g[0]);
         if (r.lapl) {
@@ -455,7 +459,26 @@
     }
     r.xlist[chain].clear();
     const XcView xv = xc_view(c, xk < 0 ? 0 : xk);
-    if (chain == 0 && r.has_g && r.gsplit) {
+    if (chain == 0 && r.pspec) {
+        acc_t* ehp;
+        const size_t rows = (size_t)(c->gx.total / c->gx.n0) + 1;
+        if (int rc = get_ws(c, "zh:part", sizeof(acc_t) * rows, (void**)&ehp)) return rc;
+        XfIo dio{};
+        dio.in[0] = dio.out[0] = r.s_g[0];
+        const double ehpref = 2.0 * kPi / (double)c->npts_g;
+        if (r.lapl) {
+            dio.in[1] = r.s_l;
+            dio.in[2] = r.s_n;
+            if (int rc = xfused_energy<3>(c, dio, MixDerivAH<true>{c->kg, ehp, ehpref, c->n2 / 2}, st, "xfused_div")) return rc;
+        } else {
+            dio.in[1] = r.s_n;
+            if (int rc = xfused_energy<2>(c, dio, MixDerivAH<false>{c->kg, ehp, ehpref, c->n2 / 2}, st, "xfused_div")) return rc;
+        }
+        r.za.eh_part = ehp;
+        r.za.eh_rows = c->xpass_blocks;
+        c->fft_count++;
+        r.xlist[0].push_back(r.s_g[0]);
+    } else if (chain == 0 && r.has_g && r.gsplit) {
         XfIo dio{};
         XfLayout lay{};
         dio.in[0] = dio.out[0] = r.s_g[0];
@@ -529,6 +552,8 @@
             cplx *send, *recv;
             if ((rc = dist_buffers(c, 0, &send, &recv))) return rc;
             if (part != 2 && (rc = ypass_xchg<true>(c, {dsp}, recv, st))) return rc;
+        } else if (r.pspec) {
+            if ((rc = yderiv_add(c, r.s_g[1], dsp, dsp, (double)c->n0g, st))) return rc;
         } else if (chunked) {
             r.deferred.push_back(dsp);
         } else if ((rc = fast_axis_pass<true>(c, 1, dsp, st))) {
@@ -536,7 +561,7 @@
         }
         c->fft_count++;
         r.za.div = dsp;
-        r.za.div2 = r.gsplit ? r.s_g[1] : nullptr;
+        r.za.div2 = (r.gsplit && !r.pspec) ? r.s_g[1] : nullptr;
         r.za.dfdn = r.dfdn;
     }
     r.xlist[0].clear();
diff --git a/professad_amd/csrc/fft_kernels.h b/professad_amd/csrc/fft_kernels.h
--- a/professad_amd/csrc/fft_kernels.h
+++ b/professad_amd/csrc/fft_kernels.h
@@ -173,11 +173,11 @@
     }
 }
 
-template <int LEN>
+template <int LEN, bool ADD = false>
 __global__ __launch_bounds__(PassCfg<LEN>::TPB) void yderiv_kernel(const cplx* in, cplx* out,
                                                                    LineMap m_main, LineMap m_rem, int main_blocks,
                                                                    long long rem_offset, const cplx* __restrict__ tw,
-                                                                   real scale, cplx* fwd) {
+                                                                   real scale, cplx* fwd, const cplx* add = nullptr) {
     constexpr int P = PassCfg<LEN>::P, E = PassCfg<LEN>::E, LPW = PassCfg<LEN>::LPW;
     extern __shared__ __attribute__((aligned(16))) real lds[];
     const int tid = threadIdx.x;
@@ -199,6 +199,12 @@
 #pragma unroll
     for (int q = 0; q < E; ++q)
         v[q] = (PL::slot_in(q) && valid && PL::lane_in(j, q)) ? buf_load_c(in + roff + b0 + PL::cin(q) * se_u, voff) : mkc(0.0, 0.0);
+    cplx x[ADD ? E : 1];
+    if constexpr (ADD) {
+#pragma unroll
+        for (int q = 0; q < E; ++q)
+            x[q] = (PL::slot_out(q) && valid && PL::lane_out(j, q)) ? buf_load_c(add + roff + b0 + PL::cout(q) * se_u, voff) : mkc(0.0, 0.0);
+    }
     real* mine = lds + l * PassCfg<LEN>::LSTR;
     line_fft<LEN, false, kCX>(v, j, mine, tw);
     if (fwd && valid) {
@@ -211,6 +217,7 @@
         const int e = j + PL::cout(q);
         const real f = scale * (real)(e <= LEN / 2 ? e : e - LEN);
         v[q] = mkc(-f * v[q].y, f * v[q].x);
+        if constexpr (ADD) v[q] = cadd(v[q], x[q]);
     }
     __syncthreads();
     repattern_out_to_in<PL, false>(v, j, mine);
diff --git a/professad_amd/csrc/lines.hip b/professad_amd/csrc/lines.hip
--- a/professad_amd/csrc/lines.hip
+++ b/professad_amd/csrc/lines.hip
@@ -579,6 +579,34 @@
     if (fwd) c->fft_passes_fused++, c->yfwd_fused++;
     return 0;
 }
+template <int LEN>
+int launch_yderiv_add_t(ofdft_ctx* c, const cplx* in, const cplx* add, cplx* out, double scale, hipStream_t st) {
+    cplx* tw;
+    if (int rc = get_twiddle(c, LEN, &tw)) return rc;
+    using Cfg = PassCfg<LEN>;
+    LineMap main, rem;
+    pass_maps(c, 1, main, rem);
+    const int mb = (main.nlines + Cfg::LPW - 1) / Cfg::LPW, rb = (rem.nlines + Cfg::LPW - 1) / Cfg::LPW;
+    OFDFT_LAUNCH(c, st, "yderiv", (yderiv_kernel<LEN, true>), dim3(mb + rb), dim3(Cfg::TPB), Cfg::LDS, in, out, main, rem, mb,
+                 c->g.main_count, (const cplx*)tw, (real)scale, (cplx*)nullptr, add);
+    return 0;
+}
+int yderiv_add(ofdft_ctx* c, const cplx* in, const cplx* add, cplx* out, double scale, hipStream_t st) {
+    switch (c->n1) {
+        case 8: return launch_yderiv_add_t<8>(c, in, add, out, scale, st);
+        case 16: return launch_yderiv_add_t<16>(c, in, add, out, scale, st);
+        case 32: return launch_yderiv_add_t<32>(c, in, add, out, scale, st);
+        case 64: return launch_yderiv_add_t<64>(c, in, add, out, scale, st);
+        case 128: return launch_yderiv_add_t<128>(c, in, add, out, scale, st);
+        case 256: return launch_yderiv_add_t<256>(c, in, add, out, scale, st);
+        case 512: return launch_yderiv_add_t<512>(c, in, add, out, scale, st);
+        case 1024: return launch_yderiv_add_t<1024>(c, in, add, out, scale, st);
+#define X(L) case L: return launch_yderiv_add_t<L>(c, in, add, out, scale, st);
+        OFDFT_MIXED_LINES(X)
+#undef X
+    }
+    return fail(c, OFDFT_EINVAL, "unsupported fast FFT length %d", c->n1);
+}
 int yderiv(ofdft_ctx* c, const cplx* in, cplx* out, double scale, hipStream_t st, cplx* fwd) {
     switch (c->n1) {
         case 8: return launch_yderiv_t<8>(c, in, out, scale, st, fwd);
diff --git a/professad_amd/csrc/pointwise_kernels.h b/professad_amd/csrc/pointwise_kernels.h
--- a/professad_amd/csrc/pointwise_kernels.h
+++ b/professad_amd/csrc/pointwise_kernels.h
@@ -445,6 +445,39 @@
             kvec_xyz(kg, x, y, z, kx, ky, kz, k2);
             return 0.5 * k2;
         }
+    }
+};
+
+template <bool HAS_L> struct MixDerivAH {
+    KGeom kg;
+    acc_t* epart;
+    double ehpref;
+    int kz_nyq;
+    static constexpr bool kEnergy = true;
+    static constexpr int NI = HAS_L ? 3 : 2;
+    static __device__ __forceinline__ constexpr bool imag(int) { return true; }
+    template <int O, int I> static __device__ __forceinline__ constexpr bool present() { return true; }
+    template <int O, int I> static __device__ __forceinline__ constexpr bool imag_oi() { return I == 0; }
+    template <int O, int I>
+    __device__ __forceinline__ real coef(int x, int y, int z, long long, unsigned) const {
+        if constexpr (I == 0) {
+            return ifreq(x, kg.g.n0);
+        } else {
+            real kx, ky, kz, k2;
+            kvec_xyz(kg, x, y, z, kx, ky, kz, k2);
+            if constexpr (HAS_L && I == 1) return 0.5 * k2;
+            return (k2 != 0.0) ? -2.0 * kPiR / k2 : 0.0;
+        }
+    }
+    template <int NIN>
+    __device__ __forceinline__ acc_t energy(const cplx (&in)[NIN], int x, int y, int z) const {
+        static_assert(NIN == NI, "inputs");
+        real kx, ky, kz, k2;
+        kvec_xyz(kg, x, y, z, kx, ky, kz, k2);
+        if (k2 == 0.0) return 0.0;
+        const cplx nk = in[NIN - 1];
+        const acc_t w = (z == 0 || z == kz_nyq) ? 1.0 : 2.0;
+        return w * ehpref * ((acc_t)nk.x * nk.x + (acc_t)nk.y * nk.y) / (acc_t)k2;
     }
 };
 
diff --git a/professad_amd/csrc/xcross.h b/professad_amd/csrc/xcross.h
--- a/professad_amd/csrc/xcross.h
+++ b/professad_amd/csrc/xcross.h
@@ -227,6 +227,7 @@
                 for (int ap = 0; ap < A; ++ap) v[I][nl][r + RR * ap] = c[ap];
             }
     });
+    acc_t eacc = 0.0;
 #pragma unroll
     for (int nl = 0; nl < NL; ++nl)
 #pragma unroll
@@ -236,6 +237,7 @@
             for (int I = 0; I < NIN; ++I) in[I] = v[I][nl][q];
             if constexpr (NC > 0) mix.apply(out, in, cfs[nl][q]);
             else xw_outputs<NIN, NOUT, 0, Mix>(out, in, mix, J + PP * q, y[nl], kz[nl], b0 + q * tqstep, tloff + nl);
+            if constexpr (mix_has_energy<Mix>::value) eacc += mix.energy(in, J + PP * q, y[nl], kz[nl]);
 #pragma unroll
             for (int O = 0; O < NOUT; ++O) v[O][nl][q] = out[O];
         }
@@ -281,6 +283,7 @@
             }
         }
     });
-}
-
-}
+    if constexpr (mix_has_energy<Mix>::value) xpart_store<TPB>(eacc, mix.epart, lds);
+}
+
+}
diff --git a/professad_amd/csrc/xpass_a.hip b/professad_amd/csrc/xpass_a.hip
--- a/professad_amd/csrc/xpass_a.hip
+++ b/professad_amd/csrc/xpass_a.hip
@@ -6,5 +6,19 @@
 template int xfused<1, 1, MixScale<SPEC_LINDHARD>>(ofdft_ctx*, const XfIo&, const MixScale<SPEC_LINDHARD>&, hipStream_t, const char*, const XfLayout&);
 template int xfused<1, 1, MixDerivA>(ofdft_ctx*, const XfIo&, const MixDerivA&, hipStream_t, const char*, const XfLayout&);
 template int xfused<2, 1, MixDerivAL>(ofdft_ctx*, const XfIo&, const MixDerivAL&, hipStream_t, const char*, const XfLayout&);
+template int xfused_energy<2, MixDerivAH<false>>(ofdft_ctx*, const XfIo&, const MixDerivAH<false>&, hipStream_t, const char*);
+template int xfused_energy<3, MixDerivAH<true>>(ofdft_ctx*, const XfIo&, const MixDerivAH<true>&, hipStream_t, const char*);
 template int xfused<3, 1, MixDiv>(ofdft_ctx*, const XfIo&, const MixDiv&, hipStream_t, const char*, const XfLayout&);
+bool xfused_energy_serves(const ofdft_ctx* c, int nin) {
+    const bool xc = nin == 2 ? xc_serves<2, 1>(c) : xc_serves<3, 1>(c);
+    const bool xc_len = c->n0g == 128 || c->n0g == 256 || c->n0g == 512 || c->n0g == 1024;
+    const bool xw = c->use_xwave == 2 || c->use_xwave == 1 || c->use_xwave >= 5 || (c->use_xwave == 4 && c->n0g < 512);
+    if (xc && xc_len && XcCfg<1024>::NL > 1 && c->n0g == 1024) {
+        LineMap m, r;
+        pass_maps(c, 0, m, r);
+        constexpr int NL = XcCfg<1024>::NL;
+        if (m.sl != 1 || r.sl != 1 || m.d % NL || r.d % NL || m.nlines % NL || r.nlines % NL) return false;
+    }
+    return (xc && xc_len) || (xw && is_pow2(c->n0g) && c->n0g >= 8 && c->n0g <= 512);
 }
+}
diff --git a/professad_amd/csrc/xpass_impl.h b/professad_amd/csrc/xpass_impl.h
--- a/professad_amd/csrc/xpass_impl.h
+++ b/professad_amd/csrc/xpass_impl.h
@@ -6,6 +6,8 @@
 
 template <int LEN, int NIN, int NOUT, class Mix>
 int launch_xfused_t(ofdft_ctx* c, const XfIo& io, const Mix& mix, const XfLayout& lay, hipStream_t st, const char* nm) {
+    if constexpr (mix_has_energy<Mix>::value)
+        return fail(c, OFDFT_EINVAL, "%s: the group-parallel x pass does not integrate energies", nm);
     constexpr int G = NIN > NOUT ? NIN : NOUT;
     using Cfg = XfCfg<LEN, G, NOUT>;
     cplx* tw;
@@ -35,6 +37,7 @@
     main.blk0 = line0 / Cfg::LPW;
     const int mb = (main.nlines - line0 + Cfg::LPW - 1) / Cfg::LPW, rb = (rem.nlines + Cfg::LPW - 1) / Cfg::LPW;
     c->xpass_kinds |= OFDFT_XPASS_GROUP;
+    c->xpass_blocks = mb + rb;
     OFDFT_LAUNCH(c, st, nm, (xfused_kernel<LEN, NIN, NOUT, Mix>), dim3(mb + rb), dim3(Cfg::TPB), Cfg::LDS, io, main, rem, mb,
                  gk, tw, mix, XfStride{lay.se_out, lay.tse});
     return 0;
@@ -71,6 +74,7 @@
     main.blk0 = line0 / Cfg::LPB;
     const int mb = (main.nlines - line0 + Cfg::LPB - 1) / Cfg::LPB, rb = (rem.nlines + Cfg::LPB - 1) / Cfg::LPB;
     c->xpass_kinds |= OFDFT_XPASS_WAVE;
+    c->xpass_blocks = mb + rb;
     OFDFT_LAUNCH(c, st, nm, (xw_kernel<LEN, NIN, NOUT, Mix>), dim3(mb + rb), dim3(Cfg::TPB), Cfg::LDS, io, main, rem, mb, gk,
                  (const cplx*)tw, mix, XfStride{lay.se_out, lay.tse});
     return 0;
@@ -124,6 +128,7 @@
         }
     }
     c->xpass_kinds |= Cfg::NL == 2 ? OFDFT_XPASS_CROSS2 : OFDFT_XPASS_CROSS1;
+    c->xpass_blocks = mb + rb;
     OFDFT_LAUNCH(c, st, nm, (xc_kernel<LEN, NIN, NOUT, Mix>), dim3(mb + rb), dim3(Cfg::TPB), lds, io, main, rem, mb, gk,
                  (const cplx*)tw, mix, XfStride{lay.se_out, lay.tse});
     return 0;
@@ -174,4 +179,27 @@
     return fail(c, OFDFT_EINVAL, "unsupported fast FFT length %d", c->n0g);
 }
 
-}
+template <int NIN, class Mix>
+int xfused_energy(ofdft_ctx* c, const XfIo& io, const Mix& mix, hipStream_t st, const char* nm) {
+    const XfLayout lay{};
+    if (xc_serves<NIN, 1>(c)) {
+        switch (c->n0g) {
+            case 128: return launch_xc_t<128, NIN, 1, Mix>(c, io, mix, lay, st, nm);
+            case 256: return launch_xc_t<256, NIN, 1, Mix>(c, io, mix, lay, st, nm);
+            case 512: return launch_xc_t<512, NIN, 1, Mix>(c, io, mix, lay, st, nm);
+            case 1024: return launch_xc_t<1024, NIN, 1, Mix>(c, io, mix, lay, st, nm);
+        }
+    }
+    switch (c->n0g) {
+        case 8: return launch_xw_t<8, NIN, 1, Mix>(c, io, mix, lay, st, nm);
+        case 16: return launch_xw_t<16, NIN, 1, Mix>(c, io, mix, lay, st, nm);
+        case 32: return launch_xw_t<32, NIN, 1, Mix>(c, io, mix, lay, st, nm);
+        case 64: return launch_xw_t<64, NIN, 1, Mix>(c, io, mix, lay, st, nm);
+        case 128: return launch_xw_t<128, NIN, 1, Mix>(c, io, mix, lay, st, nm);
+        case 256: return launch_xw_t<256, NIN, 1, Mix>(c, io, mix, lay, st, nm);
+        case 512: return launch_xw_t<512, NIN, 1, Mix>(c, io, mix, lay, st, nm);
+    }
+    return fail(c, OFDFT_EINVAL, "%s: no energy-integrating x pass for %d-point lines", nm, c->n0g);
+}
+
+}
diff --git a/professad_amd/csrc/xwave.h b/professad_amd/csrc/xwave.h
--- a/professad_amd/csrc/xwave.h
+++ b/professad_amd/csrc/xwave.h
@@ -54,6 +54,23 @@
 template <class Mix> struct mix_has_fold<Mix, std::void_t<decltype(std::declval<const Mix&>().fold_n0)>> : std::true_type {};
 template <class Mix, class = void> struct mix_coef_count { static constexpr int N = 0; };
 template <class Mix> struct mix_coef_count<Mix, std::void_t<decltype(Mix::kTableReals)>> { static constexpr int N = Mix::kTableReals; };
+template <class Mix, class = void> struct mix_has_energy : std::false_type {};
+template <class Mix> struct mix_has_energy<Mix, std::void_t<decltype(Mix::kEnergy)>> : std::bool_constant<Mix::kEnergy> {};
+template <int TPB>
+__device__ __forceinline__ void xpart_store(acc_t v, acc_t* __restrict__ out, real* lds) {
+#pragma unroll
+    for (int off = 32; off > 0; off >>= 1) v += __shfl_down(v, off, 64);
+    acc_t* red = reinterpret_cast<acc_t*>(lds);
+    __syncthreads();
+    if ((threadIdx.x & 63) == 0) red[threadIdx.x >> 6] = v;
+    __syncthreads();
+    if (threadIdx.x == 0) {
+        acc_t t = 0.0;
+#pragma unroll
+        for (int w = 0; w < TPB / 64; ++w) t += red[w];
+        out[blockIdx.x] = t;
+    }
+}
 
 template <int NIN, int NOUT, int O, int I, class Mix>
 __device__ __forceinline__ void xw_accumulate(real& acr, real& aci, const cplx (&in)[NIN], const Mix& mix, int x, int y, int kz,
@@ -172,6 +189,7 @@
         xw_line_fft<LEN, false>(a[I], j, mine, tw, lx);
         exchange_sync<true>();
     });
+    acc_t eacc = 0.0;
 #pragma unroll
     for (int q = 0; q < E; ++q) {
         cplx in[NIN], out[NOUT];
@@ -179,6 +197,7 @@
         for (int I = 0; I < NIN; ++I) in[I] = a[I][q];
         if constexpr (NC > 0) mix.apply(out, in, cfs[q]);
         else xw_outputs<NIN, NOUT, 0, Mix>(out, in, mix, j + P * q, y, kz, b0 + q * tqstep, tloff);
+        if constexpr (mix_has_energy<Mix>::value) eacc += mix.energy(in, j + P * q, y, kz);
 #pragma unroll
         for (int O = 0; O < NOUT; ++O) a[O][q] = out[O];
     }
@@ -195,6 +214,7 @@
             }
         }
     });
-}
-
-}
+    if constexpr (mix_has_energy<Mix>::value) xpart_store<Cfg::TPB>(eacc, mix.epart, lds);
+}
+
+}
diff --git a/professad_amd/csrc/zpass.h b/professad_amd/csrc/zpass.h
--- a/professad_amd/csrc/zpass.h
+++ b/professad_amd/csrc/zpass.h
@@ -658,6 +658,8 @@
     const cplx* gw[3];
     const cplx* div;
     const cplx* div2;
+    const acc_t* eh_part;
+    long long eh_rows;
     real* v_out;
     const real* v_part;
     int v_part_deferred;
@@ -817,7 +819,7 @@
         }
     };
     request_after(std::integral_constant<int, -1>{});
-    if (a.mask & 2u) {
+    if ((a.mask & 2u) && a.vh) {
         take_row(std::integral_constant<int, 0>{}, a.vh);
         real e = 0.0;
 #pragma unroll
@@ -949,6 +951,9 @@
     if (!z.valid) {
 #pragma unroll
         for (int s = 0; s < kCombineScalars; ++s) acc[s] = 0.0;
+    }
+    if (a.eh_part && g.blk0 + blockIdx.x == 0) {
+        for (long long i = threadIdx.x; i < a.eh_rows; i += blockDim.x) acc[1] += a.eh_part[i];
     }
     if (a.v_out) z_store_real<M, E>(vacc, z, a.v_out);
     block_reduce_store<kCombineScalars>(acc, partial + (long long)g.blk0 * kCombineScalars);
```

Result: faster. 411.8 evals/s (median of 6 runs) (+4.3%).
